# banyancomputer/hot-proofs-blake3-circom

Hardware: AMD Instinct MI355X
Metric: BLAKE3-compression witnesses/sec (higher is better)
Workload: dtype u32

## Files before the change

hot-proofs-blake3-circom_amd/__init__.py:

```python
import ctypes
import os
import re

import numpy as np

from . import workloads


def __getattr__(name):
    if name in ("sharding", "chain", "bao"):
        import importlib
        return importlib.import_module(__name__ + "." + name)
    raise AttributeError(name)

PKG_DIR = os.path.dirname(os.path.abspath(__file__))
LIB_PATH = os.environ.get("B3WIT_LIB") or os.path.join(PKG_DIR, "libb3wit.so")

CIRCUITS = ("compression", "nova_bn254", "nova_vesta", "nova_bn254_o1")
CIRCUIT_ID = {c: i for i, c in enumerate(CIRCUITS)}

B3W_OK = 0
PLACEMENT_NAMES = {0: "plain", 1: "mixed", 2: "interleaved"}
B3W_E_ASSERT_FAILED = 4
B3W_E_BAD_ARGUMENT = 100
B3W_E_NO_DEVICE = 101
B3W_E_DOMAIN = 103

_CIRCOM_ERR = {1: "Signal not found.\n", 2: "Too many signals set.\n", 3: "Signal already set.\n",
               4: "Assert Failed.\n", 5: "Not enough memory.\n", 6: "Input signal array access exceeds the size.\n"}


class B3WError(RuntimeError):
    def __init__(self, status, message):
        super().__init__(message)
        self.status = status


_lib = None


def lib():
    global _lib
    if _lib is not None:
        return _lib
    if not os.path.exists(LIB_PATH):
        raise B3WError(B3W_E_NO_DEVICE, f"{LIB_PATH} not built: run `python -c 'import __graft_entry__ as g; g.build()'`")
    try:
        import torch
    except ImportError:
        pass
    L = ctypes.CDLL(LIB_PATH)
    vp, u32, i32, u64, sz = ctypes.c_void_p, ctypes.c_uint32, ctypes.c_int32, ctypes.c_uint64, ctypes.c_size_t
    sig = {
        "b3w_abi_version": (u32, []),
        "b3w_identify_wasm": (i32, [vp, sz]),
        "b3w_create": (i32, [i32, i32, ctypes.POINTER(vp)]),
        "b3w_destroy": (None, [vp]),
        "b3w_info": (i32, [vp, vp, vp, vp, vp, vp]),
        "b3w_input_signal_size": (i32, [vp, u64]),
        "b3w_calc_witness": (i32, [vp, vp, vp, vp, u32, vp]),
        "b3w_write_wtns_header": (i32, [vp, vp]),
        "b3w_last_error": (i32, [vp, ctypes.c_char_p, sz]),
        "b3w_batch_run_device": (i32, [vp, vp, u32, vp, u64, vp, vp, vp]),
        "b3w_public_words": (u32, [vp]),
        "b3w_batch_alloc": (i32, [vp, u32, u64, ctypes.POINTER(vp)]),
        "b3w_batch_free": (None, [vp]),
        "b3w_batch_run": (i32, [vp, vp, u32, vp]),
        "b3w_batch_outputs": (i32, [vp, vp, vp]),
        "b3w_batch_fetch": (i32, [vp, u32, vp]),
        "b3w_batch_device_ptr": (vp, [vp, ctypes.POINTER(u64)]),
        "b3w_batch_time_device": (i32, [vp, vp, u32, vp, u64, vp, vp, vp, u32, ctypes.POINTER(ctypes.c_float)]),
        "b3w_batch_verify_device": (i32, [vp, vp, u32, u64, vp, vp]),
        "b3w_batch_verify": (i32, [vp, vp]),
        "b3w_r1cs_create": (i32, [vp, vp, sz, ctypes.POINTER(vp)]),
        "b3w_r1cs_info": (i32, [vp, ctypes.POINTER(u32), ctypes.POINTER(u32), ctypes.POINTER(u64), ctypes.POINTER(u32),
                                ctypes.POINTER(u32), ctypes.POINTER(u32)]),
        "b3w_r1cs_is_tiled": (i32, [vp]),
        "b3w_r1cs_destroy": (None, [vp]),
        "b3w_r1cs_check_device": (i32, [vp, vp, vp, u32, u64, vp, vp, vp]),
        "b3w_batch_r1cs_check": (i32, [vp, vp, vp, vp]),
        "b3w_r1cs_consumer": (None, [vp, vp, u64, u64, u32, vp]),
        "b3w_batch_write_wtns": (i32, [vp, u32, u32, ctypes.c_char_p, ctypes.c_char_p, ctypes.POINTER(u32)]),
        "b3w_batch_write_wtns_ex": (i32, [vp, u32, u32, ctypes.c_char_p, ctypes.c_char_p, u32, ctypes.POINTER(u32)]),
        "b3w_batch_autotune_device": (i32, [vp, vp, u32, vp, u64, vp, vp, vp, ctypes.POINTER(i32), ctypes.POINTER(ctypes.c_float)]),
        "b3w_bodies_alloc": (i32, [vp, u64, ctypes.POINTER(vp), ctypes.POINTER(i32)]),
        "b3w_bodies_free": (i32, [vp, vp]),
        "b3w_bodies_trim": (None, []),
        "b3w_ctx_trim": (i32, [vp]),
        "b3w_bodies_configure": (None, [ctypes.c_int64, ctypes.c_int64]),
        "b3w_bodies_stats": (i32, [vp, vp]),
        "b3w_bodies_search_stats": (i32, [vp, ctypes.POINTER(ctypes.c_double)]),
        "b3w_bodies_search_limit": (None, [ctypes.c_double]),
        "b3w_bodies_search_breakdown": (i32, [vp, ctypes.POINTER(ctypes.c_double)]),
        "b3w_bodies_store_rate": (i32, [vp, vp, u32, u64, i32, u32, vp, ctypes.POINTER(ctypes.c_double)]),
        "b3w_batch_placement": (i32, [vp]),
        "b3w_chain_num_chunks": (u64, [u64]),
        "b3w_chain_num_leaf_steps": (u64, [u64]),
        "b3w_chain_path_len": (u32, [u64, u64]),
        "b3w_chain_num_parent_steps": (u64, [u64, u64, u64]),
        "b3w_chain_parent_row": (u64, [u64, u64]),
        "b3w_chain_path_provable": (i32, [u64, u64]),
        "b3w_chain_plan_leaves_device": (i32, [vp, vp, u64, u64, u32, vp, vp, vp]),
        "b3w_chain_tree_device": (i32, [vp, vp, u64, vp, vp]),
        "b3w_chain_plan_parents_device": (i32, [vp, vp, u64, u64, u64, u32, vp, vp]),
        "b3w_commit_key_create": (i32, [vp, i32, u32, vp, ctypes.POINTER(vp)]),
        "b3w_commit_key_create_ex": (i32, [vp, i32, u32, vp, u32, ctypes.POINTER(vp)]),
        "b3w_commit_key_create_folded": (i32, [vp, i32, u32, vp, vp, u32, ctypes.POINTER(vp)]),
        "b3w_slot_widths": (i32, [vp, vp]),
        "b3w_commit_key_window": (u32, [vp]),
        "b3w_commit_key_destroy": (None, [vp]),
        "b3w_commit_key_count": (i32, [vp, i32]),
        "b3w_commit_key_counts": (i32, [vp, ctypes.POINTER(u64)]),
        "b3w_commit_records_device": (i32, [vp, vp, vp, u32, vp, vp, vp, vp]),
        "b3w_commit_records": (i32, [vp, vp, vp, u32, vp, vp, vp]),
        "b3w_chain_commit_only": (i32, [vp, vp, vp]),
        "b3w_chain_commit_from_records": (i32, [vp, vp, vp]),
        "b3w_chain_commit_overlap": (i32, [vp, i32]),
        "b3w_chain_violations_device": (vp, [vp]),
        "b3w_chain_commitments": (i32, [vp, vp, vp]),
        "b3w_chain_check_constraints": (i32, [vp, vp]),
        "b3w_chain_violations": (i32, [vp, vp, vp]),
        "b3w_batch_commit_device": (i32, [vp, vp, vp, u32, u64, vp, vp, vp]),
        "b3w_batch_commit": (i32, [vp, vp, vp, vp]),
        "b3w_commit_consumer": (None, [vp, vp, u64, u64, u32, vp]),
        "b3w_comm_unique_id": (i32, [vp]),
        "b3w_comm_create": (i32, [vp, vp, i32, i32, ctypes.POINTER(vp)]),
        "b3w_comm_create_host": (i32, [vp, ctypes.c_char_p, i32, i32, ctypes.POINTER(vp)]),
        "b3w_comm_create_external": (i32, [vp, i32, i32, vp, vp, ctypes.POINTER(vp)]),
        "b3w_comm_rank": (i32, [vp]),
        "b3w_comm_size": (i32, [vp]),
        "b3w_comm_destroy": (None, [vp]),
        "b3w_comm_allgather": (i32, [vp, vp, vp, u64, vp]),
        "b3w_batch_allgather_public": (i32, [vp, vp, vp]),
        "b3w_chain_create": (i32, [vp, u64, u64, u32, u32, u32, i32, ctypes.POINTER(vp)]),
        "b3w_chain_destroy": (None, [vp]),
        "b3w_chain_run_leaves": (i32, [vp, vp, vp, vp, vp]),
        "b3w_chain_run_parents": (i32, [vp, vp, vp, vp, vp]),
        "b3w_chain_shard": (None, [u64, i32, i32, ctypes.POINTER(u64), ctypes.POINTER(u32)]),
        "b3w_chain_run_parents_sharded": (i32, [vp, vp, vp, vp, vp]),
        "b3w_chain_allgather_hout": (i32, [vp, vp, vp, vp, vp]),
        "b3w_chain_allgather_hout_host": (i32, [vp, vp, vp, vp, vp]),
        "b3w_chain_exchange_ms": (i32, [vp, ctypes.POINTER(ctypes.c_float)]),
        "b3w_chain_info": (i32, [vp, ctypes.POINTER(u64), ctypes.POINTER(u64), ctypes.POINTER(u64), ctypes.POINTER(u32), ctypes.POINTER(i32)]),
        "b3w_chain_outputs": (i32, [vp, vp, vp, vp, vp]),
        "b3w_chain_records": (vp, [vp]),
        "b3w_chain_public": (vp, [vp]),
        "b3w_chain_status": (vp, [vp]),
        "b3w_chain_local_cvs": (vp, [vp]),
        "b3w_chain_root": (vp, [vp]),
        "b3w_bao_outboard_size": (u64, [u64]),
        "b3w_bao_outboard_device": (i32, [vp, vp, u64, vp, vp, vp, vp]),
        "b3w_bao_path_nodes": (i32, [u64, u64, ctypes.POINTER(u64), ctypes.POINTER(u32)]),
        "b3w_bao_slice": (i32, [vp, u64, u64, vp, vp, ctypes.POINTER(u64)]),
        "b3w_sample_rows": (ctypes.c_int64, [u64, vp, u32, vp]),
        "b3w_sample_plan_device": (i32, [vp, u64, vp, vp, vp, u32, vp, vp, vp, vp]),
        "b3w_bao_batch_layout": (u64, [vp, u32, vp]),
        "b3w_bao_batch_scratch_bytes": (u64, [vp, u32]),
        "b3w_bao_outboard_batch_device": (i32, [vp, vp, vp, vp, u32, vp, vp, vp, u64, vp]),
        "b3w_sample_rows_batch": (ctypes.c_int64, [vp, u32, vp, vp, u32, vp]),
        "b3w_sample_plan_batch_device": (i32, [vp, vp, u32, vp, vp, vp, vp, u32, vp, vp, vp, vp]),
        "b3w_bao_group_outboard_size": (u64, [u64, u32]),
        "b3w_bao_group_batch_layout": (u64, [vp, u32, u32, vp]),
        "b3w_bao_group_path_nodes": (i32, [u64, u64, u32, ctypes.POINTER(u64), ctypes.POINTER(u32)]),
        "b3w_bao_group_outboard_batch_device": (i32, [vp, vp, vp, vp, u32, u32, vp, vp, vp, u64, vp]),
        "b3w_sample_plan_group_batch_device": (i32, [vp, vp, u32, u32, vp, vp, vp, vp, u32, vp, vp, vp, vp]),
        "b3w_bao_slice_size": (u64, [u64, u64]),
        "b3w_bao_slice_batch_layout": (ctypes.c_int64, [vp, u32, vp, vp, u32, vp]),
        "b3w_bao_slice_decode": (i32, [vp, u64, u64, u64, vp, vp, ctypes.POINTER(u32), ctypes.POINTER(i32)]),
        "b3w_bao_slice_batch_device": (i32, [vp, vp, u32, u32, vp, vp, vp, u32, vp, vp, vp]),
        "b3w_sample_plan_slices_device": (i32, [vp, vp, u32, vp, vp, vp, u32, vp, vp, vp, vp]),
        "b3w_bao_verify_layout": (u64, [vp, u32, u32, vp]),
        "b3w_bao_verify_scratch_bytes": (u64, [vp, u32]),
        "b3w_bao_verify_batch_device": (i32, [vp, vp, vp, vp, u32, u32, vp, vp, vp, vp, vp, vp, u64, vp]),
        "b3w_bao_verify": (i32, [vp, u64, vp, u32, vp, vp, ctypes.POINTER(i32), ctypes.POINTER(u64)]),
        "b3w_bao_stream_scratch_bytes": (u64, [u64, u32]),
        "b3w_bao_stream_outboard_begin": (i32, [vp, u64, u32, vp, vp, vp, u64, ctypes.POINTER(vp)]),
        "b3w_bao_stream_verify_begin": (i32, [vp, u64, u32, vp, vp, vp, vp, vp, vp, u64, vp, ctypes.POINTER(vp)]),
        "b3w_bao_stream_push": (i32, [vp, u64, vp, u64, vp]),
        "b3w_bao_stream_finish": (i32, [vp, vp]),
        "b3w_bao_stream_free": (None, [vp]),
        "b3w_bao_stream_push_many": (i32, [vp, vp, vp, vp, vp, u32, vp]),
        "b3w_bao_stream_finish_many": (i32, [vp, vp, u32, vp]),
        "b3w_bao_stream_open_staging_bytes": (u64, [u64, u32]),
        "b3w_bao_stream_open_scratch_bytes": (u64, [u64]),
        "b3w_bao_stream_open_block_pos": (u64, [u64, u32, u64]),
        "b3w_bao_stream_open_begin": (i32, [vp, u64, u32, vp, u64, vp, u64, ctypes.POINTER(vp)]),
        "b3w_bao_stream_open_finish": (i32, [vp, vp, u64, vp, u64, vp, vp, ctypes.POINTER(u64)]),
        "b3w_bao_stream_open_finish_many": (i32, [vp, vp, vp, vp, vp, vp, vp, u32, vp, vp]),
        "b3w_sample_plan_arena_device": (i32, [vp, vp, u64, vp, vp, u32, u32, vp, vp, vp, vp, u32, vp, vp, vp]),
        "b3w_bao_slice_arena_device": (i32, [vp, vp, u64, vp, vp, u32, u32, vp, vp, vp, u32, vp, vp]),
        "b3w_bao_update_scratch_bytes": (u64, [vp, vp, vp, vp, u32]),
        "b3w_bao_outboard_update_batch_device": (i32, [vp, vp, u64, vp, vp, u32, u32, vp, vp, vp, vp, vp, vp, u32, vp, u64, vp]),
        "b3w_bao_outboard_update": (i32, [vp, u64, vp, u32, vp, vp, u32, vp]),
        "b3w_bao_resize_kept_tiles": (u64, [u64, u64]),
        "b3w_bao_resize_scratch_bytes": (u64, [vp, vp, u32]),
        "b3w_bao_outboard_resize_batch_device": (i32, [vp, vp, u64, vp, vp, vp, u32, u32, vp, vp, vp, vp, vp, vp, u32, vp, u64, vp]),
        "b3w_bao_outboard_resize": (i32, [vp, u64, vp, u64, u32, vp, vp]),
        "b3w_bao_verify_ranges_scratch_bytes": (u64, [vp, vp, vp, vp, u32]),
        "b3w_bao_verify_ranges_batch_device": (i32, [vp, vp, u64, vp, vp, u32, u32, vp, vp, vp, vp, vp, vp, u32, vp, vp, vp, vp, vp, u64, vp]),
        "b3w_bao_verify_ranges": (i32, [vp, u64, vp, u32, vp, vp, vp, u32, vp, vp, vp]),
    }
    for name, (res, args) in sig.items():
        fn = getattr(L, name)
        fn.restype, fn.argtypes = res, args
    _lib = L
    return L


EXPORTED_SYMBOLS = ("b3w_abi_version", "b3w_identify_wasm", "b3w_create", "b3w_destroy", "b3w_info",
                    "b3w_input_signal_size", "b3w_calc_witness", "b3w_write_wtns_header", "b3w_last_error",
                    "b3w_batch_run_device", "b3w_public_words", "b3w_batch_alloc", "b3w_batch_free",
                    "b3w_batch_run", "b3w_batch_outputs", "b3w_batch_fetch", "b3w_batch_device_ptr",
                    "b3w_batch_time_device", "b3w_batch_verify_device", "b3w_batch_verify",
                    "b3w_r1cs_create", "b3w_r1cs_info", "b3w_r1cs_is_tiled", "b3w_r1cs_destroy", "b3w_r1cs_check_device", "b3w_batch_r1cs_check", "b3w_r1cs_consumer", "b3w_batch_write_wtns", "b3w_batch_write_wtns_ex", "b3w_batch_autotune_device", "b3w_bodies_alloc", "b3w_bodies_free", "b3w_bodies_trim", "b3w_ctx_trim", "b3w_bodies_configure", "b3w_bodies_stats", "b3w_bodies_search_stats", "b3w_bodies_search_limit", "b3w_bodies_search_breakdown", "b3w_bodies_store_rate", "b3w_batch_placement", "b3w_chain_num_chunks", "b3w_chain_num_leaf_steps", "b3w_chain_path_len",
                    "b3w_chain_num_parent_steps", "b3w_chain_parent_row", "b3w_chain_path_provable",
                    "b3w_chain_plan_leaves_device", "b3w_chain_tree_device", "b3w_chain_plan_parents_device",
                    "b3w_commit_key_create", "b3w_commit_key_create_ex", "b3w_commit_key_create_folded", "b3w_slot_widths", "b3w_commit_key_window", "b3w_commit_key_destroy", "b3w_commit_key_count", "b3w_commit_key_counts", "b3w_commit_records_device", "b3w_commit_records", "b3w_chain_commit_only", "b3w_chain_commit_from_records", "b3w_chain_commit_overlap", "b3w_chain_violations_device", "b3w_chain_commitments", "b3w_chain_check_constraints", "b3w_chain_violations", "b3w_batch_commit_device", "b3w_batch_commit", "b3w_commit_consumer",
                    "b3w_comm_unique_id", "b3w_comm_create", "b3w_comm_create_host", "b3w_comm_create_external", "b3w_comm_rank", "b3w_comm_size", "b3w_comm_destroy", "b3w_comm_allgather", "b3w_batch_allgather_public",
                    "b3w_chain_create", "b3w_chain_destroy", "b3w_chain_run_leaves", "b3w_chain_run_parents", "b3w_chain_shard", "b3w_chain_run_parents_sharded", "b3w_chain_allgather_hout", "b3w_chain_allgather_hout_host", "b3w_chain_exchange_ms", "b3w_chain_info",
                    "b3w_chain_outputs", "b3w_chain_records", "b3w_chain_public", "b3w_chain_status", "b3w_chain_local_cvs", "b3w_chain_root",
                    "b3w_bao_outboard_size", "b3w_bao_outboard_device", "b3w_bao_path_nodes", "b3w_bao_slice", "b3w_sample_rows",
                    "b3w_sample_plan_device", "b3w_bao_batch_layout", "b3w_bao_batch_scratch_bytes", "b3w_bao_outboard_batch_device",
                    "b3w_sample_rows_batch", "b3w_sample_plan_batch_device", "b3w_bao_group_outboard_size", "b3w_bao_group_batch_layout",
                    "b3w_bao_group_path_nodes", "b3w_bao_group_outboard_batch_device", "b3w_sample_plan_group_batch_device",
                    "b3w_bao_slice_size", "b3w_bao_slice_batch_layout", "b3w_bao_slice_decode", "b3w_bao_slice_batch_device",
                    "b3w_sample_plan_slices_device",
                    "b3w_bao_verify_layout", "b3w_bao_verify_scratch_bytes", "b3w_bao_verify_batch_device", "b3w_bao_verify",
                    "b3w_bao_stream_scratch_bytes", "b3w_bao_stream_outboard_begin", "b3w_bao_stream_verify_begin", "b3w_bao_stream_push",
                    "b3w_bao_stream_finish", "b3w_bao_stream_free", "b3w_bao_stream_push_many", "b3w_bao_stream_finish_many",
                    "b3w_bao_stream_open_staging_bytes", "b3w_bao_stream_open_scratch_bytes", "b3w_bao_stream_open_block_pos",
                    "b3w_bao_stream_open_begin", "b3w_bao_stream_open_finish", "b3w_bao_stream_open_finish_many",
                    "b3w_sample_plan_arena_device", "b3w_bao_slice_arena_device",
                    "b3w_bao_update_scratch_bytes", "b3w_bao_outboard_update_batch_device", "b3w_bao_outboard_update",
                    "b3w_bao_resize_kept_tiles", "b3w_bao_resize_scratch_bytes", "b3w_bao_outboard_resize_batch_device", "b3w_bao_outboard_resize",
                    "b3w_bao_verify_ranges_scratch_bytes", "b3w_bao_verify_ranges_batch_device", "b3w_bao_verify_ranges")


class graph_capture:

    def __init__(self, graph, stream=None, **kw):
        import torch
        self._inner = torch.cuda.graph(graph, stream=stream, **kw)
        self._gc_was_on = False

    def __enter__(self):
        import gc
        gc.collect()
        self._gc_was_on = gc.isenabled()
        gc.disable()
        try:
            return self._inner.__enter__()
        except BaseException:
            if self._gc_was_on:
                gc.enable()
            raise

    def __exit__(self, *exc):
        import gc
        try:
            return self._inner.__exit__(*exc)
        finally:
            if self._gc_was_on:
                gc.enable()


def fnv_hash(name):
    h = 0xCBF29CE484222325
    for ch in name:
        h ^= ord(ch)
        h = (h * 0x100000001B3) % (1 << 64)
    return h


def flat_array(a):
    out = []

    def fill(x):
        if isinstance(x, (list, tuple)):
            for y in x:
                fill(y)
        else:
            out.append(x)
    fill(a)
    return out


def _to_int(v):
    if isinstance(v, str):
        return int(v, 0)
    return int(v)


class Context:

    def __init__(self, circuit, device=0):
        self.circuit = circuit if isinstance(circuit, str) else CIRCUITS[circuit]
        self._lib = lib()
        h = ctypes.c_void_p()
        rc = self._lib.b3w_create(CIRCUIT_ID[self.circuit], int(device), ctypes.byref(h))
        if rc != B3W_OK:
# ... 183 lines not shown
        c._cb = _ALLGATHER_FN(_cb)
        h = ctypes.c_void_p()
        rc = lib().b3w_comm_create_external(ctx.handle, int(rank), int(nranks), ctypes.cast(c._cb, ctypes.c_void_p), None, ctypes.byref(h))
        if rc != B3W_OK:
            raise B3WError(rc, f"b3w_comm_create_external: status {rc}: {ctx.last_error()}")
        c.handle = h
        return c

    def allgather(self, d_send, d_recv, bytes_per_rank, stream=0):
        rc = lib().b3w_comm_allgather(self.handle, d_send, d_recv, bytes_per_rank, stream or None)
        if rc != B3W_OK:
            err, self._cb_error = self._cb_error, None
            raise B3WError(rc, f"b3w_comm_allgather: status {rc}: {self.ctx.last_error()}" + (f" ({err!r})" if err else ""))

    def close(self):
        if getattr(self, "handle", None):
            lib().b3w_comm_destroy(self.handle)
            self.handle = None


R1CS_DIR = os.path.join(PKG_DIR, "constraints")
BUILTIN_R1CS = {"compression": "blake3_compression.r1cs.gz", "nova_bn254_o1": "blake3_nova_bn254_o1.r1cs.gz",
                "nova_bn254": "blake3_nova_bn254.r1cs.gz", "nova_vesta": "blake3_nova_vesta.r1cs.gz"}


def read_r1cs_image(image):
    if isinstance(image, (str, os.PathLike)):
        path = image if os.path.exists(image) else os.path.join(R1CS_DIR, image)
        raw = open(path, "rb").read()
        if raw[:2] == b"\x1f\x8b":
            import gzip
            raw = gzip.decompress(raw)
        return raw
    return bytes(image)


class R1cs:

    def __init__(self, ctx, image=None):
        self.ctx = ctx
        if image is None:
            if ctx.circuit not in BUILTIN_R1CS:
                raise B3WError(100, f"no derived constraint system for {ctx.circuit}: pass the circuit's .r1cs")
            image = os.path.join(R1CS_DIR, BUILTIN_R1CS[ctx.circuit])
        if isinstance(image, (str, os.PathLike)):
            raw = open(image, "rb").read()
            if raw[:2] == b"\x1f\x8b":
                import gzip
                raw = gzip.decompress(raw)
            image = raw
        buf = bytes(image)
        h = ctypes.c_void_p()
        rc = lib().b3w_r1cs_create(ctx.handle, buf, len(buf), ctypes.byref(h))
        if rc != B3W_OK:
            raise B3WError(rc, f"b3w_r1cs_create: status {rc}: {ctx.last_error()}")
        self.handle = h
        m, nw, nt, po, pi, pr = (ctypes.c_uint32(), ctypes.c_uint32(), ctypes.c_uint64(), ctypes.c_uint32(), ctypes.c_uint32(),
                                 ctypes.c_uint32())
        lib().b3w_r1cs_info(h, ctypes.byref(m), ctypes.byref(nw), ctypes.byref(nt), ctypes.byref(po), ctypes.byref(pi), ctypes.byref(pr))
        self.n_constraints, self.n_wires, self.n_terms = m.value, nw.value, nt.value
        self.n_pub_out, self.n_pub_in, self.n_prv_in = po.value, pi.value, pr.value
        self.tiled = bool(lib().b3w_r1cs_is_tiled(h))

    def check_device(self, d_bodies, n, pitch, d_violations, d_first=0, stream=0):
        rc = lib().b3w_r1cs_check_device(self.ctx.handle, self.handle, d_bodies, n, pitch, d_violations, d_first or None, stream or None)
        if rc != B3W_OK:
            raise B3WError(rc, f"b3w_r1cs_check_device: status {rc}: {self.ctx.last_error()}")

    def close(self):
        if getattr(self, "handle", None):
            lib().b3w_r1cs_destroy(self.handle)
            self.handle = None

    def __del__(self):
        try:
            self.close()
        except Exception:
            pass


class CommitKey:
    CURVES = {"bn254_g1": 0, "pallas": 1, "vesta": 1}

    def __init__(self, ctx, curve, generators, first_slot=0, window=0, fold=None):
        self.ctx = ctx
        buf = bytes(generators)
        nslots = ctx.witness_size - first_slot
        if len(buf) != 64 * nslots:
            raise B3WError(100, "generators: 64 bytes per committed slot")
        self.folded_slots, mask = 0, None
        if fold is not None and fold is not False:
            from . import fold as _fold
            image = read_r1cs_image(BUILTIN_R1CS[ctx.circuit]) if fold is True else read_r1cs_image(fold)
            buf, mask, self.fold_stats = _fold.fold_generators(image, ctx.slot_widths(), first_slot, buf, curve)
            self.folded_slots = sum(1 for v in mask if v)
        h = ctypes.c_void_p()
        rc = lib().b3w_commit_key_create_folded(ctx.handle, self.CURVES[curve], first_slot, buf, bytes(mask) if mask is not None else None, window,
                                                ctypes.byref(h))
        if rc != B3W_OK:
            raise B3WError(rc, f"b3w_commit_key_create_folded: status {rc}: {ctx.last_error()}")
        self.handle = h
        self.window = lib().b3w_commit_key_window(h)

    def commit_device(self, d_bodies, n, pitch, d_points, d_status=0, stream=0):
        rc = lib().b3w_batch_commit_device(self.ctx.handle, self.handle, d_bodies, n, pitch, d_points, d_status or None, stream or None)
        if rc != B3W_OK:
            raise B3WError(rc, f"b3w_batch_commit_device: status {rc}: {self.ctx.last_error()}")

    def commit_records_device(self, d_records, n, d_points, d_status, d_public=0, stream=0):
        rc = lib().b3w_commit_records_device(self.ctx.handle, self.handle, d_records, n, d_points, d_public or None, d_status, stream or None)
        if rc != B3W_OK:
            raise B3WError(rc, f"b3w_commit_records_device: status {rc}: {self.ctx.last_error()}")

    def commit_records(self, records):
        recs = np.ascontiguousarray(records, dtype=np.uint32)
        n = recs.shape[0]
        pts = np.zeros((n, 64), dtype=np.uint8)
        pub = np.zeros((n, self.ctx.public_words), dtype=np.uint32)
        st = np.zeros(n, dtype=np.int32)
        rc = lib().b3w_commit_records(self.ctx.handle, self.handle, recs.ctypes.data, n, pts.ctypes.data, pub.ctypes.data, st.ctypes.data)
        if rc != B3W_OK:
            raise B3WError(rc, f"b3w_commit_records: status {rc}: {self.ctx.last_error()}")
        return pts, pub, st

    def count(self, on=True):
        lib().b3w_commit_key_count(self.handle, 1 if on else 0)

    def counts(self):
        out = (ctypes.c_uint64 * 2)()
        lib().b3w_commit_key_counts(self.handle, out)
        return int(out[0]), int(out[1])

    def close(self):
        if getattr(self, "handle", None):
            lib().b3w_commit_key_destroy(self.handle)
            self.handle = None

    def __del__(self):
        try:
            self.close()
        except Exception:
            pass


class ChainPlanner:

    def __init__(self, ctx):
        self.ctx = ctx

    def _chk(self, rc, what):
        if rc != B3W_OK:
            raise B3WError(rc, f"{what}: status {rc}: {self.ctx.last_error()}")

    def parent_rows(self, n_chunks, first_chunk=0, n_chunks_local=None):
        L = lib()
        nl = n_chunks - first_chunk if n_chunks_local is None else n_chunks_local
        r0 = L.b3w_chain_parent_row(first_chunk, n_chunks)
        return [(L.b3w_chain_parent_row(c, n_chunks) - r0, L.b3w_chain_path_len(c, n_chunks), bool(L.b3w_chain_path_provable(c, n_chunks)))
                for c in range(first_chunk, first_chunk + nl)]

    def plan(self, d_preimage, with_parents=True, first_chunk=0, n_chunks_local=None, stream=0):
        import torch
        L = lib()
        ln = d_preimage.numel()
        dev = d_preimage.device
        n = L.b3w_chain_num_chunks(ln)
        nl = n - first_chunk if n_chunks_local is None else n_chunks_local
        last_local = first_chunk + nl == n
        last_blocks = (max(ln - (n - 1) * 1024, 1) + 63) // 64
        n_leaf = nl * 16 - ((16 - last_blocks) if last_local else 0)
        P = L.b3w_chain_path_len(0, n)
        complete = (n & (n - 1)) == 0
        n_par = L.b3w_chain_num_parent_steps(ln, first_chunk, nl) if with_parents else 0
        recs = torch.zeros((nl * 16 + n_par, 32), dtype=torch.int32, device=dev)
        levels = torch.zeros(((2 * n + 64) * 8,), dtype=torch.int32, device=dev)
        root = torch.zeros(8, dtype=torch.int32, device=dev)
        s = stream or None
        allrecs = recs if (first_chunk == 0 and nl == n) else None
        if allrecs is None:
            tmp = torch.zeros((n * 16, 32), dtype=torch.int32, device=dev)
            self._chk(L.b3w_chain_plan_leaves_device(self.ctx.handle, d_preimage.data_ptr(), ln, 0, n, tmp.data_ptr(),
                                                     levels.data_ptr(), s), "plan_leaves")
            recs[:nl * 16] = tmp[first_chunk * 16:(first_chunk + nl) * 16]
        else:
            self._chk(L.b3w_chain_plan_leaves_device(self.ctx.handle, d_preimage.data_ptr(), ln, 0, n, recs.data_ptr(),
                                                     levels.data_ptr(), s), "plan_leaves")
        self._chk(L.b3w_chain_tree_device(self.ctx.handle, levels.data_ptr(), n, root.data_ptr(), s), "tree")
        if n_par:
            self._chk(L.b3w_chain_plan_parents_device(self.ctx.handle, levels.data_ptr(), n, ln, first_chunk, nl,
                                                      recs[nl * 16:].data_ptr(), s), "plan_parents")
        if last_local and last_blocks < 16:
            keep = torch.ones(recs.shape[0], dtype=torch.bool, device=dev)
            keep[(nl - 1) * 16 + last_blocks: nl * 16] = False
            recs = recs[keep].contiguous()
        return dict(records=recs, n_leaf_steps=n_leaf, n_parent_steps=n_par, chunk_cvs=levels[:n * 8].view(n, 8),
                    root=root, n_chunks=n, path_len=P, complete=complete, last_blocks=last_blocks)


class Batch:

    def __init__(self, ctx, capacity, pitch=0):
        self.ctx = ctx
        h = ctypes.c_void_p()
        rc = lib().b3w_batch_alloc(ctx.handle, capacity, pitch, ctypes.byref(h))
        if rc != B3W_OK:
            raise B3WError(rc, f"b3w_batch_alloc: status {rc}: {ctx.last_error()}")
        self.handle, self.capacity, self.n = h, capacity, 0

    def run(self, records):
        records = np.ascontiguousarray(records, dtype=np.uint32)
        assert records.ndim == 2 and records.shape[1] == self.ctx.input_size
        rc = lib().b3w_batch_run(self.handle, records.ctypes.data, records.shape[0], None)
        if rc != B3W_OK:
            raise B3WError(rc, f"b3w_batch_run: status {rc}: {self.ctx.last_error()}")
        self.n = records.shape[0]

    def outputs(self):
        pub = np.zeros((self.n, self.ctx.public_words), dtype=np.uint32)
        st = np.zeros(self.n, dtype=np.int32)
# ... 153 lines not shown
```

hot-proofs-blake3-circom_amd/build.py:

```python
import os, shutil, subprocess, sys

PKG = os.path.dirname(os.path.abspath(__file__))
ROOT = os.path.dirname(PKG)
CSRC = os.path.join(PKG, "csrc")
LIB = os.path.join(PKG, "libb3wit.so")
NAPI = os.path.join(PKG, "js", "b3wit_napi.node")
ARCH = "gfx950"


def _newer(target, sources):
    if not os.path.exists(target):
        return True
    t = os.path.getmtime(target)
    return any(os.path.getmtime(s) > t for s in sources)


def _run(cmd, **kw):
    print("+", " ".join(cmd), flush=True)
    subprocess.check_call(cmd, **kw)


def hipcc():
    for c in (os.environ.get("HIPCC"), shutil.which("hipcc"), "/opt/rocm/bin/hipcc"):
        if c and os.path.exists(c):
            return c
    raise RuntimeError("hipcc not found")


def build_lib(force=False, extra_flags=()):
    from concurrent.futures import ThreadPoolExecutor
    names = ("b3w_kernels.hip", "b3w_exact.hip", "b3w_plan.hip", "b3w_bao.hip", "b3w_placement.hip", "b3w_commit.hip", "b3w_r1cs.hip", "b3w_r1cs_walk.hip", "b3w_r1cs_host.cpp", "b3w_hostcomm.cpp",
             "b3w_ctx.cpp", "b3w_bodies.cpp", "b3w_wtns.cpp", "b3w_r1cs_api.cpp", "b3w_commit_api.cpp", "b3w_comm.cpp", "b3w_chain.cpp")
    srcs = [os.path.join(CSRC, f) for f in names]
    hdrs = [os.path.join(CSRC, f) for f in sorted(os.listdir(CSRC)) if f.endswith((".h", ".inc"))] + \
        [os.path.join(ROOT, "include", "b3wit.h")]
    objdir = os.path.join(PKG, "build")
    os.makedirs(objdir, exist_ok=True)
    if os.environ.get("B3W_BUILD_DIAG") == "1":
        extra_flags = (*extra_flags, "-DB3W_R1CS_DIAG")
    flags = [f"--offload-arch={ARCH}", "-O3", "-std=c++17", "-fPIC", "-x", "hip", "-Wall", "-Wno-unused-function", *extra_flags]
    jobs = []
    for src in srcs:
        obj = os.path.join(objdir, os.path.basename(src) + ".o")
        if force or extra_flags or _newer(obj, [src] + hdrs):
            jobs.append([hipcc(), *flags, "-c", src, "-o", obj])
    if jobs:
        with ThreadPoolExecutor(max_workers=min(len(jobs), os.cpu_count() or 1)) as ex:
            list(ex.map(_run, jobs))
    objs = [os.path.join(objdir, os.path.basename(src) + ".o") for src in srcs]
    if jobs or _newer(LIB, objs):
        _run([hipcc(), f"--offload-arch={ARCH}", "-fPIC", "-shared", "-o", LIB, *objs, "-ldl", "-lrt", "-lpthread"])
    return LIB


def build_oracle(force=False):
    so = os.path.join(ROOT, "oracle", "libb3w_oracle.so")
    if force or _newer(so, [os.path.join(ROOT, "oracle", "b3w_oracle.c")]):
        _run(["make", "-C", os.path.join(ROOT, "oracle")])
    return so


def build_napi(force=False):
    src = os.path.join(PKG, "js", "b3wit_napi.cc")
    if not os.path.exists(src):
        return None
    inc = "/usr/include/node"
    if not os.path.exists(os.path.join(inc, "node_api.h")):
        print("node_api.h not found; skipping N-API addon", file=sys.stderr)
        return None
    if force or _newer(NAPI, [src, os.path.join(ROOT, "include", "b3wit.h")]):
        _run(["g++", "-O2", "-std=c++17", "-fPIC", "-shared", "-DNODE_GYP_MODULE_NAME=b3wit_napi", "-I", inc,
              "-I", os.path.join(ROOT, "include"), "-o", NAPI, src, "-ldl"])
    return NAPI


def build_all(force=False):
    build_lib(force)
    build_oracle(force)
    build_napi(force)


if __name__ == "__main__":
    build_all(force="--force" in sys.argv)
```

hot-proofs-blake3-circom_amd/chain.py:

```python
import ctypes

import numpy as np
import torch
import torch.distributed as dist

from . import B3W_OK, PLACEMENT_NAMES, B3WError, lib
from .sharding import gather_rows, shard_range


def _chk(ctx, rc, what):
    if rc != B3W_OK:
        raise B3WError(rc, f"{what}: status {rc}: {ctx.last_error()}")


class _DevArray:

    def __init__(self, ptr, shape, typestr):
        self.__cuda_array_interface__ = {"shape": tuple(shape), "typestr": typestr, "data": (ptr, False), "version": 2,
                                         "strides": None}


def _view(ptr, shape, typestr, dev):
    return torch.as_tensor(_DevArray(ptr, shape, typestr), device=dev)


_CONSUMER = ctypes.CFUNCTYPE(None, ctypes.c_void_p, ctypes.c_void_p, ctypes.c_uint64, ctypes.c_uint64, ctypes.c_uint32,
                             ctypes.c_void_p)


def step_shards(preimage_len, world, with_parents=True):
    L = lib()
    n = L.b3w_chain_num_chunks(preimage_len)
    last_bytes = preimage_len - (n - 1) * 1024 if preimage_len > (n - 1) * 1024 else 0
    last_blocks = -(-last_bytes // 64) if last_bytes else 1
    out = []
    for r in range(world):
        f, e = shard_range(n, r, world)
        k = e - f
        leaf = k * 16 - ((16 - last_blocks) if (k and e == n) else 0)
        p0 = L.b3w_chain_parent_row(f, n) if with_parents else 0
        p1 = L.b3w_chain_parent_row(e, n) if with_parents else 0
        out.append((f, k, leaf, p0, p1 - p0))
    return out


def gather_h_out(public_local, n_leaf_local, preimage_len, with_parents=True, group=None):
    world = dist.get_world_size(group) if dist.is_initialized() else 1
    h = public_local[:, 2:10]
    if world == 1:
        return h[:n_leaf_local], h[n_leaf_local:]
    sh = step_shards(preimage_len, world, with_parents)
    leaf = gather_rows(h[:n_leaf_local].contiguous(), [x[2] for x in sh], group)
    par = gather_rows(h[n_leaf_local:].contiguous(), [x[4] for x in sh], group)
    return leaf, par


COMMIT_OVERLAP = {"auto": -1, "serial": 0, "free": 1, "gated": 2}


def fold_witnesses(ctx, preimage, batch_steps=16384, ring=2, slice_chunks=1024, with_parents=True, consumer=None,
                   device=None, commit_only=None, gather_hout=True, comm=None, commit_records=None, check=None, commit_overlap="auto"):
    L = lib()
    world = dist.get_world_size() if dist.is_initialized() else 1
    rank = dist.get_rank() if dist.is_initialized() else 0
    if comm is not None:
        world, rank = comm.nranks, comm.rank
    dev = device or torch.device("cuda", torch.cuda.current_device())
    host = torch.from_numpy(preimage) if isinstance(preimage, np.ndarray) else preimage
    assert host.dtype == torch.uint8 and host.dim() == 1 and host.numel() > 0 and host.is_contiguous()
    ln = host.numel()
    n = L.b3w_chain_num_chunks(ln)
    c0, c1 = shard_range(n, rank, world)
    nl = c1 - c0
    body = ctx.body_bytes

    cache = ctx.__dict__.setdefault("_chain_cache", {})
    key = (ln, c0, nl, batch_steps, ring, bool(with_parents))
    if key not in cache:
        for h in cache.values():
            L.b3w_chain_destroy(h)
        cache.clear()
        h = ctypes.c_void_p()
        _chk(ctx, L.b3w_chain_create(ctx.handle, ln, c0, nl, batch_steps, ring, 1 if with_parents else 0, ctypes.byref(h)),
             "b3w_chain_create")
        cache[key] = h
    h = cache[key]
    nleaf, npar, nch, P, pl = ctypes.c_uint64(), ctypes.c_uint64(), ctypes.c_uint64(), ctypes.c_uint32(), ctypes.c_int32()
    L.b3w_chain_info(h, ctypes.byref(nleaf), ctypes.byref(npar), ctypes.byref(nch), ctypes.byref(P), ctypes.byref(pl))
    n_leaf, n_par = nleaf.value, npar.value
    if commit_only is not None:
        _chk(ctx, L.b3w_chain_commit_only(h, commit_only[0].handle, commit_only[1].data_ptr()), "b3w_chain_commit_only")
    elif commit_records is not None:
        _chk(ctx, L.b3w_chain_commit_from_records(h, commit_records[0].handle, commit_records[1].data_ptr()), "b3w_chain_commit_from_records")
    else:
        _chk(ctx, L.b3w_chain_commit_only(h, None, None), "b3w_chain_commit_only")
    if commit_records is not None:
        _chk(ctx, L.b3w_chain_commit_overlap(h, COMMIT_OVERLAP[commit_overlap]), "b3w_chain_commit_overlap")
    _chk(ctx, L.b3w_chain_check_constraints(h, check.handle if check is not None else None), "b3w_chain_check_constraints")
    compute = torch.cuda.current_stream(dev)
    nbatch = [0]
    cb = _CONSUMER()
    if consumer is not None:
        def _cb(user, d_bodies, pitch, first_step, count, stream):
            nbatch[0] += 1
            consumer(_view(d_bodies, (count, body), "|u1", dev), first_step, count)
        cb = _CONSUMER(_cb)
    _chk(ctx, L.b3w_chain_run_leaves(h, host.data_ptr(), cb, None, compute.cuda_stream), "b3w_chain_run_leaves")

    rows = n_leaf + n_par
    public = _view(L.b3w_chain_public(h), (rows, 15), "<i4", dev)
    h_leaf, h_par = None, None
    timer = None
    if comm is not None:
        _chk(ctx, L.b3w_chain_run_parents_sharded(h, comm.handle, cb, None, compute.cuda_stream), "b3w_chain_run_parents_sharded")
        if gather_hout:
            sh = step_shards(ln, world, with_parents)
            h_leaf = torch.empty((sum(x[2] for x in sh), 8), dtype=torch.int32, device=dev)
            h_par = torch.empty((sum(x[4] for x in sh), 8), dtype=torch.int32, device=dev)
            with torch.cuda.stream(compute):
                _chk(ctx, L.b3w_chain_allgather_hout(h, comm.handle, h_leaf.data_ptr(), h_par.data_ptr() if h_par.numel() else None,
                                                     compute.cuda_stream), "b3w_chain_allgather_hout")
        timer = ("native", h, bool(gather_hout))
    else:
        all_cvs = None
        ev = [torch.cuda.Event(enable_timing=True) for _ in range(4)] if world > 1 else None
        if world > 1:
            ev[0].record(compute)
            cvs_local = _view(L.b3w_chain_local_cvs(h), (max(nl, 1), 8), "<i4", dev)
            all_cvs = gather_rows(cvs_local[:nl], [e - s for s, e in (shard_range(n, r, world) for r in range(world))]).contiguous()
            ev[1].record(compute)
        _chk(ctx, L.b3w_chain_run_parents(h, all_cvs.data_ptr() if all_cvs is not None else None, cb, None, compute.cuda_stream),
             "b3w_chain_run_parents")
        if gather_hout or world == 1:
            if world > 1:
                ev[2].record(compute)
            h_leaf, h_par = gather_h_out(public, n_leaf, ln, with_parents)
            if world > 1:
                ev[3].record(compute)
        if world > 1:
            timer = ("torch", ev, bool(gather_hout))

    return dict(public=public, h_out_all=h_leaf, h_out_parents_all=h_par, chunk_cvs_local=_view(L.b3w_chain_local_cvs(h), (max(nl, 1), 8), "<i4", dev)[:nl],
                status=_view(L.b3w_chain_status(h), (rows,), "<i4", dev),
                violations=_view(L.b3w_chain_violations_device(h), (rows,), "<i4", dev) if check is not None else None,
                records=_view(L.b3w_chain_records(h), (rows, 32), "<i4", dev), root=_view(L.b3w_chain_root(h), (8,), "<i4", dev),
                n_leaf_steps=n_leaf, n_parent_steps=n_par, first_chunk=c0, n_chunks_local=nl, n_chunks=n, path_len=P.value,
                batches=-(-n_leaf // batch_steps) + -(-n_par // batch_steps) if consumer is None else nbatch[0],
                placement=PLACEMENT_NAMES.get(pl.value, "plain"), exchange_timer=timer)


def exchange_ms(out):
    t = out.get("exchange_timer")
    if t is None:
        return 0.0, 0.0
    if t[0] == "native":
        ms = (ctypes.c_float * 2)()
        lib().b3w_chain_exchange_ms(t[1], ms)
        return float(ms[0]), float(ms[1]) if t[2] else 0.0
    ev = t[1]
    ev[1].synchronize()
    a = ev[0].elapsed_time(ev[1])
    b = 0.0
    if t[2]:
        ev[3].synchronize()
        b = ev[2].elapsed_time(ev[3])
    return a, b
```

hot-proofs-blake3-circom_amd/csrc/b3w_commit.hip:

```cpp
#include <hip/hip_runtime.h>
#include <stdint.h>
#include <stdlib.h>
#include "b3w_kernels.h"
#include "b3w_atoms.h"

namespace {

struct Fp { uint32_t l[8]; };
struct Jac { Fp X, Y, Z; };

__device__ __forceinline__ bool fp_is_zero(const Fp &a) {
  uint32_t o = 0;
#pragma unroll
  for (int i = 0; i < 8; ++i) o |= a.l[i];
  return o == 0;
}
__device__ __forceinline__ bool fp_eq(const Fp &a, const Fp &b) {
  uint32_t o = 0;
#pragma unroll
  for (int i = 0; i < 8; ++i) o |= a.l[i] ^ b.l[i];
  return o == 0;
}
__device__ __forceinline__ Fp fp_zero() { Fp r; for (int i = 0; i < 8; ++i) r.l[i] = 0; return r; }

// ... 443 lines not shown
  const F9 XX = sqr29(P.X, C), M = s_add(s_dbl(XX, C), XX, C);
  const F9 X3 = s_sub(sqr29(M, C), s_dbl(S, C), C);
  const F9 Y3 = s_sub(mul29(M, s_sub(S, X3, C), C), mul29(W, P.Y, C), C);
  P.ZZ = mul29(V, P.ZZ, C);
  P.ZZZ = mul29(W, P.ZZZ, C);
  P.X = X3; P.Y = Y3;
}
template <class CV>
__device__ __forceinline__ void j9_madd(J9 &P, const F9 &x2, const F9 &y2, const CV &C) {
  if (P.inf) {
    P.X = x2; P.Y = y2; P.ZZ = one29(C); P.ZZZ = one29(C); P.inf = false;
    return;
  }
  const F9 U2 = mul29(x2, P.ZZ, C), S2 = mul29(y2, P.ZZZ, C);
  const F9 Pd = cn29(sub29(U2, P.X, C));
  const F9 R = cn29(sub29(S2, P.Y, C));
  if (Pd.l[0] == C.kp0[0] || Pd.l[0] == C.kp0[1] || Pd.l[0] == C.kp0[2]) {
    if (is_kp29(Pd, 3, C) || is_kp29(Pd, 4, C) || is_kp29(Pd, 5, C)) {
      if (!(is_kp29(R, 3, C) || is_kp29(R, 4, C) || is_kp29(R, 5, C))) { P.inf = true; return; }
      P.X = x2; P.Y = y2; P.ZZ = one29(C); P.ZZZ = one29(C);
      j9_dbl(P, C);
      return;
    }
  }
  const F9 PP = sqr29(Pd, C);
  const F9 PPP = mul29(Pd, PP, C), Q = mul29(P.X, PP, C);
  const F9 X3 = red29(add29(add29(sqr29(R, C), neg29(PPP, C)), shl29(neg29(Q, C), 1)), C);
  P.Y = muladd29(R, sub29(Q, X3, C), neg29(P.Y, C), PPP, C);
  P.X = X3;
  P.ZZ = mul29(P.ZZ, PP, C);
  P.ZZZ = mul29(P.ZZZ, PPP, C);
}
template <class CV>
__device__ __forceinline__ void j9_add(J9 &P, const J9 &Q, const CV &C) {
  if (Q.inf) return;
  if (P.inf) { P.X = Q.X; P.Y = Q.Y; P.ZZ = Q.ZZ; P.ZZZ = Q.ZZZ; P.inf = false; return; }
  const F9 U1 = mul29(P.X, Q.ZZ, C), U2 = mul29(Q.X, P.ZZ, C);
  const F9 S1 = mul29(P.Y, Q.ZZZ, C), S2 = mul29(Q.Y, P.ZZZ, C);
  const F9 Pd = s_sub(U2, U1, C), R = s_sub(S2, S1, C);
  if (s_is_zero(Pd, C)) {
    if (s_is_zero(R, C)) j9_dbl(P, C); else P.inf = true;
    return;
  }
  const F9 PP = sqr29(Pd, C), PPP = mul29(Pd, PP, C), Qq = mul29(U1, PP, C);
  const F9 X3 = s_sub(s_sub(sqr29(R, C), PPP, C), s_dbl(Qq, C), C);
  P.Y = s_sub(mul29(R, s_sub(Qq, X3, C), C), mul29(S1, PPP, C), C);
  P.ZZ = mul29(mul29(P.ZZ, Q.ZZ, C), PP, C);
  P.ZZZ = mul29(mul29(P.ZZZ, Q.ZZZ, C), PPP, C);
  P.X = X3;
}

__global__ __launch_bounds__(64) void b3w_commit_setup_kernel(const uint32_t *__restrict__ gens ,
                                                              const uint32_t *__restrict__ first_v, const uint32_t *__restrict__ nbits,
                                                              uint32_t nslots, uint32_t *__restrict__ points, B3wCurve C) {
  const uint32_t s = blockIdx.x, t = threadIdx.x;
  if (s >= nslots) return;
  const uint32_t nb = nbits[s], v0 = first_v[s];
  if (t >= nb) return;
  Fp r2;
#pragma unroll
  for (int i = 0; i < 8; ++i) r2.l[i] = C.r2[i];
  Jac P;
  P.X = fp_mul(load_fp(gens + (uint64_t)s * 16), r2, C);
  P.Y = fp_mul(load_fp(gens + (uint64_t)s * 16 + 8), r2, C);
#pragma unroll
  for (int i = 0; i < 8; ++i) P.Z.l[i] = C.one[i];
  Fp c32;
#pragma unroll
  for (int k = 0; k < 8; ++k) c32.l[k] = C.one[k];
#pragma unroll 1
  for (int k = 0; k < 5; ++k) c32 = fp_dbl(c32, C);
#pragma unroll 1
  for (uint32_t i = 0; i < t; ++i) P = jac_dbl(P, C);
#pragma unroll 1
  for (uint32_t k = t; k < nb; k += 64) {
    Fp x, y;
    if (k == 0) { x = P.X; y = P.Y; } else jac_to_affine(P, x, y, C);
    store_fp(points + (uint64_t)(v0 + k) * 16, fp_mul(x, c32, C));
    store_fp(points + (uint64_t)(v0 + k) * 16 + 8, fp_mul(y, c32, C));
    if (k + 64 < nb)
#pragma unroll 1
      for (int i = 0; i < 64; ++i) P = jac_dbl(P, C);
  }
}

__global__ __launch_bounds__(64) void b3w_commit_invtab_kernel(const uint32_t *__restrict__ gens ,
                                                               const uint32_t *__restrict__ inv_slot ,
                                                               const uint32_t *__restrict__ inverses ,
                                                               uint32_t njobs, uint32_t nk, uint32_t *__restrict__ invtab, B3wCurve C) {
  const uint64_t gid = (uint64_t)blockIdx.x * 64 + threadIdx.x;
  if (gid >= (uint64_t)njobs * nk) return;
  const uint32_t j = (uint32_t)(gid / nk), mag = (uint32_t)(gid % nk) + 1u;
  uint32_t *o = invtab + ((uint64_t)j * 2 * nk + mag - 1u) * 16, *on = o + (uint64_t)nk * 16;
  const uint32_t s = inv_slot[j];
  if (s == 0xFFFFFFFFu) { store_fp(o, fp_zero()); store_fp(o + 8, fp_zero()); store_fp(on, fp_zero()); store_fp(on + 8, fp_zero()); return; }
  Fp r2;
#pragma unroll
  for (int i = 0; i < 8; ++i) r2.l[i] = C.r2[i];
  const Fp gx = fp_mul(load_fp(gens + (uint64_t)s * 16), r2, C), gy = fp_mul(load_fp(gens + (uint64_t)s * 16 + 8), r2, C);
  const uint32_t *sc = inverses + 8ull * mag;
  Jac R = jac_infinity();
#pragma unroll 1
  for (int b = 255; b >= 0; --b) {
    R = jac_dbl(R, C);
    if ((sc[b >> 5] >> (b & 31)) & 1u) R = jac_madd(R, gx, gy, C);
  }
  Fp x, y, c32;
  jac_to_affine(R, x, y, C);
#pragma unroll
  for (int k = 0; k < 8; ++k) c32.l[k] = C.one[k];
#pragma unroll 1
  for (int k = 0; k < 5; ++k) c32 = fp_dbl(c32, C);
  const Fp xo = fp_mul(x, c32, C);
  store_fp(o, xo);
  store_fp(o + 8, fp_mul(y, c32, C));
  store_fp(on, xo);
  store_fp(on + 8, fp_mul(fp_sub(fp_zero(), y, C), c32, C));
}

#define B3W_WINDOW_K 4
template <int W>
__global__ __launch_bounds__(64) void b3w_commit_window_kernel(const uint32_t *__restrict__ points, uint32_t nwin,
                                                               uint32_t *__restrict__ table, B3wCurve C, B3wCurve9 C9) {
  constexpr int K = B3W_WINDOW_K;
  constexpr uint32_t CHUNKS = (1u << W) / K;
  __shared__ uint32_t lds[5 * K * 9 * 64];
  const uint32_t tid = threadIdx.x;
  const uint64_t gid = (uint64_t)blockIdx.x * 64 + tid;
  if (gid >= (uint64_t)nwin * CHUNKS) return;
  const uint32_t win = (uint32_t)(gid / CHUNKS), g0 = (uint32_t)(gid % CHUNKS) * K;
  auto at = [&](int what, int e, int l) -> uint32_t & { return lds[((what * K + e) * 9 + l) * 64 + tid]; };
  auto point = [&](uint32_t b, bool negate, F9 &x, F9 &y) {
    const uint32_t *pt = points + (uint64_t)(win * W + b) * 16;
    Fp py = load_fp(pt + 8);
    if (negate) py = fp_sub(fp_zero(), py, C);
    x = to29(load_fp(pt)); y = to29(py);
  };
  J9 acc = j9_infinity();
  const uint32_t m0 = g0 ^ (g0 >> 1);
#pragma unroll 1
  for (uint32_t b = 0; b < (uint32_t)W; ++b) {
    if (!((m0 >> b) & 1)) continue;
    F9 x, y;
    point(b, false, x, y);
    j9_madd(acc, x, y, C9);
  }
#pragma unroll 1
  for (int e = 0; e < K; ++e) {
    if (e > 0) {
      const uint32_t g = g0 + e, m = g ^ (g >> 1), b = (uint32_t)__builtin_ctz(g);
      F9 x, y;
      point(b, !((m >> b) & 1), x, y);
      j9_madd(acc, x, y, C9);
    }
    const F9 A = acc.inf ? one29(C9) : mul29(acc.ZZ, acc.ZZZ, C9);
#pragma unroll
    for (int l = 0; l < 9; ++l) {
      at(0, e, l) = acc.X.l[l]; at(1, e, l) = acc.Y.l[l];
      at(2, e, l) = acc.inf ? 0u : acc.ZZ.l[l]; at(3, e, l) = acc.inf ? 0u : acc.ZZZ.l[l];
    }
    F9 c;
    if (e == 0) c = A;
    else {
#pragma unroll
      for (int l = 0; l < 9; ++l) c.l[l] = at(4, e - 1, l);
      c = mul29(c, A, C9);
// ... 301 lines not shown
    F9 a = one29(C9);
    if (w < n) {
      const F9 zz = coord(w, 2);
      if (!is_zero(zz)) a = mul29(zz, coord(w, 3), C9);
    }
    pre[e] = e == 0 ? a : mul29(pre[e - 1], a, C9);
  }
  F9 inv = inv29(pre[K - 1], C.pm2, C9);
  F9 unit;
#pragma unroll
  for (int i = 0; i < 9; ++i) unit.l[i] = i == 0 ? 1u : 0u;
#pragma unroll
  for (int e = K - 1; e >= 0; --e) {
    const uint64_t w = w0 + e;
    if (w >= n) continue;
    const F9 zz = coord(w, 2);
    Fp x = fp_zero(), y = fp_zero();
    if (!is_zero(zz)) {
      const F9 zzz = coord(w, 3);
      const F9 ia = e > 0 ? mul29(inv, pre[e - 1], C9) : inv;
      inv = mul29(inv, mul29(zz, zzz, C9), C9);
      const F9 xs = mul29(mul29(coord(w, 0), mul29(ia, zzz, C9), C9), unit, C9);
      const F9 ys = mul29(mul29(coord(w, 1), mul29(ia, zz, C9), C9), unit, C9);
      uint32_t hi;
      x = from29(xs, hi); x = fp_reduce_once(x, hi, C);
      y = from29(ys, hi); y = fp_reduce_once(y, hi, C);
    }
    uint32_t *o = reinterpret_cast<uint32_t *>(out + w * 64);
    store_fp(o, x);
    store_fp(o + 8, y);
  }
}

void u288_split29(const uint32_t w[9], uint32_t out[9]) {
  for (int k = 0; k < 9; ++k) {
    const int bit = 29 * k, i = bit >> 5, sh = bit & 31;
    uint64_t v = w[i];
    if (i + 1 < 9) v |= (uint64_t)w[i + 1] << 32;
    out[k] = (uint32_t)(v >> sh) & (k < 8 ? M29 : 0xFFFFFFFFu);
  }
}
bool u256_geq_h(const uint32_t a[8], const uint32_t b[8]) {
  for (int i = 7; i >= 0; --i) if (a[i] != b[i]) return a[i] > b[i];
  return true;
}
void u256_dbl_mod_h(uint32_t a[8], const uint32_t p[8]) {
  uint32_t c = 0;
  for (int i = 0; i < 8; ++i) { const uint32_t n = (a[i] << 1) | c; c = a[i] >> 31; a[i] = n; }
  if (c || u256_geq_h(a, p)) { uint64_t br = 0; for (int i = 0; i < 8; ++i) { const uint64_t t = (uint64_t)a[i] - p[i] - br; a[i] = (uint32_t)t; br = (t >> 63) & 1; } }
}
B3wCurve9 make_curve9(const B3wCurve &C) {
  B3wCurve9 D{};
  uint32_t w[9];
  for (int i = 0; i < 8; ++i) w[i] = C.p[i];
  w[8] = 0;
  u288_split29(w, D.p);
  uint32_t p4[9];
  for (int i = 0; i < 9; ++i) p4[i] = (i < 8 ? C.p[i] << 2 : 0u) | (i > 0 ? C.p[i - 1] >> 30 : 0u);
  u288_split29(p4, D.sp4);
  for (int i = 0; i < 8; ++i) D.sp4[i] += (1u << 29) - (i > 0 ? 1u : 0u);
  D.sp4[8] -= 1u;
  uint32_t x[8];
  for (int i = 0; i < 8; ++i) x[i] = C.one[i];
  for (int k = 0; k < 5; ++k) u256_dbl_mod_h(x, C.p);
  for (int i = 0; i < 8; ++i) w[i] = x[i];
  w[8] = 0;
  u288_split29(w, D.one);
  D.inv = C.inv & M29;
  const uint64_t phi = ((uint64_t)C.p[7] << 32) | C.p[6];
  D.mu = (uint32_t)((((unsigned __int128)1) << 77) / ((unsigned __int128)phi + 1));
  for (uint32_t k = 3; k <= 5; ++k) D.kp0[k - 3] = (k * D.p[0]) & M29;
  return D;
}

}

extern "C" int b3w_launch_commit_setup(const uint32_t *d_gens, const uint32_t *d_first_v, const uint32_t *d_nbits, uint32_t nslots,
                                       uint32_t *d_points, const B3wCurve *curve, hipStream_t stream) {
  if (!nslots) return 0;
  hipLaunchKernelGGL(b3w_commit_setup_kernel, dim3(nslots), dim3(64), 0, stream, d_gens, d_first_v, d_nbits, nslots, d_points, *curve);
  return (int)hipGetLastError();
}

extern "C" int b3w_launch_commit_windows(const uint32_t *d_points, uint32_t nwin, uint32_t window, uint32_t *d_table, const B3wCurve *curve, hipStream_t stream) {
  if (!nwin) return 0;
  if (!B3W_COMMIT_WINDOW_OK(window)) return (int)hipErrorInvalidValue;
  const uint64_t total = (uint64_t)nwin * ((1u << window) / B3W_WINDOW_K);
  const dim3 grid((uint32_t)((total + 63) / 64));
  const B3wCurve9 c9 = make_curve9(*curve);
  if (window == B3W_COMMIT_WINDOW_XL)
    hipLaunchKernelGGL(b3w_commit_window_kernel<B3W_COMMIT_WINDOW_XL>, grid, dim3(64), 0, stream, d_points, nwin, d_table, *curve, c9);
  else if (window == B3W_COMMIT_WINDOW_LARGE)
    hipLaunchKernelGGL(b3w_commit_window_kernel<B3W_COMMIT_WINDOW_LARGE>, grid, dim3(64), 0, stream, d_points, nwin, d_table, *curve, c9);
  else
    hipLaunchKernelGGL(b3w_commit_window_kernel<B3W_COMMIT_WINDOW_SMALL>, grid, dim3(64), 0, stream, d_points, nwin, d_table, *curve, c9);
  return (int)hipGetLastError();
}

extern "C" int b3w_launch_commit(const uint8_t *d_bodies, uint32_t n, uint64_t pitch, uint32_t first_slot, uint32_t nslots,
                                 const uint32_t *d_slotdesc, const uint32_t *d_images , uint32_t img_row, const uint32_t *d_runs,
                                 uint32_t nruns, const uint32_t *d_table, uint32_t nwin, uint32_t window,
                                 uint32_t *d_sums , uint8_t *d_out, int32_t *d_status,
                                 const uint32_t *d_invtab, uint32_t inv_nk, const uint32_t *d_invmeta, const uint32_t *d_aux,
                                 unsigned long long *d_adds, const B3wCurve *curve, hipStream_t stream) {
  if (!n) return 0;
  if (!d_images && !(d_invtab && d_invmeta && d_aux)) { d_invtab = nullptr; d_invmeta = nullptr; }
  if (!B3W_COMMIT_WINDOW_OK(window)) return (int)hipErrorInvalidValue;
  const uint32_t bits_words = (nwin * window + 31) / 32 + 2;
  if (bits_words * 4 > 32 * 1024) return (int)hipErrorInvalidValue;
  const B3wCurve9 c9 = make_curve9(*curve);
  static const int env_tpw = getenv("B3W_COMMIT_THREADS") ? atoi(getenv("B3W_COMMIT_THREADS")) : 0;
  const int tpw = window > B3W_COMMIT_WINDOW_LARGE ? 64 : env_tpw ? env_tpw : ((uint64_t)nwin * window > 55200 || n >= 8192) ? 64 : 32;
  bool vesta = true;
  for (int i = 0; i < 9; ++i) vesta = vesta && c9.p[i] == B3wCurve9Vesta::P(i);
  vesta = vesta && c9.inv == B3wCurve9Vesta::INV() && tpw == 64;
  B3wCurve9Vesta c9v;
  static_cast<B3wCurve9 &>(c9v) = c9;
#define B3W_COMMIT_LAUNCH(T, WPB, W, CV, cv)                                                                              \
  {                                                                                                                       \
    const uint32_t region = bits_words > 36u * T ? bits_words : 36u * T;                                                  \
    if ((size_t)region * WPB * 4 > 64 * 1024) return (int)hipErrorInvalidValue;    \
    hipLaunchKernelGGL((b3w_commit_kernel<T, WPB, W, CV>), dim3((n + WPB - 1) / WPB), dim3(T * WPB), region * WPB * 4, stream, d_bodies, n, \
                       pitch, first_slot, nslots, d_slotdesc, d_images, img_row, reinterpret_cast<const uint2 *>(d_runs), nruns, region, d_table, nwin, \
                       d_sums, d_status, d_invtab, inv_nk, d_invmeta, d_aux, d_adds, cv);                                         \
  }
  if (window == B3W_COMMIT_WINDOW_XL) {
    if (vesta) B3W_COMMIT_LAUNCH(64, 4, B3W_COMMIT_WINDOW_XL, B3wCurve9Vesta, c9v)
    else B3W_COMMIT_LAUNCH(64, 4, B3W_COMMIT_WINDOW_XL, B3wCurve9, c9)
  } else if (window == B3W_COMMIT_WINDOW_LARGE) {
    if (vesta) B3W_COMMIT_LAUNCH(64, 4, B3W_COMMIT_WINDOW_LARGE, B3wCurve9Vesta, c9v)
    else if (tpw == 64) B3W_COMMIT_LAUNCH(64, 4, B3W_COMMIT_WINDOW_LARGE, B3wCurve9, c9)
    else B3W_COMMIT_LAUNCH(32, 2, B3W_COMMIT_WINDOW_LARGE, B3wCurve9, c9)
  } else {
    if (vesta) B3W_COMMIT_LAUNCH(64, 4, B3W_COMMIT_WINDOW_SMALL, B3wCurve9Vesta, c9v)
    else if (tpw == 64) B3W_COMMIT_LAUNCH(64, 4, B3W_COMMIT_WINDOW_SMALL, B3wCurve9, c9)
    else B3W_COMMIT_LAUNCH(32, 2, B3W_COMMIT_WINDOW_SMALL, B3wCurve9, c9)
  }
#undef B3W_COMMIT_LAUNCH
  if (!d_out) return (int)hipGetLastError();
  if (vesta) hipLaunchKernelGGL(b3w_commit_normalize_kernel<B3wCurve9Vesta>, dim3((n + 63) / 64), dim3(64), 0, stream, d_sums, n, d_out, *curve, c9v);
  else hipLaunchKernelGGL(b3w_commit_normalize_kernel<B3wCurve9>, dim3((n + 63) / 64), dim3(64), 0, stream, d_sums, n, d_out, *curve, c9);
  return (int)hipGetLastError();
}

extern "C" int b3w_launch_commit_normalize(const uint32_t *d_sums, uint64_t n, uint8_t *d_out, const B3wCurve *curve, hipStream_t stream) {
  if (!n) return 0;
  const B3wCurve9 c9 = make_curve9(*curve);
  const uint64_t threads = (n + B3W_NORMALIZE_K - 1) / B3W_NORMALIZE_K;
  hipLaunchKernelGGL(b3w_commit_normalize_many_kernel<B3wCurve9>, dim3((uint32_t)((threads + 63) / 64)), dim3(64), 0, stream, d_sums, n, d_out, *curve, c9);
  return (int)hipGetLastError();
}

extern "C" int b3w_launch_commit_invtab(const uint32_t *d_gens, const uint32_t *d_inv_slot, const uint32_t *d_inverses, uint32_t njobs, uint32_t nk,
                                        uint32_t *d_invtab, const B3wCurve *curve, hipStream_t stream) {
  if (!njobs || !nk) return 0;
  const uint64_t total = (uint64_t)njobs * nk;
  hipLaunchKernelGGL(b3w_commit_invtab_kernel, dim3((uint32_t)((total + 63) / 64)), dim3(64), 0, stream, d_gens, d_inv_slot, d_inverses, njobs, nk, d_invtab,
                     *curve);
  return (int)hipGetLastError();
}
```

hot-proofs-blake3-circom_amd/csrc/b3w_commit_api.cpp:

```cpp
#include "b3w_internal.h"


struct b3w_commit_key {
  b3w_ctx *ctx = nullptr;
  B3wCurve curve{};
  uint32_t first_slot = 0, nwin = 0, window = 0;
  uint32_t nslots = 0;
  uint32_t *d_slotdesc = nullptr;
  uint32_t *d_runs = nullptr; uint32_t nruns = 0;
  uint32_t *d_images = nullptr; uint32_t images_cap = 0;
  uint32_t *d_table = nullptr;
  uint32_t *d_invtab = nullptr; uint32_t inv_nk = 0;
  uint32_t *d_invmeta = nullptr;
  uint32_t *d_sums = nullptr;
  uint32_t sums_cap = 0;
  unsigned long long *d_counts = nullptr;
  uint64_t host_witnesses = 0;
  bool counting = false;
};

namespace {
bool u256_geq(const uint32_t a[8], const uint32_t b[8]) { for (int i = 7; i >= 0; --i) if (a[i] != b[i]) return a[i] > b[i]; return true; }
void u256_sub_host(uint32_t a[8], const uint32_t b[8]) {
  uint64_t br = 0;
  for (int i = 0; i < 8; i++) { const uint64_t t = (uint64_t)a[i] - b[i] - br; a[i] = (uint32_t)t; br = (t >> 63) & 1; }
}
void u256_double_mod(uint32_t a[8], const uint32_t p[8]) {
  uint32_t c = 0;
  for (int i = 0; i < 8; i++) { const uint32_t n = (a[i] << 1) | c; c = a[i] >> 31; a[i] = n; }
  if (c || u256_geq(a, p)) u256_sub_host(a, p);
}
B3wCurve make_curve(const uint64_t p64[4]) {
  B3wCurve C{};
  memcpy(C.p, p64, 32);
  uint32_t x[8] = {1, 0, 0, 0, 0, 0, 0, 0};
  for (int i = 0; i < 256; i++) u256_double_mod(x, C.p);
  memcpy(C.one, x, 32);
  for (int i = 0; i < 256; i++) u256_double_mod(x, C.p);
  memcpy(C.r2, x, 32);
  memcpy(C.pm2, C.p, 32);
  const uint32_t two[8] = {2, 0, 0, 0, 0, 0, 0, 0};
  u256_sub_host(C.pm2, two);
  uint32_t inv = C.p[0];
  for (int i = 0; i < 5; i++) inv *= 2u - C.p[0] * inv;
  C.inv = 0u - inv;
  return C;
}
const uint64_t Q_BN254[4] = {0x3c208c16d87cfd47ull, 0x97816a916871ca8dull, 0xb85045b68181585dull, 0x30644e72e131a029ull};
const uint64_t P_VESTA_BASE[4] = {0x992d30ed00000001ull, 0x224698fc094cf91bull, 0x0ull, 0x4000000000000000ull};
}

extern "C" {

int32_t b3w_commit_key_create(b3w_ctx *ctx, int32_t curve, uint32_t first_slot, const uint8_t *host_generators, b3w_commit_key **out) {
  return b3w_commit_key_create_ex(ctx, curve, first_slot, host_generators, 0, out);
}

uint32_t b3w_commit_key_window(const b3w_commit_key *key) { return key ? key->window : 0; }

int32_t b3w_commit_key_create_ex(b3w_ctx *ctx, int32_t curve, uint32_t first_slot, const uint8_t *host_generators, uint32_t window_bits,
                                 b3w_commit_key **out) {
  return b3w_commit_key_create_folded(ctx, curve, first_slot, host_generators, nullptr, window_bits, out);
}

int32_t b3w_slot_widths(b3w_ctx *ctx, uint16_t *out_bits) {
  if (!ctx || !out_bits) return B3W_E_BAD_ARGUMENT;
  std::vector<uint32_t> table;
  if (!b3w_int_build_slot_table(ctx->desc, table, ctx->last_error)) return B3W_E_BAD_ARGUMENT;
  for (uint32_t i = 0; i < ctx->desc.nwit; i++) {
    const uint32_t mode = (table[i] >> 17) & 3u;
    out_bits[i] = mode == B3W_MODE_BIT ? 1 : mode == B3W_MODE_W32 ? 32 : mode == B3W_MODE_W64 ? 64 : 256;
  }
  return B3W_OK;
}

static int32_t commit_key_create_once(b3w_ctx *ctx, int32_t curve, uint32_t first_slot, const uint8_t *host_generators,
                                      const uint8_t *folded, uint32_t window_bits, b3w_commit_key **out, uint32_t *auto_window, hipError_t *herr);

int32_t b3w_commit_key_create_folded(b3w_ctx *ctx, int32_t curve, uint32_t first_slot, const uint8_t *host_generators,
                                     const uint8_t *folded , uint32_t window_bits, b3w_commit_key **out) {
  uint32_t chosen = 0;
  hipError_t herr = hipSuccess;
  int32_t rc = commit_key_create_once(ctx, curve, first_slot, host_generators, folded, window_bits, out, &chosen, &herr);
  while (rc == B3W_E_HIP && herr == hipErrorOutOfMemory && chosen > B3W_COMMIT_WINDOW_SMALL) {
    (void)hipGetLastError();
    const uint32_t narrower = chosen == B3W_COMMIT_WINDOW_XL ? B3W_COMMIT_WINDOW_LARGE : B3W_COMMIT_WINDOW_SMALL;
    uint32_t ignored = 0;
    herr = hipSuccess;
    rc = commit_key_create_once(ctx, curve, first_slot, host_generators, folded, narrower, out, &ignored, &herr);
    chosen = narrower;
  }
  return rc;
}

static int32_t commit_key_create_once(b3w_ctx *ctx, int32_t curve, uint32_t first_slot, const uint8_t *host_generators,
                                      const uint8_t *folded, uint32_t window_bits, b3w_commit_key **out, uint32_t *auto_window, hipError_t *herr) {
  if (!ctx || !out || !host_generators || (curve != B3W_CURVE_BN254_G1 && curve != B3W_CURVE_VESTA) || first_slot >= ctx->desc.nwit ||
      (window_bits != 0 && !B3W_COMMIT_WINDOW_OK(window_bits))) {
    if (ctx) ctx->last_error = "commit key: curve 0/1, first_slot < witness_size, window_bits 0 (auto), 12, 16 or 18";
    return B3W_E_BAD_ARGUMENT;
  }
  *out = nullptr;
  std::vector<uint32_t> table;
  if (!b3w_int_build_slot_table(ctx->desc, table, ctx->last_error)) return B3W_E_BAD_ARGUMENT;
  const uint32_t nslots = ctx->desc.nwit - first_slot;
  std::vector<uint32_t> nbits(nslots), first_v(nslots);
  uint64_t nv = 0;
  for (uint32_t i = 0; i < nslots; i++) {
    const uint32_t mode = (table[first_slot + i] >> 17) & 3u;
    nbits[i] = mode == B3W_MODE_BIT ? 1u : mode == B3W_MODE_W32 ? 32u : mode == B3W_MODE_W64 ? 64u : 256u;
    if (folded && folded[i] == 1) nbits[i] = 0;
    else if (folded && (folded[i] & 0x80)) {
      if (mode != B3W_MODE_W32 || (folded[i] & 0x60)) { ctx->last_error = "commit key: a single-bit fold needs a 32-bit slot and a bit below 32"; return B3W_E_BAD_ARGUMENT; }
      nbits[i] = 1;
    } else if (folded && folded[i]) { ctx->last_error = "commit key: folded[] holds 0, 1 or 0x80 | bit"; return B3W_E_BAD_ARGUMENT; }
    first_v[i] = (uint32_t)nv;
    nv += nbits[i];
  }
  DeviceGuard guard(ctx->device);
  hipError_t e = guard.err;
  uint32_t window = window_bits;
  if (!window && getenv("B3W_COMMIT_WINDOW")) {
    window = (uint32_t)atoi(getenv("B3W_COMMIT_WINDOW"));
    if (!B3W_COMMIT_WINDOW_OK(window)) window = 0;
  }
  if (!window) {
    size_t free_b = 0, total_b = 0;
    bool known = e == hipSuccess && hipMemGetInfo(&free_b, &total_b) == hipSuccess;
    if (known && getenv("B3W_COMMIT_ASSUME_FREE_GIB")) free_b = (size_t)atoll(getenv("B3W_COMMIT_ASSUME_FREE_GIB")) << 30;
    auto table_bytes = [&](uint32_t w) { return (nv / w + 1) * (uint64_t)B3W_COMMIT_ENTRIES(w) * 64; };
    window = known && table_bytes(B3W_COMMIT_WINDOW_XL) <= free_b / 4      ? B3W_COMMIT_WINDOW_XL
             : known && table_bytes(B3W_COMMIT_WINDOW_LARGE) <= free_b / 4 ? B3W_COMMIT_WINDOW_LARGE
                                                                           : B3W_COMMIT_WINDOW_SMALL;
    *auto_window = window;
  }
  const uint32_t V0 = (uint32_t)nv;
  nv = (nv + window - 1) / window * window;
  b3w_commit_key *key = new b3w_commit_key;
  key->ctx = ctx;
  key->curve = make_curve(curve == B3W_CURVE_BN254_G1 ? Q_BN254 : P_VESTA_BASE);
  key->first_slot = first_slot;
  key->window = window;
  key->nwin = (uint32_t)(nv / window);
  key->nslots = nslots;
  uint32_t *d_gens = nullptr, *d_first = nullptr, *d_nbits = nullptr, *d_points = nullptr;
  std::vector<uint32_t> desc(nslots);
  auto one_bit_of_word = [&](uint32_t i) { return folded && (folded[i] & 0x80) != 0; };
  for (uint32_t i = 0; i < nslots; i++)
    desc[i] = first_v[i] | (one_bit_of_word(i) ? 8u + (folded[i] & 31u) : nbits[i] == 0 ? 4u : nbits[i] == 1 ? 0u : nbits[i] == 32 ? 1u : nbits[i] == 64 ? 2u : 3u) << 24;
  static const bool want_invtab = !(getenv("B3W_COMMIT_INVTAB") && !strcmp(getenv("B3W_COMMIT_INVTAB"), "0"));
  const bool order_is_prime = (ctx->desc.prime == P_BN254 && curve == B3W_CURVE_BN254_G1) || (ctx->desc.prime == P_VESTA && curve == B3W_CURVE_PALLAS);
  const bool with_invtab = want_invtab && order_is_prime && ctx->desc.kind == B3W_KIND_NOVA_O2 && ctx->d_aux;
  std::vector<uint32_t> invmeta(2 * B3W_NOVA_ISZERO + 4, 0xFFFFFFFFu);
  if (with_invtab) {
    for (uint32_t i = 0; i < nslots; i++) {
      const uint32_t src = table[first_slot + i] & 0xFFFu;
      if (nbits[i] == 256 && src >= B3W_LDS_WIDE && (src - B3W_LDS_WIDE) % 8 == 0 && (src - B3W_LDS_WIDE) / 8 < B3W_NOVA_ISZERO)
        invmeta[(src - B3W_LDS_WIDE) / 8] = i;
    }
    const uint32_t want_src[4] = {B3W_LDS_NV + NV_N_BLOCKS, B3W_LDS_NV + NV_BLOCK_COUNT, B3W_LDS_NV + NV_TOTAL_DEPTH, B3W_LDS_NV + NV_DEPTH};
    bool inputs_found = true;
    for (int q = 0; q < 4; q++) {
      for (uint32_t sidx = 0; sidx < ctx->desc.nwit && invmeta[B3W_NOVA_ISZERO + q] == 0xFFFFFFFFu; sidx++)
        if ((table[sidx] & 0xFFFu) == want_src[q] && ((table[sidx] >> 17) & 3u) == B3W_MODE_W32 && ((table[sidx] >> 12) & 31u) == 0) invmeta[B3W_NOVA_ISZERO + q] = sidx;
      inputs_found = inputs_found && invmeta[B3W_NOVA_ISZERO + q] != 0xFFFFFFFFu;
    }
    for (uint32_t j = 0; j < B3W_NOVA_ISZERO; j++)
      if (invmeta[j] != 0xFFFFFFFFu) {
        invmeta[B3W_NOVA_ISZERO + 4 + j] = first_v[invmeta[j]];
        if (inputs_found) desc[invmeta[j]] = j | 5u << 24;
      }
  }
  std::vector<uint32_t> runs;
  for (uint32_t i = 0; i < nslots; i++) {
    const uint32_t ent = table[first_slot + i], src = ent & 0xFFFu, sh = (ent >> 12) & 31u, v0 = first_v[i];
    if (nbits[i] == 0) continue;
    if (one_bit_of_word(i)) {
      runs.push_back(v0 | 0u << 24); runs.push_back(src | (sh + (folded[i] & 31u)) << 16);
      continue;
    }
    if (nbits[i] == 1) {
      if (!runs.empty()) {
        const uint32_t a = runs[runs.size() - 2], b = runs[runs.size() - 1];
        const uint32_t plen = (a >> 24) + 1, pv = a & 0xFFFFFFu, psrc = b & 0xFFFFu, psh = b >> 16;
        if ((a >> 31) == 0 && psrc == src && psh + plen == sh && pv + plen == v0 && plen < 32 && i > 0 && nbits[i - 1] == 1) {
          runs[runs.size() - 2] = pv | plen << 24;
          continue;
        }
      }
      runs.push_back(v0 | 0u << 24); runs.push_back(src | sh << 16);
    } else {
      const uint32_t words = nbits[i] / 32;
      for (uint32_t k = 0; k < words; k++) {
        runs.push_back((v0 + 32 * k) | 31u << 24); runs.push_back((src + k) | ((k == 0 || k == 4) ? sh : 0u) << 16);
      }
    }
  }
  key->nruns = (uint32_t)(runs.size() / 2);
  if (e == hipSuccess) e = hipMalloc((void **)&key->d_runs, runs.size() * 4);
  if (e == hipSuccess) e = hipMemcpy(key->d_runs, runs.data(), runs.size() * 4, hipMemcpyHostToDevice);
  if (e == hipSuccess) e = hipMalloc((void **)&key->d_slotdesc, (size_t)nslots * 4);
  if (e == hipSuccess) e = hipMemcpy(key->d_slotdesc, desc.data(), (size_t)nslots * 4, hipMemcpyHostToDevice);
  if (e == hipSuccess) e = hipMalloc((void **)&key->d_table, (size_t)key->nwin * B3W_COMMIT_ENTRIES(window) * 64);
  if (e == hipSuccess) e = hipMalloc((void **)&d_points, (size_t)nv * 64);
  if (e == hipSuccess) e = hipMalloc((void **)&d_gens, (size_t)nslots * 64);
  if (e == hipSuccess) e = hipMalloc((void **)&d_first, (size_t)nslots * 4);
  if (e == hipSuccess) e = hipMalloc((void **)&d_nbits, (size_t)nslots * 4);
  if (e == hipSuccess) e = hipMemcpy(d_gens, host_generators, (size_t)nslots * 64, hipMemcpyHostToDevice);
  if (e == hipSuccess) e = hipMemcpy(d_first, first_v.data(), (size_t)nslots * 4, hipMemcpyHostToDevice);
  if (e == hipSuccess) e = hipMemcpy(d_nbits, nbits.data(), (size_t)nslots * 4, hipMemcpyHostToDevice);
  int rc = e == hipSuccess ? b3w_launch_commit_setup(d_gens, d_first, d_nbits, nslots, d_points, &key->curve, nullptr) : 0;
  for (uint32_t v = V0; v < nv && e == hipSuccess && rc == 0; v++)
    e = hipMemcpyAsync(d_points + (size_t)v * 16, d_points, 64, hipMemcpyDeviceToDevice, nullptr);
  if (e == hipSuccess && rc == 0) rc = b3w_launch_commit_windows(d_points, key->nwin, key->window, key->d_table, &key->curve, nullptr);
  if (e == hipSuccess && rc == 0 && with_invtab) {
    key->inv_nk = B3W_INV_TABLE_N - 1;
    e = hipMalloc((void **)&key->d_invmeta, invmeta.size() * 4);
    if (e == hipSuccess) e = hipMemcpy(key->d_invmeta, invmeta.data(), invmeta.size() * 4, hipMemcpyHostToDevice);
    if (e == hipSuccess) e = hipMalloc((void **)&key->d_invtab, (size_t)B3W_NOVA_ISZERO * 2 * key->inv_nk * 64);
    if (e == hipSuccess)
      rc = b3w_launch_commit_invtab(d_gens, key->d_invmeta, static_cast<const uint32_t *>(ctx->d_aux) + 16, B3W_NOVA_ISZERO, key->inv_nk, key->d_invtab, &key->curve,
                                    nullptr);
  }
  if (e == hipSuccess && rc == 0) e = hipDeviceSynchronize();
  if (d_gens) (void)hipFree(d_gens);
  if (d_first) (void)hipFree(d_first);
  if (d_nbits) (void)hipFree(d_nbits);
  if (d_points) (void)hipFree(d_points);
  if (e != hipSuccess || rc != 0) {
    b3w_commit_key_destroy(key);
    *herr = e != hipSuccess ? e : (hipError_t)rc;
    (void)hipGetLastError();
    return hip_fail(ctx, e != hipSuccess ? e : (hipError_t)rc, "commitment key set-up");
  }
  *out = key;
  return B3W_OK;
}

void b3w_commit_key_destroy(b3w_commit_key *key) {
  if (!key) return;
  B3wCaptureRelaxed relaxed;
  DeviceGuard guard(key->ctx->device);
  if (key->d_slotdesc) (void)hipFree(key->d_slotdesc);
  if (key->d_invmeta) (void)hipFree(key->d_invmeta);
  if (key->d_runs) (void)hipFree(key->d_runs);
  if (key->d_images) (void)hipFree(key->d_images);
  if (key->d_table) (void)hipFree(key->d_table);
  if (key->d_invtab) (void)hipFree(key->d_invtab);
  if (key->d_sums) (void)hipFree(key->d_sums);
  if (key->d_counts) (void)hipFree(key->d_counts);
  delete key;
}

int32_t b3w_commit_key_count(b3w_commit_key *key, int32_t on) {
  if (!key) return B3W_E_BAD_ARGUMENT;
  b3w_ctx *ctx = key->ctx;
  ON_DEVICE(ctx);
  HIP_TRY(ctx, hipDeviceSynchronize());
  if (on && !key->d_counts) HIP_TRY(ctx, hipMalloc((void **)&key->d_counts, 8));
  if (on) { HIP_TRY(ctx, hipMemset(key->d_counts, 0, 8)); key->host_witnesses = 0; }
  key->counting = on != 0;
  return B3W_OK;
}

int32_t b3w_commit_key_counts(const b3w_commit_key *key, uint64_t out[2]) {
  if (!key || !out) return B3W_E_BAD_ARGUMENT;
  b3w_ctx *ctx = key->ctx;
  out[0] = 0; out[1] = key->host_witnesses;
  if (!key->d_counts) return B3W_OK;
  ON_DEVICE(ctx);
  HIP_TRY(ctx, hipDeviceSynchronize());
  unsigned long long v = 0;
  HIP_TRY(ctx, hipMemcpy(&v, key->d_counts, 8, hipMemcpyDeviceToHost));
  out[0] = v;
  return B3W_OK;
}

int32_t b3w_batch_commit_device(b3w_ctx *ctx, const b3w_commit_key *key, const uint8_t *d_bodies, uint32_t n, uint64_t pitch,
                                uint8_t *d_points, int32_t *d_status, void *stream) {
  if (!ctx || !key || key->ctx != ctx || !d_bodies || !d_points) return B3W_E_BAD_ARGUMENT;
  const uint64_t body = 32ull * ctx->desc.nwit;
  if (pitch == 0) pitch = body;
  if (pitch < body || (pitch & 15) || (reinterpret_cast<uintptr_t>(d_bodies) & 15) || (reinterpret_cast<uintptr_t>(d_points) & 15)) {
    ctx->last_error = "pitch must be >= witness_size*32 and a multiple of 16, bodies and points 16-byte aligned";
    return B3W_E_BAD_ARGUMENT;
  }
  b3w_commit_key *k = const_cast<b3w_commit_key *>(key);
  ON_DEVICE(ctx);
  if (k->sums_cap < n) {
    HIP_TRY(ctx, hipStreamSynchronize((hipStream_t)stream));
    if (k->d_sums) (void)hipFree(k->d_sums);
    k->d_sums = nullptr; k->sums_cap = 0;
    HIP_TRY(ctx, hipMalloc((void **)&k->d_sums, (size_t)n * B3W_COMMIT_SUM_WORDS * 4));
    k->sums_cap = n;
  }
  const int rc = b3w_launch_commit(d_bodies, n, pitch, key->first_slot, key->nslots, key->d_slotdesc, nullptr, 0, nullptr, 0, key->d_table,
                                   key->nwin, key->window, k->d_sums, d_points, d_status, key->d_invtab, key->inv_nk, key->d_invmeta,
                                   static_cast<const uint32_t *>(ctx->d_aux), key->counting ? key->d_counts : nullptr, &key->curve, (hipStream_t)stream);
  if (rc == 0 && key->counting) k->host_witnesses += n;
  return rc ? hip_fail(ctx, (hipError_t)rc, "commit launch") : B3W_OK;
}

int32_t b3w_commit_records_device(b3w_ctx *ctx, const b3w_commit_key *key, const uint32_t *d_records, uint32_t n, uint8_t *d_points,
                                  uint32_t *d_public, int32_t *d_status, void *stream) {
  return b3w_int_commit_records(ctx, key, d_records, n, d_points, d_public, d_status, stream, nullptr, nullptr, nullptr);
}

}

int32_t b3w_int_commit_normalize(b3w_ctx *ctx, const b3w_commit_key *key, const uint32_t *d_sums, uint64_t n, uint8_t *d_points, void *stream) {
  if (!ctx || !key || key->ctx != ctx || !d_sums || !d_points) return B3W_E_BAD_ARGUMENT;
  ON_DEVICE(ctx);
  const int rc = b3w_launch_commit_normalize(d_sums, n, d_points, &key->curve, (hipStream_t)stream);
  return rc ? hip_fail(ctx, (hipError_t)rc, "commit normalise launch") : B3W_OK;
}

int32_t b3w_int_commit_records(b3w_ctx *ctx, const b3w_commit_key *key, const uint32_t *d_records, uint32_t n, uint8_t *d_points, uint32_t *d_public,
                               int32_t *d_status, void *stream, uint32_t *d_sums_out, void *trace_stream, hipEvent_t trace_done) {
  if (!ctx || !key || key->ctx != ctx || !d_records || !d_points || !d_status) return B3W_E_BAD_ARGUMENT;
  const bool split = trace_done != nullptr && trace_stream != stream;
  if (split && n > 32768u) return B3W_E_BAD_ARGUMENT;
  if (n == 0) return B3W_OK;
  if ((reinterpret_cast<uintptr_t>(d_points) & 15) || (reinterpret_cast<uintptr_t>(d_records) & 3)) {
    ctx->last_error = "records 4-byte and points 16-byte aligned";
    return B3W_E_BAD_ARGUMENT;
  }
  ON_DEVICE(ctx);
  b3w_commit_key *k = const_cast<b3w_commit_key *>(key);
  constexpr uint32_t CHUNK = 32768;
  const uint32_t want = std::min(n, CHUNK);
  if (k->images_cap < want || k->sums_cap < want) {
    HIP_TRY(ctx, hipStreamSynchronize((hipStream_t)stream));
    if (split) HIP_TRY(ctx, hipStreamSynchronize((hipStream_t)trace_stream));
    if (k->sums_cap < want) {
      if (k->d_sums) (void)hipFree(k->d_sums);
      k->d_sums = nullptr; k->sums_cap = 0;
      HIP_TRY(ctx, hipMalloc((void **)&k->d_sums, (size_t)want * B3W_COMMIT_SUM_WORDS * 4));
      k->sums_cap = want;
    }
    if (k->images_cap < want) {
      if (k->d_images) (void)hipFree(k->d_images);
      k->d_images = nullptr; k->images_cap = 0;
      HIP_TRY(ctx, hipMalloc((void **)&k->d_images, (size_t)want * ctx->desc.lds_words * 4));
      k->images_cap = want;
    }
  }
  const uint32_t cap = k->images_cap;
  const uint32_t rw = ctx->desc.nin, pw = ctx->desc.npub;
  for (uint32_t c0 = 0; c0 < n; c0 += cap) {
    const uint32_t cn = std::min(cap, n - c0);
    int lrc = b3w_launch_trace(ctx->desc.kind, d_records + (uint64_t)c0 * rw, cn, k->d_images, cap, ctx->d_table, ctx->desc.nwit,
                               d_public ? d_public + (uint64_t)c0 * pw : nullptr, d_status + c0, ctx->d_aux, (hipStream_t)(split ? trace_stream : stream));
    if (lrc == 0 && split) {
      hipError_t e = hipEventRecord(trace_done, (hipStream_t)trace_stream);
      if (e == hipSuccess) e = hipStreamWaitEvent((hipStream_t)stream, trace_done, 0);
      if (e != hipSuccess) return hip_fail(ctx, e, "TRACE event");
    }
    if (lrc == 0)
      lrc = b3w_launch_commit(nullptr, cn, 0, key->first_slot, key->nslots, key->d_slotdesc, k->d_images, cap, key->d_runs, key->nruns,
                              key->d_table, key->nwin, key->window, d_sums_out ? d_sums_out + (uint64_t)c0 * B3W_COMMIT_SUM_WORDS : k->d_sums,
                              d_sums_out ? nullptr : d_points + (uint64_t)c0 * 64, nullptr, key->d_invtab, key->inv_nk,
                              nullptr, nullptr, key->counting ? key->d_counts : nullptr, &key->curve, (hipStream_t)stream);
    if (lrc == 0 && key->counting) k->host_witnesses += cn;
    if (lrc) return hip_fail(ctx, (hipError_t)lrc, "commit-from-records launch");
  }
  return B3W_OK;
}

extern "C" {

int32_t b3w_commit_records(b3w_ctx *ctx, const b3w_commit_key *key, const uint32_t *host_records, uint32_t n, uint8_t *host_points,
                           uint32_t *host_public, int32_t *host_status) {
  if (!ctx || !key || key->ctx != ctx || !host_records || !host_points) return B3W_E_BAD_ARGUMENT;
  if (n == 0) return B3W_OK;
  ON_DEVICE(ctx);
  const size_t rb = (size_t)n * ctx->desc.nin * 4, pb = (size_t)n * ctx->desc.npub * 4;
  uint8_t *d = nullptr;
  const size_t o_pts = (rb + 255) & ~(size_t)255, o_pub = o_pts + (size_t)n * 64, o_st = o_pub + ((pb + 255) & ~(size_t)255);
  HIP_TRY(ctx, hipMalloc((void **)&d, o_st + (size_t)n * 4));
  hipError_t e = hipMemset(d + o_pub, 0, o_st - o_pub);
  if (e == hipSuccess) e = hipMemcpy(d, host_records, rb, hipMemcpyHostToDevice);
  int32_t rc = B3W_OK;
  if (e == hipSuccess) rc = b3w_commit_records_device(ctx, key, reinterpret_cast<uint32_t *>(d), n, d + o_pts, reinterpret_cast<uint32_t *>(d + o_pub),
                                                      reinterpret_cast<int32_t *>(d + o_st), nullptr);
  if (e == hipSuccess && rc == B3W_OK) e = hipMemcpy(host_points, d + o_pts, (size_t)n * 64, hipMemcpyDeviceToHost);
  if (e == hipSuccess && rc == B3W_OK && host_public) e = hipMemcpy(host_public, d + o_pub, pb, hipMemcpyDeviceToHost);
  if (e == hipSuccess && rc == B3W_OK && host_status) e = hipMemcpy(host_status, d + o_st, (size_t)n * 4, hipMemcpyDeviceToHost);
  (void)hipFree(d);
  if (rc) return rc;
  return e == hipSuccess ? B3W_OK : hip_fail(ctx, e, "hipMemcpy(commit from records)");
}

void b3w_commit_consumer(void *user, const uint8_t *d_bodies, uint64_t pitch, uint64_t first_step, uint32_t count, void *stream) {
  b3w_commit_sink *sink = static_cast<b3w_commit_sink *>(user);
  if (!sink || !sink->ctx || !sink->key || !sink->d_points) return;
  const int32_t rc = b3w_batch_commit_device(sink->ctx, sink->key, d_bodies, count, pitch, sink->d_points + first_step * 64,
                                             sink->d_status ? sink->d_status + first_step : nullptr, stream);
  if (rc && !sink->error) sink->error = rc;
}

int32_t b3w_batch_commit(b3w_batch *b, const b3w_commit_key *key, uint8_t *host_points, int32_t *host_status) {
  if (!b || !key || !host_points) return B3W_E_BAD_ARGUMENT;
  b3w_ctx *ctx = b->ctx;
  if (!b->n) return B3W_OK;
  ON_DEVICE(ctx);
  uint8_t *d_pts = nullptr;
  int32_t *d_st = nullptr;
  HIP_TRY(ctx, hipMalloc((void **)&d_pts, (size_t)b->n * 64));
  HIP_TRY(ctx, hipMalloc((void **)&d_st, (size_t)b->n * 4));
  int32_t rc = b3w_batch_commit_device(ctx, key, b->d_bodies, b->n, b->pitch, d_pts, d_st, nullptr);
  hipError_t e = rc == B3W_OK ? hipMemcpy(host_points, d_pts, (size_t)b->n * 64, hipMemcpyDeviceToHost) : hipSuccess;
  if (rc == B3W_OK && e == hipSuccess && host_status) e = hipMemcpy(host_status, d_st, (size_t)b->n * 4, hipMemcpyDeviceToHost);
  (void)hipFree(d_pts); (void)hipFree(d_st);
  if (rc) return rc;
  return e == hipSuccess ? B3W_OK : hip_fail(ctx, e, "hipMemcpy(commitments)");
}

}

b3w_ctx *b3w_int_key_ctx(const b3w_commit_key *key) { return key ? key->ctx : nullptr; }
```

hot-proofs-blake3-circom_amd/csrc/b3w_ctx.cpp:

```cpp
#include "b3w_internal.h"
#include "b3w_layout_tables.inc"
#include "b3w_trace_tables.inc"

namespace {

struct Sha256 {
  uint32_t h[8];
  uint8_t buf[64];
  uint64_t len = 0;
  size_t fill = 0;
  Sha256() {
    static const uint32_t init[8] = {0x6a09e667, 0xbb67ae85, 0x3c6ef372, 0xa54ff53a, 0x510e527f, 0x9b05688c, 0x1f83d9ab, 0x5be0cd19};
    memcpy(h, init, sizeof h);
  }
  static uint32_t ror(uint32_t x, int r) { return (x >> r) | (x << (32 - r)); }
  void block(const uint8_t *p) {
    static const uint32_t K[64] = {
        0x428a2f98, 0x71374491, 0xb5c0fbcf, 0xe9b5dba5, 0x3956c25b, 0x59f111f1, 0x923f82a4, 0xab1c5ed5, 0xd807aa98, 0x12835b01,
        0x243185be, 0x550c7dc3, 0x72be5d74, 0x80deb1fe, 0x9bdc06a7, 0xc19bf174, 0xe49b69c1, 0xefbe4786, 0x0fc19dc6, 0x240ca1cc,
        0x2de92c6f, 0x4a7484aa, 0x5cb0a9dc, 0x76f988da, 0x983e5152, 0xa831c66d, 0xb00327c8, 0xbf597fc7, 0xc6e00bf3, 0xd5a79147,
        0x06ca6351, 0x14292967, 0x27b70a85, 0x2e1b2138, 0x4d2c6dfc, 0x53380d13, 0x650a7354, 0x766a0abb, 0x81c2c92e, 0x92722c85,
        0xa2bfe8a1, 0xa81a664b, 0xc24b8b70, 0xc76c51a3, 0xd192e819, 0xd6990624, 0xf40e3585, 0x106aa070, 0x19a4c116, 0x1e376c08,
        0x2748774c, 0x34b0bcb5, 0x391c0cb3, 0x4ed8aa4a, 0x5b9cca4f, 0x682e6ff3, 0x748f82ee, 0x78a5636f, 0x84c87814, 0x8cc70208,
        0x90befffa, 0xa4506ceb, 0xbef9a3f7, 0xc67178f2};
    uint32_t w[64];
    for (int i = 0; i < 16; i++) w[i] = (uint32_t)p[4 * i] << 24 | (uint32_t)p[4 * i + 1] << 16 | (uint32_t)p[4 * i + 2] << 8 | p[4 * i + 3];
    for (int i = 16; i < 64; i++) {
      uint32_t s0 = ror(w[i - 15], 7) ^ ror(w[i - 15], 18) ^ (w[i - 15] >> 3);
      uint32_t s1 = ror(w[i - 2], 17) ^ ror(w[i - 2], 19) ^ (w[i - 2] >> 10);
      w[i] = w[i - 16] + s0 + w[i - 7] + s1;
    }
    uint32_t a = h[0], b = h[1], c = h[2], d = h[3], e = h[4], f = h[5], g = h[6], hh = h[7];
    for (int i = 0; i < 64; i++) {
      uint32_t t1 = hh + (ror(e, 6) ^ ror(e, 11) ^ ror(e, 25)) + ((e & f) ^ (~e & g)) + K[i] + w[i];
      uint32_t t2 = (ror(a, 2) ^ ror(a, 13) ^ ror(a, 22)) + ((a & b) ^ (a & c) ^ (b & c));
      hh = g; g = f; f = e; e = d + t1; d = c; c = b; b = a; a = t1 + t2;
    }
    h[0] += a; h[1] += b; h[2] += c; h[3] += d; h[4] += e; h[5] += f; h[6] += g; h[7] += hh;
  }
  void update(const uint8_t *p, size_t n) {
    len += n;
    while (n) {
      size_t k = 64 - fill < n ? 64 - fill : n;
      memcpy(buf + fill, p, k);
      fill += k; p += k; n -= k;
      if (fill == 64) { block(buf); fill = 0; }
    }
  }
  void final(uint8_t out[32]) {
    uint64_t bits = len * 8;
    uint8_t pad = 0x80;
    update(&pad, 1);
    uint8_t z = 0;
    while (fill != 56) update(&z, 1);
    uint8_t lb[8];
    for (int i = 0; i < 8; i++) lb[i] = (uint8_t)(bits >> (56 - 8 * i));
    update(lb, 8);
    for (int i = 0; i < 8; i++) { out[4 * i] = h[i] >> 24; out[4 * i + 1] = h[i] >> 16; out[4 * i + 2] = h[i] >> 8; out[4 * i + 3] = h[i]; }
  }
};

const char *const WASM_SHA256[4] = {
    "6faf23ddfd697bbb7e8e922577589c2c06486258968a5a14f96fb5a16091b142",
    "020bd11f289864c54c7d02cd05723dcf8323e31fa5c77d8700c618232685978e",
    "b982f960ebbfcabe957fe13857ea47adfeee30e18fbe05474e9b982eab187f46",
    "8d6317b72eab34d34e12dfd7bd310dce40f4190768669772f992a9510c441fca"};


uint64_t fnv1a64(const char *s) {
  uint64_t h = 0xCBF29CE484222325ull;
  for (; *s; ++s) { h ^= (uint8_t)*s; h *= 0x100000001B3ull; }
  return h;
}
const CircuitDesc CIRCUITS[4] = {
    {B3W_KIND_COMP, 24093, 28, 16, P_BN254, B3W_LAYOUT_0, B3W_LAYOUT_0_NRUNS, B3W_LDS_WORDS_COMP},
    {B3W_KIND_NOVA_O2, 23291, 32, 15, P_BN254, B3W_LAYOUT_1, B3W_LAYOUT_1_NRUNS, B3W_LDS_WORDS_NOVA_O2},
    {B3W_KIND_NOVA_O2, 23291, 32, 15, P_VESTA, B3W_LAYOUT_2, B3W_LAYOUT_2_NRUNS, B3W_LDS_WORDS_NOVA_O2},
    {B3W_KIND_NOVA_O1, 24614, 32, 15, P_BN254, B3W_LAYOUT_3, B3W_LAYOUT_3_NRUNS, B3W_LDS_WORDS_NOVA_O1},
};

bool atom_lds(int kind, uint32_t atom, uint32_t *word, int *width ) {
  if (atom < B3W_A_HG) { *word = atom; *width = 32; return true; }
  if (atom < B3W_A_NV) {
    const uint32_t k = (atom - B3W_A_HG) / 8, j = (atom - B3W_A_HG) % 8;
    static const uint32_t off[8] = {0, 0, 2, 2, 4, 5, 6, 7};
    *word = B3W_LDS_HG + 8 * k + off[j];
    *width = (j == B3W_HG_S1 || j == B3W_HG_S3) ? 64 : 32;
    return true;
  }
  if (kind == B3W_KIND_COMP) return false;
  const uint32_t i = atom - B3W_A_NV;
  if (i == NV_CHUNK_IDX) { *word = B3W_LDS_CHUNK_IDX; *width = 64; return true; }
  if (i < NV_NARROW_COUNT) { *word = B3W_LDS_NV + i; *width = 32; return true; }
  if (i >= NV_COUNT) return false;
  uint32_t j = i - NV_NARROW_COUNT;
  if (kind == B3W_KIND_NOVA_O2) {
    if (j < 3) {  }
    else if (i >= NV_EQ_INV && i < NV_EQ_INV + 64) j = 3 + (i - NV_EQ_INV);
    else return false;
  }
  *word = B3W_LDS_WIDE + 8 * j;
  *width = 256;
  return true;
}

void inv_small_host(uint32_t k, const uint32_t P[8], uint32_t out[8]) {
  uint64_t r = 0;
  for (int i = 7; i >= 0; --i) r = ((r << 32) | P[i]) % k;
  int64_t x0 = 0, x1 = 1;
  uint64_t a = k, b = r;
  while (b > 1) {
    const uint64_t q = a / b, tt = a - q * b;
    a = b; b = tt;
    const int64_t tx = x0 - (int64_t)q * x1;
    x0 = x1; x1 = tx;
  }
  int64_t x = x1 % (int64_t)k;
  if (x < 0) x += k;
  const uint64_t t = ((uint64_t)k - (uint64_t)x) % k;
  uint32_t prod[9];
  uint64_t carry = 1;
  for (int i = 0; i < 8; ++i) {
    const uint64_t cur = (uint64_t)P[i] * t + carry;
    prod[i] = (uint32_t)cur;
    carry = cur >> 32;
  }
  prod[8] = (uint32_t)carry;
  uint64_t rem = 0;
  for (int i = 8; i >= 0; --i) {
    const uint64_t cur = (rem << 32) | prod[i];
    const uint64_t qd = cur / k;
    rem = cur - qd * k;
    if (i < 8) out[i] = (uint32_t)qd;
  }
}
std::vector<uint32_t> build_nova_aux(const uint64_t *prime) {
  std::vector<uint32_t> aux(16 + 8 * B3W_INV_TABLE_N, 0);
  memcpy(aux.data(), prime, 32);
  aux[8] = B3W_INV_TABLE_N;
  for (uint32_t k = 1; k < B3W_INV_TABLE_N; ++k) inv_small_host(k, aux.data(), aux.data() + 16 + 8 * k);
  return aux;
}

bool build_slot_table(const CircuitDesc &c, std::vector<uint32_t> &table, std::string &err) {
  const uint32_t padded = ((c.nwit + 31) / 32 + 8) * 32;
  table.assign(padded, B3W_ENTRY(0, 31, B3W_MODE_BIT));
  std::vector<uint8_t> seen(c.nwit, 0);
  char msg[128];
  for (uint32_t r = 0; r < c.nruns; r++) {
    const b3w_layout_run &run = c.runs[r];
    for (uint32_t j = 0; j < run.len; j++) {
      const uint32_t slot = run.slot + j;
      if (slot >= c.nwit || seen[slot]) { err = "layout: bad or duplicate slot"; return false; }
      seen[slot] = 1;
      uint32_t word; int width;
      if (run.kind == 'W') {
        if (!atom_lds(c.kind, run.atom + j, &word, &width)) {
          snprintf(msg, sizeof msg, "layout: atom %u not staged for this circuit kind", run.atom + j);
          err = msg; return false;
        }
        table[slot] = B3W_ENTRY(word, 0, width == 32 ? B3W_MODE_W32 : width == 64 ? B3W_MODE_W64 : B3W_MODE_W256);
      } else {
        const uint32_t bit = run.bit0 + j;
        if (run.atom == B3W_A_NV + NV_CHUNK_IDX && bit == 64) {
          table[slot] = B3W_ENTRY(B3W_A_ONE, 31, B3W_MODE_BIT);
          continue;
        }
        if (!atom_lds(c.kind, run.atom, &word, &width) || (int)bit >= width || width == 256) {
          snprintf(msg, sizeof msg, "layout: bit %u of atom %u not expressible", bit, run.atom);
          err = msg; return false;
        }
        table[slot] = B3W_ENTRY(word + bit / 32, bit % 32, B3W_MODE_BIT);
      }
    }
  }
  for (uint32_t s = 0; s < c.nwit; s++) if (!seen[s]) { err = "layout: uncovered slot"; return false; }
  return true;
}

bool build_exact_table(const CircuitDesc &c, std::vector<uint32_t> &table) {
  table.assign(c.nwit, 0);
  for (uint32_t r = 0; r < c.nruns; r++) {
    const b3w_layout_run &run = c.runs[r];
    for (uint32_t j = 0; j < run.len; j++) {
      const uint32_t slot = run.slot + j;
      if (slot >= c.nwit) return false;
      if (run.kind == 'W') table[slot] = (run.atom + j) | (0xFFFFu << 16);
      else table[slot] = run.atom | ((run.bit0 + j) << 16);
    }
  }
  return true;
}

const char *reference_trace(int circuit, uint32_t site) {
  static const b3w_trace_entry *const T[4] = {B3W_TRACES_0, B3W_TRACES_1, B3W_TRACES_2, B3W_TRACES_3};
  static const uint32_t N[4] = {B3W_TRACES_0_N, B3W_TRACES_1_N, B3W_TRACES_2_N, B3W_TRACES_3_N};
  for (uint32_t i = 0; i < N[circuit]; i++) if (T[circuit][i].site == site) return T[circuit][i].text;
  return nullptr;
}

bool build_input_slots(const CircuitDesc &c, std::vector<uint32_t> &slots) {
  slots.assign(c.nin, 0xFFFFFFFFu);
  const uint32_t first = c.kind == B3W_KIND_COMP ? B3W_A_H : B3W_A_NV;
  for (uint32_t r = 0; r < c.nruns; r++) {
    const b3w_layout_run &run = c.runs[r];
    if (run.kind != 'W') continue;
    for (uint32_t j = 0; j < run.len; j++) {
      const uint32_t atom = run.atom + j;
      if (atom >= first && atom < first + c.nin && slots[atom - first] == 0xFFFFFFFFu) slots[atom - first] = run.slot + j;
    }
  }
  for (uint32_t v : slots) if (v == 0xFFFFFFFFu) return false;
  return true;
}

const char *assert_site_text(uint32_t site, char *buf, size_t len) {
  const uint32_t code = site & 0xFF, r = (site >> 8) & 0xF, g = (site >> 12) & 0xF, hf = (site >> 16) & 1;
  switch (code) {
    case 1: snprintf(buf, len, "Error in template Bits34 line: 201 (rounds[%u].GS[%u].half%u.add1)\n", r, g, hf + 1); break;
    case 2: snprintf(buf, len, "Error in template ToBits line: 153 (rounds[%u].GS[%u].half%u.rxor2.tb)\n", r, g, hf + 1); break;
    case 3: snprintf(buf, len, "Error in template Bits33 line: 176 (rounds[%u].GS[%u].half%u.add3)\n", r, g, hf + 1); break;
    case 4: snprintf(buf, len, "Error in template ToBits line: 153 (rounds[%u].GS[%u].half%u.rxor4.tb)\n", r, g, hf + 1); break;
    case 5: snprintf(buf, len, "Error in template ToBits line: 153 (outXor[%u].tb_x)\n", g + 8 * hf); break;
    case 6: snprintf(buf, len, "Error in template ToBits line: 153 (outXor[%u].tb_y)\n", g + 8 * hf); break;
    case 10: snprintf(buf, len, "Error in template Num2Bits line: 38 (check_depth.check_parent.n2b)\n"); break;
    case 11: snprintf(buf, len, "Error in template Num2Bits line: 38 (check_depth.exceed_depth.lt.n2b)\n"); break;
    case 12: snprintf(buf, len, "Error in template Blake3NovaTreePath_CheckDepth line: 38\n"); break;
    case 13: snprintf(buf, len, "Error in template Num2Bits line: 38 (final_m.down_left_path.n2b)\n"); break;
    case 14: snprintf(buf, len, "Error in template Blake3GetDownLeftPath line: 77\n"); break;
    default: snprintf(buf, len, "assert site %u\n", site);
  }
  return buf;
}

}

bool b3w_int_build_slot_table(const CircuitDesc &c, std::vector<uint32_t> &table, std::string &err) { return build_slot_table(c, table, err); }

namespace {
int32_t ensure_scratch(b3w_ctx *ctx) {
  if (ctx->d_scratch) return B3W_OK;
  ctx->scratch_cap = B3W_SWEEP_CHUNK;
  hipError_t e = hipMalloc((void **)&ctx->d_scratch, (size_t)ctx->scratch_cap * ctx->desc.lds_words * 4);
  if (e != hipSuccess) { ctx->scratch_cap = 0; return hip_fail(ctx, e, "hipMalloc(sweep scratch)"); }
  return B3W_OK;
}

void set_inputs(b3w_ctx *ctx) {
  struct Def { const char *name; uint32_t count; };
  static const Def comp[] = {{"h", 8}, {"m", 16}, {"t", 2}, {"b", 1}, {"d", 1}};
  static const Def nova[] = {{"n_blocks", 1}, {"block_count", 1}, {"h", 8}, {"chunk_idx_low", 1}, {"chunk_idx_high", 1},
                             {"leaf_depth", 1}, {"total_depth", 1}, {"depth", 1}, {"m", 16}, {"b", 1}};
  const Def *d = ctx->desc.kind == B3W_KIND_COMP ? comp : nova;
  const int nd = ctx->desc.kind == B3W_KIND_COMP ? 5 : 10;
  uint32_t off = 0;
  for (int i = 0; i < nd; i++) {
    ctx->inputs.push_back({d[i].name, d[i].count, off, fnv1a64(d[i].name)});
    off += d[i].count;
  }
}
}

int b3w_int_default_variant(const b3w_ctx *ctx, uint32_t n, const uint8_t *d_bodies, uint64_t pitch) {
  const bool comp = ctx->desc.kind == B3W_KIND_COMP, nova2 = ctx->desc.kind == B3W_KIND_NOVA_O2;
  const bool fillable = ctx->fill_ok && !(reinterpret_cast<uintptr_t>(d_bodies) & 31) && !(pitch & 31) && pitch < (1ull << 30) &&
                        (uint64_t)n * pitch + (1ull << 20) < (1ull << 37);
  if (fillable && comp && n >= 128 && (n <= 3072 || !b3w_place_is_mixed(d_bodies))) return B3W_VARIANT_REGIONFILL;
  if (fillable && nova2 && (b3w_place_is_mixed(d_bodies) ? n >= 768 && n <= 2560 : n >= 512)) return B3W_VARIANT_REGIONFILL;
  if (n <= 2560) return B3W_VARIANT_SLICED + (n <= (comp ? 32u : 8u) ? 64 : n <= 96 ? 32 : n <= 192 ? 16 : n <= 768 ? 8 : 4);
  if (comp) return n <= 6144 ? 0 : 8;
  if (nova2) return n <= 3072 ? 0 : n <= 32768 ? 3 : 4;
  return 0;
}

extern "C" {

uint32_t b3w_abi_version(void) { return (1u << 16) | 4u; }

int32_t b3w_identify_wasm(const uint8_t *code, size_t len) {
  if (!code) return B3W_CIRCUIT_UNKNOWN;
  Sha256 s;
  s.update(code, len);
  uint8_t dg[32];
  s.final(dg);
  char hex[65];
  for (int i = 0; i < 32; i++) snprintf(hex + 2 * i, 3, "%02x", dg[i]);
  for (int c = 0; c < 4; c++) if (!strcmp(hex, WASM_SHA256[c])) return c;
  return B3W_CIRCUIT_UNKNOWN;
}

int32_t b3w_create(int32_t circuit, int32_t device, b3w_ctx **out) {
  if (!out || circuit < 0 || circuit > 3) return B3W_E_BAD_ARGUMENT;
  *out = nullptr;
  int ndev = 0;
  if (hipGetDeviceCount(&ndev) != hipSuccess || ndev <= 0 || device < 0 || device >= ndev) return B3W_E_NO_DEVICE;
  b3w_ctx *ctx = new b3w_ctx;
  ctx->circuit = circuit;
  ctx->desc = CIRCUITS[circuit];
  ctx->device = device;
  set_inputs(ctx);
  std::vector<uint32_t> table;
  if (!build_slot_table(ctx->desc, table, ctx->last_error)) { delete ctx; return B3W_E_BAD_ARGUMENT; }
  std::vector<uint32_t> wide_slots(B3W_NOVA_ISZERO, 0xFFFFFFFFu);
  ctx->fill_ok = ctx->desc.kind == B3W_KIND_COMP || ctx->desc.kind == B3W_KIND_NOVA_O2;
  for (uint32_t i = 0; i < table.size(); i++) {
    const uint32_t e = table[i], src = e & 0xFFFu, sh = (e >> 12) & 31u, mode = (e >> 17) & 3u;
    if (mode != B3W_MODE_BIT && sh != 0) ctx->fill_ok = false;
    if (ctx->desc.kind == B3W_KIND_COMP) {
      if (src >= 1023 || mode == B3W_MODE_W256) ctx->fill_ok = false;
    } else if (mode == B3W_MODE_W256) {
      const uint32_t j = src >= B3W_LDS_WIDE && (src - B3W_LDS_WIDE) % 8 == 0 ? (src - B3W_LDS_WIDE) / 8 : 0xFFFFFFFFu;
      if (j >= B3W_NOVA_ISZERO || wide_slots[j] != 0xFFFFFFFFu) ctx->fill_ok = false; else wide_slots[j] = i;
    } else if (src + (mode == B3W_MODE_W64 ? 1u : 0u) >= B3W_LDS_WIDE) ctx->fill_ok = false;
  }
  if (ctx->desc.kind == B3W_KIND_NOVA_O2) {
    for (uint32_t v : wide_slots) if (v == 0xFFFFFFFFu) ctx->fill_ok = false;
    for (uint32_t j = 0; ctx->fill_ok && j < B3W_NOVA_ISZERO; j++) {
      if (j > 0 && wide_slots[j] <= wide_slots[j - 1]) ctx->fill_ok = false;
      for (int d = -3; ctx->fill_ok && d <= 3; d++) {
        const int64_t k = (int64_t)wide_slots[j] + d;
        if (k < 0 || k >= (int64_t)ctx->desc.nwit) continue;
        const uint32_t e = table[k], src = e & 0xFFFu, mode = (e >> 17) & 3u;
        if (mode != B3W_MODE_W256 && !((src >= B3W_A_H && src < B3W_A_O) || src >= B3W_LDS_NV)) ctx->fill_ok = false;
      }
    }
  }
  std::vector<uint16_t> ftab(table.size(), 0);
  std::vector<uint32_t> alias;
  if (ctx->fill_ok) {
    const bool nova = ctx->desc.kind != B3W_KIND_COMP;
    std::vector<uint8_t> used(4097, 0);
    for (uint32_t i = 0; i < ctx->desc.nwit; i++) {
      const uint32_t e = table[i], src = e & 0xFFFu, mode = (e >> 17) & 3u;
      if (mode == B3W_MODE_W256) continue;
      used[src] = 1;
      if (mode == B3W_MODE_W64) used[src + 1] = 1;
    }
    used[B3W_LDS_OKWORD] = used[B3W_LDS_OKWORD + 1] = 1;
    for (uint32_t k = 0; k < 16; k++) used[B3W_A_O + k] = 1;
    if (nova) for (uint32_t k : {NV_N_BLOCKS, NV_BLOCK_COUNT_OUT, NV_TOTAL_DEPTH, NV_DEPTH_OUT, NV_CIL, NV_CIH, NV_LEAF_DEPTH}) used[B3W_LDS_NV + k] = 1;
    for (uint32_t w = 2048; w < 4097; w++) if (used[w]) ctx->fill_ok = false;
    std::vector<uint16_t> to(2048, 0xFFFFu);
    uint32_t hole = B3W_LDS_HG;
    for (uint32_t w = 1024; w < 2048 && ctx->fill_ok; w++) {
      if (!used[w]) continue;
      while (hole < 1024 && used[hole]) hole++;
      if (hole >= 1024 || alias.size() >= B3W_ALIAS_MAX) { ctx->fill_ok = false; break; }
      used[hole] = 1; to[w] = (uint16_t)hole;
      alias.push_back(w | hole << 16);
    }
    for (uint32_t i = 0; i < table.size() && ctx->fill_ok; i++) {
      const uint32_t e = table[i], sh = (e >> 12) & 31u, mode = (e >> 17) & 3u;
      uint32_t src = e & 0xFFFu;
      if (mode == B3W_MODE_W256) { ftab[i] = (uint16_t)(0x8000u | 2u << 10); continue; }
      if (src >= 1024) {
        if (mode == B3W_MODE_W64 || src >= 2048 || to[src] == 0xFFFFu) { if (i < ctx->desc.nwit) ctx->fill_ok = false; continue; }
        src = to[src];
      }
      if (mode == B3W_MODE_W64 && src + 1 >= 1024) { ctx->fill_ok = false; continue; }
      ftab[i] = (uint16_t)(mode == B3W_MODE_BIT ? (src | sh << 10) : (src | (mode == B3W_MODE_W64 ? 1u : 0u) << 10 | 0x8000u));
    }
  }
  DeviceGuard guard(device);
  if (guard.err != hipSuccess) { delete ctx; return B3W_E_NO_DEVICE; }
  const CircuitDesc &d = ctx->desc;
  hipError_t e = hipMalloc((void **)&ctx->d_table_base, (table.size() + 32) * 4 + ftab.size() * 2);
  if (e == hipSuccess) e = hipMemset(ctx->d_table_base, 0, 32 * 4);
  if (e == hipSuccess) ctx->d_table = ctx->d_table_base + 32;
  if (e == hipSuccess) e = hipMemcpy(ctx->d_table, table.data(), table.size() * 4, hipMemcpyHostToDevice);
  if (e == hipSuccess) e = hipMemcpy(ctx->d_table + table.size(), ftab.data(), ftab.size() * 2, hipMemcpyHostToDevice);
  if (e == hipSuccess && d.kind != B3W_KIND_COMP) {
    std::vector<uint32_t> aux = build_nova_aux(d.prime);
    static_assert(B3W_AUX_WIDE_SLOTS == 16 + 8 * B3W_INV_TABLE_N, "b3w_kernels.h and b3w_internal.h disagree about the inverse table");
    aux.insert(aux.end(), wide_slots.begin(), wide_slots.end());
    if (ctx->fill_ok && d.kind == B3W_KIND_NOVA_O2) {
      aux.resize(B3W_AUX_LINE_LISTS + 2 * 4 * B3W_LINE_LIST_MAX, 0xFFFFFFFFu);
      for (uint32_t ph = 0; ph < 4; ph++) {
        uint32_t cnt = 0, last_line = 0xFFFFFFFFu;
        for (uint32_t j = 0; j < B3W_NOVA_ISZERO; j++) {
          const uint32_t line = (ph + wide_slots[j]) >> 2;
          if (line == last_line) continue;
          last_line = line;
          for (uint32_t i = 0; i < 4; i++) {
            const uint32_t k = line * 4 + i - ph;
            if (k >= d.nwit) continue;
// ... 295 lines not shown
```

hot-proofs-blake3-circom_amd/csrc/b3w_internal.h:

```cpp
#pragma once
#include <hip/hip_runtime_api.h>
#include <hip/hip_ext.h>
#include <errno.h>
#include <fcntl.h>
#include <stdint.h>
#include <stdio.h>
#include <stdlib.h>
#include <string.h>
#include <sys/uio.h>
#include <unistd.h>
#include <algorithm>
#include <array>
#include <chrono>
#include <atomic>
#include <map>
#include <mutex>
#include <thread>
#include <string>
#include <vector>

#include "../../include/b3wit.h"
#include "b3w_atoms.h"
#include "b3w_capture.h"
#include "b3w_kernels.h"
#include "b3w_r1cs_host.h"


struct b3w_layout_run { char kind; uint32_t slot, atom, bit0, len; };

struct InputSignal { const char *name; uint32_t count; uint32_t rec_off; uint64_t hash; };

struct CircuitDesc {
  int kind;
  uint32_t nwit, nin, npub;
  const uint64_t *prime;
  const b3w_layout_run *runs;
  uint32_t nruns;
  uint32_t lds_words;
};
inline constexpr uint64_t P_BN254[4] = {0x43e1f593f0000001ull, 0x2833e84879b97091ull, 0xb85045b68181585dull, 0x30644e72e131a029ull};
inline constexpr uint64_t P_VESTA[4] = {0x8c46eb2100000001ull, 0x224698fc0994a8ddull, 0x0ull, 0x4000000000000000ull};
constexpr uint32_t B3W_INV_TABLE_N = 2048;

struct b3w_ctx {
  int circuit = -1;
  CircuitDesc desc{};
  int device = -1;
  int variant = 0;
  bool variant_auto = true;
  bool fill_ok = false;
  bool variant_tuned = false;
  std::vector<InputSignal> inputs;
  uint32_t *d_table = nullptr;
  uint32_t *d_table_base = nullptr;
  void *d_aux = nullptr;
  uint32_t *d_scratch = nullptr;
  uint32_t *d_exact_table = nullptr;
  uint32_t *d_prime = nullptr;
  uint32_t *d_fe_inputs = nullptr;
  uint32_t *d_status2 = nullptr;
  uint32_t *d_in_slots = nullptr;
  uint32_t scratch_cap = 0;
  uint32_t *d_rec1 = nullptr;
  uint8_t *d_body1 = nullptr;
  int32_t *d_status1 = nullptr;
  float plain_ms_per_gb = 0;
  struct Spare { void *ptr; uint64_t bytes; int32_t placement; };
  std::vector<Spare> ring_spares;
  uint64_t *h_samples = nullptr, *d_samples = nullptr;
  uint32_t samples_cap = 0;
  hipEvent_t samples_done = nullptr;
  uint8_t *h_batch = nullptr, *d_batch = nullptr;
  uint64_t batch_cap = 0;
  hipEvent_t batch_done = nullptr;
  static constexpr uint32_t B3W_MANY_SLOTS = 8;
  struct ManySlot { uint8_t *h = nullptr, *d = nullptr; uint64_t cap = 0; hipEvent_t done = nullptr; bool busy = false; };
  ManySlot many_slots[B3W_MANY_SLOTS];
  uint32_t many_next = 0;
  std::string last_error;
};

struct b3w_batch {
  b3w_ctx *ctx = nullptr;
  uint32_t capacity = 0, n = 0;
  uint64_t pitch = 0;
  int32_t placement = B3W_PLACEMENT_PLAIN;
  uint32_t *d_recs = nullptr;
  uint8_t *d_bodies = nullptr;
  uint32_t *d_pub = nullptr;
  int32_t *d_status = nullptr;
};

inline int32_t hip_fail(b3w_ctx *ctx, hipError_t e, const char *what) {
  if (ctx) ctx->last_error = std::string(what) + ": " + hipGetErrorString(e);
  return B3W_E_HIP;
}
#define HIP_TRY(ctx, call)                                  \
  do {                                                      \
    hipError_t _e = (call);                                 \
    if (_e != hipSuccess) return hip_fail(ctx, _e, #call);  \
  } while (0)

struct DeviceGuard {
  int prev = -1;
  bool switched = false;
  hipError_t err = hipSuccess;
  explicit DeviceGuard(int dev) {
    err = hipGetDevice(&prev);
    if (err == hipSuccess && prev != dev) {
      err = hipSetDevice(dev);
      switched = err == hipSuccess;
    }
  }
  ~DeviceGuard() { if (switched) (void)hipSetDevice(prev); }
  DeviceGuard(const DeviceGuard &) = delete;
  DeviceGuard &operator=(const DeviceGuard &) = delete;
};
#define ON_DEVICE(ctx)                         \
  DeviceGuard _dev_guard((ctx)->device);       \
  if (_dev_guard.err != hipSuccess) return hip_fail(ctx, _dev_guard.err, "hipSetDevice")

bool b3w_int_build_slot_table(const CircuitDesc &c, std::vector<uint32_t> &table, std::string &err);
int b3w_int_default_variant(const b3w_ctx *ctx, uint32_t n, const uint8_t *d_bodies, uint64_t pitch);
b3w_ctx *b3w_int_key_ctx(const b3w_commit_key *key);
int32_t b3w_int_commit_records(b3w_ctx *ctx, const b3w_commit_key *key, const uint32_t *d_records, uint32_t n, uint8_t *d_points, uint32_t *d_public,
                               int32_t *d_status, void *stream, uint32_t *d_sums_out, void *trace_stream = nullptr, hipEvent_t trace_done = nullptr);
int32_t b3w_int_commit_normalize(b3w_ctx *ctx, const b3w_commit_key *key, const uint32_t *d_sums, uint64_t n, uint8_t *d_points, void *stream);
b3w_ctx *b3w_int_r1cs_ctx(const b3w_r1cs *r1cs);
constexpr uint64_t B3W_RING_SPARE_CAP = 26ull << 30;
```

hot-proofs-blake3-circom_amd/csrc/b3w_kernels.h:

```cpp
#pragma once
#include <hip/hip_runtime_api.h>
#include <stdint.h>

#define B3W_VARIANT_SWEEP 100
#define B3W_VARIANT_SLICED 20
#define B3W_VARIANT_REGIONFILL 200
#define B3W_VARIANT_REGIONFILL_LIGHT 201
#define B3W_REGIONFILL_GRID 256
#define B3W_AUX_WIDE_SLOTS (16 + 8 * 2048)
#define B3W_AUX_LINE_COUNTS (B3W_AUX_WIDE_SLOTS + 68)
#define B3W_AUX_LINE_LISTS (B3W_AUX_LINE_COUNTS + 4)
#define B3W_LINE_LIST_MAX 160
#define B3W_AUX_ALIAS_COUNT (B3W_AUX_LINE_LISTS + 2 * 4 * B3W_LINE_LIST_MAX)
#define B3W_AUX_ALIAS_LIST (B3W_AUX_ALIAS_COUNT + 1)
#define B3W_ALIAS_MAX 192
#define B3W_SWEEP_GRID 256
#define B3W_SWEEP_LOGC 13
#define B3W_SWEEP_CHUNK (1u << B3W_SWEEP_LOGC)

extern "C" int b3w_launch_batch(int kind, int variant, const uint32_t *d_recs, uint32_t n, uint8_t *d_out,
                                uint64_t pitch, const uint32_t *d_table, uint32_t nwit, uint32_t *d_pub,
                                int32_t *d_status, const void *d_aux, uint32_t *d_scratch, uint32_t scratch_cap,
                                hipStream_t stream);

extern "C" int b3w_launch_exact(int nova, const uint32_t *d_inputs, const uint32_t *d_prime, const uint32_t *d_table,
                                uint32_t nwit, uint8_t *d_out, uint32_t *d_status, hipStream_t stream);

extern "C" uint32_t b3w_plan_path_len(uint64_t chunk, uint64_t nchunks);
extern "C" int b3w_launch_plan_leaves(const uint8_t *d_pre, uint64_t total_len, uint64_t first_chunk, uint32_t nlocal,
                                      uint64_t nchunks, uint32_t *d_recs, uint32_t *d_chunk_cv, hipStream_t stream);
extern "C" int b3w_launch_plan_merge(const uint32_t *d_left, const uint32_t *d_right, uint32_t stride_words, uint64_t npairs,
                                     uint32_t root, uint32_t *d_parents, hipStream_t stream);
extern "C" int b3w_launch_plan_parents(const uint32_t *d_levels, uint64_t nchunks, uint64_t first_chunk, uint32_t nlocal,
                                       uint32_t last_chunk_blocks, uint32_t *d_recs, hipStream_t stream);
extern "C" uint32_t b3w_plan_tree_first_level(uint64_t nchunks);
extern "C" int b3w_launch_plan_tree(uint32_t *d_levels, uint64_t nchunks, uint32_t l0, uint32_t *d_root, uint64_t first_chunk, uint32_t plan_nlocal,
                                    uint32_t last_chunk_blocks, uint32_t *d_recs, hipStream_t stream);
extern "C" uint64_t b3w_plan_parent_row(uint64_t chunk, uint64_t nchunks);
extern "C" int b3w_plan_path_provable(uint64_t chunk, uint64_t nchunks);
extern "C" int b3w_launch_pack_hout(const uint32_t *d_pub, uint64_t row0, uint64_t count, uint32_t *d_dst, hipStream_t stream);
extern "C" int b3w_launch_unpack_hout(const uint32_t *d_gathered, uint64_t block_words, uint64_t par_off, const uint64_t *d_tab, uint32_t nranks,
                                      uint64_t max_rows, uint32_t *d_leaf_all, uint32_t *d_par_all, hipStream_t stream);

extern "C" int b3w_launch_trace(int kind, const uint32_t *d_recs, uint32_t cn, uint32_t *d_images, uint32_t row, const uint32_t *d_table,
                                uint32_t nwit, uint32_t *d_pub, int32_t *d_status, const void *d_aux, hipStream_t stream);
extern "C" int b3w_launch_verify(int kind, const uint32_t *d_in_slots, uint32_t n, const uint8_t *d_bodies, uint64_t pitch,
                                 const uint32_t *d_table, uint32_t nwit, uint32_t *d_mismatch, const void *d_aux,
                                 hipStream_t stream);

extern "C" int b3w_place_alloc(int device, uint64_t bytes, int want_mixed, void **out, int *mixed, float *rates);
extern "C" int b3w_place_free(void *ptr);
extern "C" int b3w_place_is_mixed(const void *ptr);
extern "C" void b3w_place_trim(void);
extern "C" void b3w_place_configure(int64_t search_gib, int64_t pool_gib);
extern "C" void b3w_place_stats(int device, uint64_t out[6]);
extern "C" void b3w_place_search_limit(double seconds);
extern "C" void b3w_place_search_stats(int device, double out[4]);
extern "C" void b3w_place_cost_breakdown(int device, double out[4]);
extern "C" int b3w_place_store_rate(uint8_t *buf, uint64_t pitch, uint32_t n, uint32_t body_bytes, int shape, uint32_t iters, hipStream_t stream, double *gbs);

#define B3W_COMMIT_WINDOW_SMALL 12
#define B3W_COMMIT_WINDOW_LARGE 16
#define B3W_COMMIT_WINDOW_XL 18
#define B3W_COMMIT_WINDOW_OK(w) ((w) == B3W_COMMIT_WINDOW_SMALL || (w) == B3W_COMMIT_WINDOW_LARGE || (w) == B3W_COMMIT_WINDOW_XL)
#define B3W_COMMIT_ENTRIES(W) ((1u << (W)) - 1u)
#define B3W_COMMIT_SUM_WORDS 36
struct B3wCurve {
  uint32_t p[8];
  uint32_t r2[8];
  uint32_t one[8];
  uint32_t pm2[8];
  uint32_t inv;
};
extern "C" int b3w_launch_commit_setup(const uint32_t *d_gens, const uint32_t *d_first_v, const uint32_t *d_nbits, uint32_t nslots,
                                       uint32_t *d_points, const B3wCurve *curve, hipStream_t stream);
extern "C" int b3w_launch_commit_windows(const uint32_t *d_points, uint32_t nwin, uint32_t window, uint32_t *d_table, const B3wCurve *curve, hipStream_t stream);
extern "C" int b3w_launch_commit(const uint8_t *d_bodies, uint32_t n, uint64_t pitch, uint32_t first_slot, uint32_t nslots,
                                 const uint32_t *d_slotdesc ,
                                 const uint32_t *d_images ,
                                 uint32_t img_row, const uint32_t *d_runs , uint32_t nruns,
                                 const uint32_t *d_table, uint32_t nwin, uint32_t window, uint32_t *d_sums, uint8_t *d_out,
                                 int32_t *d_status, const uint32_t *d_invtab , uint32_t inv_nk,
                                 const uint32_t *d_invmeta ,
                                 const uint32_t *d_aux ,
                                 unsigned long long *d_adds ,
                                 const B3wCurve *curve, hipStream_t stream);
extern "C" int b3w_launch_commit_normalize(const uint32_t *d_sums, uint64_t n, uint8_t *d_out, const B3wCurve *curve, hipStream_t stream);
#define B3W_NOVA_ISZERO 67
extern "C" int b3w_launch_commit_invtab(const uint32_t *d_gens, const uint32_t *d_inv_slot, const uint32_t *d_inverses, uint32_t njobs, uint32_t nk,
                                        uint32_t *d_invtab, const B3wCurve *curve, hipStream_t stream);

#include "b3w_r1cs_defs.h"
extern "C" int b3w_launch_r1cs(const uint8_t *d_bodies, uint32_t n, uint64_t pitch, uint32_t m, const uint32_t *d_rows,
                               const uint32_t *d_row_id, const uint32_t *d_wires, const uint16_t *d_cids, const uint32_t *d_coefR,
                               const B3wField *field, uint32_t *d_violations, uint32_t *d_first, hipStream_t stream);
struct B3wR1csSystem {
  uint32_t nwires, ntiles, max_ext, max_tile_terms, max_tile_rows, ncoef;
  const uint32_t *tiles, *tile_terms, *ext, *rows, *row_id, *row_k, *terms, *coefs;
  const long long *coef_small;
  const uint32_t *g_rows, *g_wires;
  const uint16_t *g_cids;
  uint32_t max_g_words, max_g_rows, smask_groups;
  const uint32_t *srows, *sgdesc, *sgwords, *sgmeta;
  const unsigned long long *smask;
  const unsigned long long *scost;
};
struct B3wWalk {
  uint32_t ntiles, exp_slots, max_gen, max_ent, ncoef, static_words, max_rows, signed_elems;
  const uint32_t *tile;
  const unsigned long long *mask;
  const uint16_t *exp;
  const uint4 *runs;
  const uint32_t *run_row, *ent_w, *ent_m, *row_id;
  const unsigned long long *stat;
  const long long *coef_small;
  const uint32_t *static_k, *static_id;
  uint32_t nstatic, pad2;
  uint32_t static_d0[4];
  uint32_t p[8];
};
extern "C" int b3w_launch_r1cs_walk(const uint8_t *d_bodies, uint32_t n, uint64_t pitch, const B3wWalk *walk, const B3wR1csSystem *sysw, const B3wField *field,
                                    unsigned long long *d_scratch, uint32_t *d_violations, uint32_t *d_first, hipStream_t stream);
extern "C" size_t b3w_r1cs_walk_scratch_bytes(const B3wWalk *walk);
#define B3W_R1CS_SLAB 8192u
extern "C" size_t b3w_r1cs_scratch_bytes(const B3wR1csSystem *sys);
extern "C" int b3w_launch_r1cs_stream(const uint8_t *d_bodies, uint32_t n, uint64_t pitch, const B3wR1csSystem *sys, const B3wField *field,
                                      unsigned long long *d_scratch, uint32_t *d_violations, uint32_t *d_first, hipStream_t stream);
```

include/b3wit.h:

```cpp
#ifndef B3WIT_H
#define B3WIT_H
#include <stddef.h>
#include <stdint.h>

#ifdef __cplusplus
extern "C" {
#endif

#define B3W_CIRCUIT_COMPRESSION_BN254 0
#define B3W_CIRCUIT_NOVA_BN254        1
#define B3W_CIRCUIT_NOVA_VESTA        2
#define B3W_CIRCUIT_NOVA_BN254_O1     3
#define B3W_CIRCUIT_UNKNOWN         (-1)

#define B3W_OK                     0
#define B3W_E_SIGNAL_NOT_FOUND     1
#define B3W_E_TOO_MANY_SIGNALS     2
#define B3W_E_SIGNAL_ALREADY_SET   3
#define B3W_E_ASSERT_FAILED        4
#define B3W_E_NOT_ENOUGH_MEMORY    5
#define B3W_E_ARRAY_ACCESS         6
#define B3W_E_BAD_ARGUMENT       100
#define B3W_E_NO_DEVICE          101
#define B3W_E_HIP                102
// ... 9 lines not shown
int32_t b3w_identify_wasm(const uint8_t *code, size_t len);

int32_t b3w_create(int32_t circuit, int32_t device, b3w_ctx **out);
void b3w_destroy(b3w_ctx *ctx);

int32_t b3w_info(const b3w_ctx *ctx, uint32_t *n32, uint8_t prime_le[32], uint32_t *witness_size,
                 uint32_t *input_size, uint32_t version[3]);

int32_t b3w_input_signal_size(const b3w_ctx *ctx, uint64_t fnv1a64_of_name);

int32_t b3w_calc_witness(b3w_ctx *ctx, const uint64_t *name_hashes, const uint32_t *counts,
                         const uint8_t *values_le32, uint32_t nkeys, uint8_t *out_body);

int32_t b3w_write_wtns_header(const b3w_ctx *ctx, uint8_t out[76]);

int32_t b3w_last_error(const b3w_ctx *ctx, char *buf, size_t len);


int32_t b3w_batch_run_device(b3w_ctx *ctx, const uint32_t *d_records, uint32_t n, uint8_t *d_bodies,
                             uint64_t pitch, uint32_t *d_public, int32_t *d_status, void *stream);

uint32_t b3w_public_words(const b3w_ctx *ctx);

int32_t b3w_batch_alloc(b3w_ctx *ctx, uint32_t capacity, uint64_t pitch , b3w_batch **out);
void b3w_batch_free(b3w_batch *batch);
int32_t b3w_batch_run(b3w_batch *batch, const uint32_t *host_records, uint32_t n, void *stream);
int32_t b3w_batch_outputs(b3w_batch *batch, uint32_t *host_public, int32_t *host_status);
int32_t b3w_batch_fetch(b3w_batch *batch, uint32_t index, uint8_t *out_body);
void *b3w_batch_device_ptr(b3w_batch *batch, uint64_t *pitch);

#define B3W_PLACEMENT_PLAIN 0
#define B3W_PLACEMENT_MIXED 1
#define B3W_PLACEMENT_INTERLEAVED 2
int32_t b3w_bodies_alloc(b3w_ctx *ctx, uint64_t bytes, void **d_ptr, int32_t *placement);
int32_t b3w_bodies_free(b3w_ctx *ctx, void *d_ptr);
void b3w_bodies_trim(void);
int32_t b3w_ctx_trim(b3w_ctx *ctx);
void b3w_bodies_configure(int64_t search_gib, int64_t pool_gib);
void b3w_bodies_search_limit(double seconds);
int32_t b3w_bodies_search_stats(const b3w_ctx *ctx, double out[5]);
int32_t b3w_bodies_search_breakdown(const b3w_ctx *ctx, double out[4]);
int32_t b3w_bodies_store_rate(b3w_ctx *ctx, void *d_bodies, uint32_t n, uint64_t pitch, int32_t shape, uint32_t iters, void *stream,
                              double *gb_per_s);
int32_t b3w_bodies_stats(const b3w_ctx *ctx, uint64_t out[6]);
int32_t b3w_batch_placement(const b3w_batch *batch);

int32_t b3w_batch_time_device(b3w_ctx *ctx, const uint32_t *d_records, uint32_t n, uint8_t *d_bodies,
                              uint64_t pitch, uint32_t *d_public, int32_t *d_status, void *stream,
                              uint32_t iters, float *avg_ms);

typedef struct b3w_r1cs b3w_r1cs;
int32_t b3w_r1cs_create(b3w_ctx *ctx, const uint8_t *r1cs_image, size_t len, b3w_r1cs **out);
int32_t b3w_r1cs_info(const b3w_r1cs *r1cs, uint32_t *n_constraints, uint32_t *n_wires, uint64_t *n_terms,
                      uint32_t *n_pub_out, uint32_t *n_pub_in, uint32_t *n_prv_in);
int32_t b3w_r1cs_is_tiled(const b3w_r1cs *r1cs);
void b3w_r1cs_destroy(b3w_r1cs *r1cs);
int32_t b3w_r1cs_check_device(b3w_ctx *ctx, const b3w_r1cs *r1cs, const uint8_t *d_bodies, uint32_t n, uint64_t pitch,
                              uint32_t *d_violations, uint32_t *d_first, void *stream);
int32_t b3w_batch_r1cs_check(b3w_batch *batch, const b3w_r1cs *r1cs, uint32_t *host_violations, uint32_t *host_first);
typedef struct {
  b3w_ctx *ctx;
  const b3w_r1cs *r1cs;
  uint32_t *d_violations;
  void (*next)(void *user, const uint8_t *d_bodies, uint64_t pitch, uint64_t first_step, uint32_t count, void *stream);
  void *next_user;
  int32_t error;
} b3w_r1cs_sink;
void b3w_r1cs_consumer(void *user, const uint8_t *d_bodies, uint64_t pitch, uint64_t first_step, uint32_t count, void *stream);

int32_t b3w_batch_verify_device(b3w_ctx *ctx, const uint8_t *d_bodies, uint32_t n, uint64_t pitch, uint32_t *d_mismatch,
                                void *stream);

#define B3W_CURVE_BN254_G1 0
#define B3W_CURVE_PALLAS   1
#define B3W_CURVE_VESTA    B3W_CURVE_PALLAS
typedef struct b3w_commit_key b3w_commit_key;
int32_t b3w_commit_key_create(b3w_ctx *ctx, int32_t curve, uint32_t first_slot, const uint8_t *host_generators, b3w_commit_key **out);
int32_t b3w_commit_key_create_ex(b3w_ctx *ctx, int32_t curve, uint32_t first_slot, const uint8_t *host_generators, uint32_t window_bits,
                                 b3w_commit_key **out);
int32_t b3w_commit_key_create_folded(b3w_ctx *ctx, int32_t curve, uint32_t first_slot, const uint8_t *host_generators,
                                     const uint8_t *folded , uint32_t window_bits,
                                     b3w_commit_key **out);
int32_t b3w_slot_widths(b3w_ctx *ctx, uint16_t *out_bits );
uint32_t b3w_commit_key_window(const b3w_commit_key *key);
int32_t b3w_commit_key_count(b3w_commit_key *key, int32_t on);
int32_t b3w_commit_key_counts(const b3w_commit_key *key, uint64_t out[2]);
void b3w_commit_key_destroy(b3w_commit_key *key);
int32_t b3w_batch_commit_device(b3w_ctx *ctx, const b3w_commit_key *key, const uint8_t *d_bodies, uint32_t n, uint64_t pitch,
                                uint8_t *d_points , int32_t *d_status, void *stream);
int32_t b3w_batch_commit(b3w_batch *batch, const b3w_commit_key *key, uint8_t *host_points, int32_t *host_status);

int32_t b3w_commit_records_device(b3w_ctx *ctx, const b3w_commit_key *key, const uint32_t *d_records, uint32_t n, uint8_t *d_points,
                                  uint32_t *d_public, int32_t *d_status, void *stream);

int32_t b3w_commit_records(b3w_ctx *ctx, const b3w_commit_key *key, const uint32_t *host_records, uint32_t n, uint8_t *host_points,
                           uint32_t *host_public, int32_t *host_status);

typedef struct {
  b3w_ctx *ctx;
  const b3w_commit_key *key;
  uint8_t *d_points;
  int32_t *d_status;
  int32_t error;
} b3w_commit_sink;
void b3w_commit_consumer(void *user, const uint8_t *d_bodies, uint64_t pitch, uint64_t first_step, uint32_t count, void *stream);

int32_t b3w_batch_verify(b3w_batch *batch, uint32_t *host_mismatch);

int32_t b3w_batch_write_wtns(b3w_batch *batch, uint32_t first, uint32_t count, const char *dir, const char *prefix,
                             uint32_t *written);
int32_t b3w_batch_write_wtns_ex(b3w_batch *batch, uint32_t first, uint32_t count, const char *dir, const char *prefix,
                                uint32_t threads, uint32_t *written);

int32_t b3w_batch_autotune_device(b3w_ctx *ctx, const uint32_t *d_records, uint32_t n, uint8_t *d_bodies,
                                  uint64_t pitch, uint32_t *d_public, int32_t *d_status, void *stream,
                                  int32_t *chosen_variant, float *chosen_ms);

uint64_t b3w_chain_num_chunks(uint64_t preimage_len);
uint64_t b3w_chain_num_leaf_steps(uint64_t preimage_len);
uint32_t b3w_chain_path_len(uint64_t chunk, uint64_t n_chunks);

int32_t b3w_chain_plan_leaves_device(b3w_ctx *ctx, const uint8_t *d_preimage, uint64_t preimage_len, uint64_t first_chunk,
                                     uint32_t n_chunks_local, uint32_t *d_records, uint32_t *d_chunk_cvs, void *stream);

int32_t b3w_chain_tree_device(b3w_ctx *ctx, uint32_t *d_levels, uint64_t n_chunks, uint32_t *d_root, void *stream);

uint64_t b3w_chain_num_parent_steps(uint64_t preimage_len, uint64_t first_chunk, uint64_t n_chunks_local);
uint64_t b3w_chain_parent_row(uint64_t chunk, uint64_t n_chunks);
int32_t b3w_chain_path_provable(uint64_t chunk, uint64_t n_chunks);
int32_t b3w_chain_plan_parents_device(b3w_ctx *ctx, const uint32_t *d_levels, uint64_t n_chunks, uint64_t preimage_len,
                                      uint64_t first_chunk, uint32_t n_chunks_local, uint32_t *d_records, void *stream);

typedef struct b3w_comm b3w_comm;
#define B3W_COMM_ID_BYTES 128
int32_t b3w_comm_unique_id(uint8_t id[B3W_COMM_ID_BYTES]);
int32_t b3w_comm_create(b3w_ctx *ctx, const uint8_t id[B3W_COMM_ID_BYTES], int32_t rank, int32_t nranks, b3w_comm **out);
typedef int32_t (*b3w_allgather_fn)(void *user, const void *d_send, void *d_recv, uint64_t bytes_per_rank, void *stream);
int32_t b3w_comm_create_host(b3w_ctx *ctx, const char *name, int32_t rank, int32_t nranks, b3w_comm **out);
int32_t b3w_comm_create_external(b3w_ctx *ctx, int32_t rank, int32_t nranks, b3w_allgather_fn allgather, void *user, b3w_comm **out);
int32_t b3w_comm_rank(const b3w_comm *comm);
int32_t b3w_comm_size(const b3w_comm *comm);
void b3w_comm_destroy(b3w_comm *comm);
int32_t b3w_comm_allgather(b3w_comm *comm, const void *d_send, void *d_recv, uint64_t bytes_per_rank, void *stream);
int32_t b3w_batch_allgather_public(b3w_batch *batch, b3w_comm *comm, uint32_t *host_all);

typedef struct b3w_chain b3w_chain;
typedef void (*b3w_batch_consumer)(void *user, const uint8_t *d_bodies, uint64_t pitch, uint64_t first_step, uint32_t count,
                                   void *stream);
int32_t b3w_chain_create(b3w_ctx *ctx, uint64_t preimage_len, uint64_t first_chunk, uint32_t n_chunks_local,
                         uint32_t batch_steps, uint32_t ring, int32_t with_parents, b3w_chain **out);
void b3w_chain_destroy(b3w_chain *chain);
int32_t b3w_chain_commit_only(b3w_chain *chain, const b3w_commit_key *key, uint8_t *d_points);
int32_t b3w_chain_commit_from_records(b3w_chain *chain, const b3w_commit_key *key, uint8_t *d_points);
#define B3W_COMMIT_OVERLAP_AUTO   (-1)
#define B3W_COMMIT_OVERLAP_SERIAL 0
#define B3W_COMMIT_OVERLAP_FREE   1
#define B3W_COMMIT_OVERLAP_GATED  2
int32_t b3w_chain_commit_overlap(b3w_chain *chain, int32_t mode);
int32_t b3w_chain_commitments(b3w_chain *chain, uint8_t *host_points, void *stream);
int32_t b3w_chain_check_constraints(b3w_chain *chain, const b3w_r1cs *r1cs);
int32_t b3w_chain_violations(b3w_chain *chain, uint32_t *host_violations, void *stream);
uint32_t *b3w_chain_violations_device(b3w_chain *chain);
int32_t b3w_chain_run_leaves(b3w_chain *chain, const uint8_t *host_preimage ,
                             b3w_batch_consumer consumer, void *user, void *stream);
int32_t b3w_chain_run_parents(b3w_chain *chain, const uint32_t *d_all_chunk_cvs , b3w_batch_consumer consumer, void *user, void *stream);
void b3w_chain_shard(uint64_t n_chunks, int32_t rank, int32_t nranks, uint64_t *first_chunk, uint32_t *n_chunks_local);
// ... 149 lines not shown
```

integrations/rust/b3wit_ffi.rs:

```rust
use std::ffi::c_void;
use std::os::raw::c_char;

#[link(name = "b3wit")]
extern "C" {
    fn b3w_create(circuit: i32, device: i32, out: *mut *mut c_void) -> i32;
    fn b3w_destroy(ctx: *mut c_void);
    fn b3w_info(ctx: *const c_void, n32: *mut u32, prime_le: *mut u8, witness_size: *mut u32,
                input_size: *mut u32, version: *mut u32) -> i32;
    fn b3w_calc_witness(ctx: *mut c_void, name_hashes: *const u64, counts: *const u32,
                        values_le32: *const u8, nkeys: u32, out_body: *mut u8) -> i32;
    fn b3w_last_error(ctx: *const c_void, buf: *mut c_char, len: usize) -> i32;
}

pub const CIRCUIT_NOVA_BN254: i32 = 1;
pub const CIRCUIT_NOVA_VESTA: i32 = 2;
pub const CURVE_BN254_G1: i32 = 0;
pub const CURVE_PALLAS: i32 = 1;

pub fn fnv1a64(name: &str) -> u64 {
    let mut h: u64 = 0xCBF29CE484222325;
    for b in name.bytes() {
        h ^= b as u64;
        h = h.wrapping_mul(0x100000001B3);
    }
    h
}

pub struct Calculator { ctx: *mut c_void, witness_size: usize }

impl Calculator {
    pub fn new(circuit: i32, device: i32) -> Result<Self, i32> {
        let mut ctx = std::ptr::null_mut();
        let rc = unsafe { b3w_create(circuit, device, &mut ctx) };
        if rc != 0 { return Err(rc); }
        let mut nwit = 0u32;
        unsafe { b3w_info(ctx, std::ptr::null_mut(), std::ptr::null_mut(), &mut nwit, std::ptr::null_mut(), std::ptr::null_mut()) };
        Ok(Calculator { ctx, witness_size: nwit as usize })
    }

    pub fn calculate_witness(&mut self, input: &[(String, Vec<[u8; 32]>)]) -> Result<Vec<[u8; 32]>, String> {
        let hashes: Vec<u64> = input.iter().map(|(k, _)| fnv1a64(k)).collect();
        let counts: Vec<u32> = input.iter().map(|(_, v)| v.len() as u32).collect();
        let values: Vec<u8> = input.iter().flat_map(|(_, v)| v.iter().flat_map(|x| x.iter().copied())).collect();
        let mut body = vec![0u8; self.witness_size * 32];
        let rc = unsafe {
            b3w_calc_witness(self.ctx, hashes.as_ptr(), counts.as_ptr(), values.as_ptr(), input.len() as u32, body.as_mut_ptr())
        };
        if rc != 0 {
            let mut buf = vec![0 as c_char; 1024];
            unsafe { b3w_last_error(self.ctx, buf.as_mut_ptr(), buf.len()) };
            let msg = unsafe { std::ffi::CStr::from_ptr(buf.as_ptr()) }.to_string_lossy().into_owned();
            return Err(format!("status {}: {}", rc, msg));
        }
        Ok(body.chunks_exact(32).map(|c| { let mut a = [0u8; 32]; a.copy_from_slice(c); a }).collect())
    }
}

impl Drop for Calculator {
    fn drop(&mut self) { unsafe { b3w_destroy(self.ctx) } }
}


pub type BatchConsumer = extern "C" fn(user: *mut c_void, d_bodies: *const u8, pitch: u64, first_step: u64, count: u32, stream: *mut c_void);
pub type AllgatherFn = extern "C" fn(user: *mut c_void, d_send: *const c_void, d_recv: *mut c_void, bytes_per_rank: u64, stream: *mut c_void) -> i32;

#[link(name = "b3wit")]
extern "C" {
    pub fn b3w_chain_create(ctx: *mut c_void, preimage_len: u64, first_chunk: u64, n_chunks_local: u32, batch_steps: u32,
                            ring: u32, with_parents: i32, out: *mut *mut c_void) -> i32;
    pub fn b3w_chain_destroy(chain: *mut c_void);
    pub fn b3w_chain_run_leaves(chain: *mut c_void, host_preimage: *const u8,
                                consumer: Option<extern "C" fn(*mut c_void, *const u8, u64, u64, u32, *mut c_void)>,
                                user: *mut c_void, stream: *mut c_void) -> i32;
    pub fn b3w_chain_run_parents(chain: *mut c_void, d_all_chunk_cvs: *const u32,
                                 consumer: Option<extern "C" fn(*mut c_void, *const u8, u64, u64, u32, *mut c_void)>,
                                 user: *mut c_void, stream: *mut c_void) -> i32;
    pub fn b3w_chain_info(chain: *const c_void, n_leaf_steps: *mut u64, n_parent_steps: *mut u64, n_chunks: *mut u64, path_len: *mut u32,
                          placement: *mut i32) -> i32;
    pub fn b3w_chain_outputs(chain: *mut c_void, host_public: *mut u32, host_status: *mut i32, host_root: *mut u32,
                             stream: *mut c_void) -> i32;
    pub fn b3w_chain_shard(n_chunks: u64, rank: i32, nranks: i32, first_chunk: *mut u64, n_chunks_local: *mut u32);
    pub fn b3w_chain_num_chunks(preimage_len: u64) -> u64;
    pub fn b3w_chain_num_leaf_steps(preimage_len: u64) -> u64;
    pub fn b3w_chain_parent_row(chunk: u64, n_chunks: u64) -> u64;
    pub fn b3w_chain_run_parents_sharded(chain: *mut c_void, comm: *mut c_void,
                                         consumer: Option<extern "C" fn(*mut c_void, *const u8, u64, u64, u32, *mut c_void)>,
                                         user: *mut c_void, stream: *mut c_void) -> i32;
    pub fn b3w_chain_allgather_hout(chain: *mut c_void, comm: *mut c_void, d_leaf_hout: *mut u32, d_parent_hout: *mut u32,
                                    stream: *mut c_void) -> i32;
    pub fn b3w_chain_allgather_hout_host(chain: *mut c_void, comm: *mut c_void, host_leaf_hout: *mut u32, host_parent_hout: *mut u32,
                                         stream: *mut c_void) -> i32;
    pub fn b3w_comm_unique_id(id: *mut u8) -> i32;
    pub fn b3w_comm_create(ctx: *mut c_void, id: *const u8, rank: i32, nranks: i32, out: *mut *mut c_void) -> i32;
    pub fn b3w_comm_create_host(ctx: *mut c_void, name: *const c_char, rank: i32, nranks: i32, out: *mut *mut c_void) -> i32;
    pub fn b3w_comm_create_external(ctx: *mut c_void, rank: i32, nranks: i32,
                                    allgather: Option<extern "C" fn(*mut c_void, *const c_void, *mut c_void, u64, *mut c_void) -> i32>,
                                    user: *mut c_void, out: *mut *mut c_void) -> i32;
    pub fn b3w_comm_destroy(comm: *mut c_void);
    pub fn b3w_commit_key_create_ex(ctx: *mut c_void, curve: i32, first_slot: u32, host_generators: *const u8, window_bits: u32,
                                    out: *mut *mut c_void) -> i32;
    pub fn b3w_commit_key_destroy(key: *mut c_void);
    pub fn b3w_commit_records(ctx: *mut c_void, key: *const c_void, host_records: *const u32, n: u32, host_points: *mut u8,
                              host_public: *mut u32, host_status: *mut i32) -> i32;
    pub fn b3w_chain_commit_only(chain: *mut c_void, key: *const c_void, d_points: *mut u8) -> i32;
    pub fn b3w_chain_commitments(chain: *mut c_void, host_points: *mut u8, stream: *mut c_void) -> i32;
    pub fn b3w_chain_commit_from_records(chain: *mut c_void, key: *const c_void, d_points: *mut u8) -> i32;
    pub fn b3w_chain_commit_overlap(chain: *mut c_void, mode: i32) -> i32;
    pub fn b3w_chain_check_constraints(chain: *mut c_void, r1cs: *const c_void) -> i32;
    pub fn b3w_chain_violations(chain: *mut c_void, host_violations: *mut u32, stream: *mut c_void) -> i32;
}

pub struct FoldOutputs { pub public: Vec<u32>, pub status: Vec<i32>, pub root: [u32; 8], pub n_leaf_steps: u64, pub n_parent_steps: u64 }

pub struct Fold { chain: *mut c_void }

impl Fold {
    pub fn new(calc: &Calculator, preimage_len: u64, batch_steps: u32, ring: u32) -> Result<Self, i32> {
        let mut chain = std::ptr::null_mut();
        let n = unsafe { b3w_chain_num_chunks(preimage_len) };
        let rc = unsafe { b3w_chain_create(calc.ctx, preimage_len, 0, n as u32, batch_steps, ring, 1, &mut chain) };
        if rc != 0 { Err(rc) } else { Ok(Fold { chain }) }
    }

    pub fn commit_only(&mut self, key: *const c_void) -> Result<(), i32> {
        let rc = unsafe { b3w_chain_commit_only(self.chain, key, std::ptr::null_mut()) };
        if rc != 0 { Err(rc) } else { Ok(()) }
    }

    pub fn fold_shaped(&mut self, key: *const c_void, r1cs: *const c_void, overlap: i32) -> Result<(), i32> {
        let mut rc = unsafe { b3w_chain_check_constraints(self.chain, r1cs) };
        if rc == 0 { rc = unsafe { b3w_chain_commit_overlap(self.chain, overlap) }; }
        if rc == 0 { rc = unsafe { b3w_chain_commit_from_records(self.chain, key, std::ptr::null_mut()) }; }
        if rc != 0 { Err(rc) } else { Ok(()) }
    }

    pub fn violations(&mut self) -> Result<Vec<u32>, i32> {
        let mut v = vec![0u32; self.steps()?];
        let rc = unsafe { b3w_chain_violations(self.chain, v.as_mut_ptr(), std::ptr::null_mut()) };
        if rc != 0 { Err(rc) } else { Ok(v) }
    }

    fn steps(&self) -> Result<usize, i32> {
        let (mut nl, mut np, mut nc, mut pl, mut place) = (0u64, 0u64, 0u64, 0u32, 0i32);
        let rc = unsafe { b3w_chain_info(self.chain, &mut nl, &mut np, &mut nc, &mut pl, &mut place) };
        if rc != 0 { Err(rc) } else { Ok((nl + np) as usize) }
    }

    pub fn run(&mut self, preimage: &[u8], consumer: Option<BatchConsumer>, user: *mut c_void) -> Result<FoldOutputs, i32> {
        let stream = std::ptr::null_mut();
        let mut rc = unsafe { b3w_chain_run_leaves(self.chain, preimage.as_ptr(), consumer, user, stream) };
        if rc == 0 { rc = unsafe { b3w_chain_run_parents(self.chain, std::ptr::null(), consumer, user, stream) }; }
        if rc != 0 { return Err(rc); }
        let (mut nl, mut np, mut nc, mut pl, mut place) = (0u64, 0u64, 0u64, 0u32, 0i32);
        unsafe { b3w_chain_info(self.chain, &mut nl, &mut np, &mut nc, &mut pl, &mut place) };
        let rows = (nl + np) as usize;
        let mut out = FoldOutputs { public: vec![0u32; rows * 15], status: vec![0i32; rows], root: [0u32; 8], n_leaf_steps: nl, n_parent_steps: np };
        rc = unsafe { b3w_chain_outputs(self.chain, out.public.as_mut_ptr(), out.status.as_mut_ptr(), out.root.as_mut_ptr(), stream) };
        if rc != 0 { Err(rc) } else { Ok(out) }
    }

    pub fn commitments(&mut self) -> Result<Vec<u8>, i32> {
        let mut pts = vec![0u8; self.steps()? * 64];
        let rc = unsafe { b3w_chain_commitments(self.chain, pts.as_mut_ptr(), std::ptr::null_mut()) };
        if rc != 0 { Err(rc) } else { Ok(pts) }
    }
}

impl Drop for Fold {
    fn drop(&mut self) { unsafe { b3w_chain_destroy(self.chain) } }
}
```

Before: 9.346 million.

## Add merged commit key that pre-sums generators of equivalent witness slots

Adds a merged commitment key type. It groups witness slots into classes, and a new GPU kernel pre-adds their generator points into one virtual generator per class, so record-based commitments do fewer scalar multiplications. The Python CommitKey now builds the merged key lazily and uses it for record and chain commitments, while keeping a plain key for body commits. It also moves the slot-table code into its own file. This touches commitment paths only, not the witness-compression path being measured, and adds a second key allocation plus extra setup cost.

```diff
diff --git a/hot-proofs-blake3-circom_amd/__init__.py b/hot-proofs-blake3-circom_amd/__init__.py
--- a/hot-proofs-blake3-circom_amd/__init__.py
+++ b/hot-proofs-blake3-circom_amd/__init__.py
@@ -106,6 +106,8 @@
         "b3w_commit_key_create": (i32, [vp, i32, u32, vp, ctypes.POINTER(vp)]),
         "b3w_commit_key_create_ex": (i32, [vp, i32, u32, vp, u32, ctypes.POINTER(vp)]),
         "b3w_commit_key_create_folded": (i32, [vp, i32, u32, vp, vp, u32, ctypes.POINTER(vp)]),
+        "b3w_commit_key_create_merged": (i32, [vp, i32, u32, vp, vp, u32, ctypes.POINTER(vp)]),
+        "b3w_commit_key_virtual_slots": (u32, [vp]),
         "b3w_slot_widths": (i32, [vp, vp]),
         "b3w_commit_key_window": (u32, [vp]),
         "b3w_commit_key_destroy": (None, [vp]),
@@ -215,7 +217,7 @@
                     "b3w_r1cs_create", "b3w_r1cs_info", "b3w_r1cs_is_tiled", "b3w_r1cs_destroy", "b3w_r1cs_check_device", "b3w_batch_r1cs_check", "b3w_r1cs_consumer", "b3w_batch_write_wtns", "b3w_batch_write_wtns_ex", "b3w_batch_autotune_device", "b3w_bodies_alloc", "b3w_bodies_free", "b3w_bodies_trim", "b3w_ctx_trim", "b3w_bodies_configure", "b3w_bodies_stats", "b3w_bodies_search_stats", "b3w_bodies_search_limit", "b3w_bodies_search_breakdown", "b3w_bodies_store_rate", "b3w_batch_placement", "b3w_chain_num_chunks", "b3w_chain_num_leaf_steps", "b3w_chain_path_len",
                     "b3w_chain_num_parent_steps", "b3w_chain_parent_row", "b3w_chain_path_provable",
                     "b3w_chain_plan_leaves_device", "b3w_chain_tree_device", "b3w_chain_plan_parents_device",
-                    "b3w_commit_key_create", "b3w_commit_key_create_ex", "b3w_commit_key_create_folded", "b3w_slot_widths", "b3w_commit_key_window", "b3w_commit_key_destroy", "b3w_commit_key_count", "b3w_commit_key_counts", "b3w_commit_records_device", "b3w_commit_records", "b3w_chain_commit_only", "b3w_chain_commit_from_records", "b3w_chain_commit_overlap", "b3w_chain_violations_device", "b3w_chain_commitments", "b3w_chain_check_constraints", "b3w_chain_violations", "b3w_batch_commit_device", "b3w_batch_commit", "b3w_commit_consumer",
+                    "b3w_commit_key_create", "b3w_commit_key_create_ex", "b3w_commit_key_create_folded", "b3w_commit_key_create_merged", "b3w_commit_key_virtual_slots", "b3w_slot_widths", "b3w_commit_key_window", "b3w_commit_key_destroy", "b3w_commit_key_count", "b3w_commit_key_counts", "b3w_commit_records_device", "b3w_commit_records", "b3w_chain_commit_only", "b3w_chain_commit_from_records", "b3w_chain_commit_overlap", "b3w_chain_violations_device", "b3w_chain_commitments", "b3w_chain_check_constraints", "b3w_chain_violations", "b3w_batch_commit_device", "b3w_batch_commit", "b3w_commit_consumer",
                     "b3w_comm_unique_id", "b3w_comm_create", "b3w_comm_create_host", "b3w_comm_create_external", "b3w_comm_rank", "b3w_comm_size", "b3w_comm_destroy", "b3w_comm_allgather", "b3w_batch_allgather_public",
                     "b3w_chain_create", "b3w_chain_destroy", "b3w_chain_run_leaves", "b3w_chain_run_parents", "b3w_chain_shard", "b3w_chain_run_parents_sharded", "b3w_chain_allgather_hout", "b3w_chain_allgather_hout_host", "b3w_chain_exchange_ms", "b3w_chain_info",
                     "b3w_chain_outputs", "b3w_chain_records", "b3w_chain_public", "b3w_chain_status", "b3w_chain_local_cvs", "b3w_chain_root",
@@ -565,7 +567,7 @@
 class CommitKey:
     CURVES = {"bn254_g1": 0, "pallas": 1, "vesta": 1}
 
-    def __init__(self, ctx, curve, generators, first_slot=0, window=0, fold=None):
+    def __init__(self, ctx, curve, generators, first_slot=0, window=0, fold=None, merge=True):
         self.ctx = ctx
         buf = bytes(generators)
         nslots = ctx.witness_size - first_slot
@@ -577,13 +579,47 @@
             image = read_r1cs_image(BUILTIN_R1CS[ctx.circuit]) if fold is True else read_r1cs_image(fold)
             buf, mask, self.fold_stats = _fold.fold_generators(image, ctx.slot_widths(), first_slot, buf, curve)
             self.folded_slots = sum(1 for v in mask if v)
+        self._args = (self.CURVES[curve], first_slot, buf, bytes(mask) if mask is not None else None, window)
+        self.merge = bool(merge)
+        self._plain = self._merged = None
+        self._counting = False
+        if not self.merge:
+            self._plain = self._create(False)
+        elif window:
+            self._merged = self._create(True)
+
+    def _create(self, merged):
+        curve, first_slot, buf, mask, window = self._args
+        name = "b3w_commit_key_create_merged" if merged else "b3w_commit_key_create_folded"
         h = ctypes.c_void_p()
-        rc = lib().b3w_commit_key_create_folded(ctx.handle, self.CURVES[curve], first_slot, buf, bytes(mask) if mask is not None else None, window,
-                                                ctypes.byref(h))
-        if rc != B3W_OK:
-            raise B3WError(rc, f"b3w_commit_key_create_folded: status {rc}: {ctx.last_error()}")
-        self.handle = h
-        self.window = lib().b3w_commit_key_window(h)
+        rc = getattr(lib(), name)(self.ctx.handle, curve, first_slot, buf, mask, window, ctypes.byref(h))
+        if rc != B3W_OK:
+            raise B3WError(rc, f"{name}: status {rc}: {self.ctx.last_error()}")
+        if self._counting:
+            lib().b3w_commit_key_count(h, 1)
+        return h
+
+    @property
+    def handle(self):
+        if self._plain is None:
+            if self._args is None:
+                return None
+            self._plain = self._create(False)
+        return self._plain
+
+    @property
+    def records_handle(self):
+        if not self.merge:
+            return self.handle
+        if self._merged is None:
+            if self._args is None:
+                return None
+            self._merged = self._create(True)
+        return self._merged
+
+    @property
+    def window(self):
+        return lib().b3w_commit_key_window(self._merged if self._merged is not None else self.handle)
 
     def commit_device(self, d_bodies, n, pitch, d_points, d_status=0, stream=0):
         rc = lib().b3w_batch_commit_device(self.ctx.handle, self.handle, d_bodies, n, pitch, d_points, d_status or None, stream or None)
@@ -591,7 +627,7 @@
             raise B3WError(rc, f"b3w_batch_commit_device: status {rc}: {self.ctx.last_error()}")
 
     def commit_records_device(self, d_records, n, d_points, d_status, d_public=0, stream=0):
-        rc = lib().b3w_commit_records_device(self.ctx.handle, self.handle, d_records, n, d_points, d_public or None, d_status, stream or None)
+        rc = lib().b3w_commit_records_device(self.ctx.handle, self.records_handle, d_records, n, d_points, d_public or None, d_status, stream or None)
         if rc != B3W_OK:
             raise B3WError(rc, f"b3w_commit_records_device: status {rc}: {self.ctx.last_error()}")
 
@@ -601,23 +637,33 @@
         pts = np.zeros((n, 64), dtype=np.uint8)
         pub = np.zeros((n, self.ctx.public_words), dtype=np.uint32)
         st = np.zeros(n, dtype=np.int32)
-        rc = lib().b3w_commit_records(self.ctx.handle, self.handle, recs.ctypes.data, n, pts.ctypes.data, pub.ctypes.data, st.ctypes.data)
+        rc = lib().b3w_commit_records(self.ctx.handle, self.records_handle, recs.ctypes.data, n, pts.ctypes.data, pub.ctypes.data, st.ctypes.data)
         if rc != B3W_OK:
             raise B3WError(rc, f"b3w_commit_records: status {rc}: {self.ctx.last_error()}")
         return pts, pub, st
 
     def count(self, on=True):
-        lib().b3w_commit_key_count(self.handle, 1 if on else 0)
+        self._counting = bool(on)
+        for h in (self._plain, self._merged):
+            if h is not None:
+                lib().b3w_commit_key_count(h, 1 if on else 0)
 
     def counts(self):
-        out = (ctypes.c_uint64 * 2)()
-        lib().b3w_commit_key_counts(self.handle, out)
-        return int(out[0]), int(out[1])
+        adds = wits = 0
+        for h in (self._plain, self._merged):
+            if h is not None:
+                out = (ctypes.c_uint64 * 2)()
+                lib().b3w_commit_key_counts(h, out)
+                adds, wits = adds + int(out[0]), wits + int(out[1])
+        return adds, wits
 
     def close(self):
-        if getattr(self, "handle", None):
-            lib().b3w_commit_key_destroy(self.handle)
-            self.handle = None
+        for name in ("_plain", "_merged"):
+            h = getattr(self, name, None)
+            if h is not None:
+                setattr(self, name, None)
+                lib().b3w_commit_key_destroy(h)
+        self._args = None
 
     def __del__(self):
         try:
diff --git a/hot-proofs-blake3-circom_amd/build.py b/hot-proofs-blake3-circom_amd/build.py
--- a/hot-proofs-blake3-circom_amd/build.py
+++ b/hot-proofs-blake3-circom_amd/build.py
@@ -30,7 +30,7 @@
 def build_lib(force=False, extra_flags=()):
     from concurrent.futures import ThreadPoolExecutor
     names = ("b3w_kernels.hip", "b3w_exact.hip", "b3w_plan.hip", "b3w_bao.hip", "b3w_placement.hip", "b3w_commit.hip", "b3w_r1cs.hip", "b3w_r1cs_walk.hip", "b3w_r1cs_host.cpp", "b3w_hostcomm.cpp",
-             "b3w_ctx.cpp", "b3w_bodies.cpp", "b3w_wtns.cpp", "b3w_r1cs_api.cpp", "b3w_commit_api.cpp", "b3w_comm.cpp", "b3w_chain.cpp")
+             "b3w_ctx.cpp", "b3w_slot_table.cpp", "b3w_bodies.cpp", "b3w_wtns.cpp", "b3w_r1cs_api.cpp", "b3w_commit_api.cpp", "b3w_commit_merge.cpp", "b3w_comm.cpp", "b3w_chain.cpp")
     srcs = [os.path.join(CSRC, f) for f in names]
     hdrs = [os.path.join(CSRC, f) for f in sorted(os.listdir(CSRC)) if f.endswith((".h", ".inc"))] + \
         [os.path.join(ROOT, "include", "b3wit.h")]
diff --git a/hot-proofs-blake3-circom_amd/chain.py b/hot-proofs-blake3-circom_amd/chain.py
--- a/hot-proofs-blake3-circom_amd/chain.py
+++ b/hot-proofs-blake3-circom_amd/chain.py
@@ -89,9 +89,9 @@
     L.b3w_chain_info(h, ctypes.byref(nleaf), ctypes.byref(npar), ctypes.byref(nch), ctypes.byref(P), ctypes.byref(pl))
     n_leaf, n_par = nleaf.value, npar.value
     if commit_only is not None:
-        _chk(ctx, L.b3w_chain_commit_only(h, commit_only[0].handle, commit_only[1].data_ptr()), "b3w_chain_commit_only")
+        _chk(ctx, L.b3w_chain_commit_only(h, commit_only[0].records_handle, commit_only[1].data_ptr()), "b3w_chain_commit_only")
     elif commit_records is not None:
-        _chk(ctx, L.b3w_chain_commit_from_records(h, commit_records[0].handle, commit_records[1].data_ptr()), "b3w_chain_commit_from_records")
+        _chk(ctx, L.b3w_chain_commit_from_records(h, commit_records[0].records_handle, commit_records[1].data_ptr()), "b3w_chain_commit_from_records")
     else:
         _chk(ctx, L.b3w_chain_commit_only(h, None, None), "b3w_chain_commit_only")
     if commit_records is not None:
diff --git a/hot-proofs-blake3-circom_amd/csrc/b3w_commit.hip b/hot-proofs-blake3-circom_amd/csrc/b3w_commit.hip
--- a/hot-proofs-blake3-circom_amd/csrc/b3w_commit.hip
+++ b/hot-proofs-blake3-circom_amd/csrc/b3w_commit.hip
@@ -549,6 +549,37 @@
 #pragma unroll 1
       for (int i = 0; i < 64; ++i) P = jac_dbl(P, C);
   }
+}
+
+__global__ __launch_bounds__(64) void b3w_commit_merge_kernel(const uint32_t *__restrict__ points, const uint32_t *__restrict__ class_start,
+                                                              const uint32_t *__restrict__ members, const uint32_t *__restrict__ class_v,
+                                                              uint32_t nclass, uint32_t *__restrict__ merged, uint32_t *__restrict__ inf, B3wCurve C,
+                                                              B3wCurve9 C9) {
+  const uint32_t c = blockIdx.x * 64 + threadIdx.x;
+  if (c >= nclass) return;
+  const uint32_t b = class_start[c], e = class_start[c + 1], o = class_v ? class_v[c] : c;
+  if (e - b == 1) {
+    inf[c] = 0;
+    if (o == 0xFFFFFFFFu) return;
+    const uint32_t *pt = points + (uint64_t)members[b] * 16;
+    store_fp(merged + (uint64_t)o * 16, load_fp(pt));
+    store_fp(merged + (uint64_t)o * 16 + 8, load_fp(pt + 8));
+    return;
+  }
+  J9 acc = j9_infinity();
+#pragma unroll 1
+  for (uint32_t i = b; i < e; ++i) {
+    const uint32_t *pt = points + (uint64_t)members[i] * 16;
+    j9_madd(acc, to29(load_fp(pt)), to29(load_fp(pt + 8)), C9);
+  }
+  inf[c] = acc.inf ? 1u : 0u;
+  if (acc.inf || o == 0xFFFFFFFFu) return;
+  const F9 ia = inv29(mul29(acc.ZZ, acc.ZZZ, C9), C.pm2, C9);
+  uint32_t hi;
+  Fp x = from29(mul29(acc.X, mul29(ia, acc.ZZZ, C9), C9), hi); x = fp_reduce_once(x, hi, C);
+  Fp y = from29(mul29(acc.Y, mul29(ia, acc.ZZ, C9), C9), hi); y = fp_reduce_once(y, hi, C);
+  store_fp(merged + (uint64_t)o * 16, x);
+  store_fp(merged + (uint64_t)o * 16 + 8, y);
 }
 
 __global__ __launch_bounds__(64) void b3w_commit_invtab_kernel(const uint32_t *__restrict__ gens ,
@@ -1016,6 +1047,15 @@
   return (int)hipGetLastError();
 }
 
+extern "C" int b3w_launch_commit_merge(const uint32_t *d_points, const uint32_t *d_class_start, const uint32_t *d_members, const uint32_t *d_class_v,
+                                       uint32_t nclass, uint32_t *d_merged, uint32_t *d_inf, const B3wCurve *curve, hipStream_t stream) {
+  if (!nclass) return 0;
+  const B3wCurve9 c9 = make_curve9(*curve);
+  hipLaunchKernelGGL(b3w_commit_merge_kernel, dim3((nclass + 63) / 64), dim3(64), 0, stream, d_points, d_class_start, d_members, d_class_v, nclass, d_merged,
+                     d_inf, *curve, c9);
+  return (int)hipGetLastError();
+}
+
 extern "C" int b3w_launch_commit_windows(const uint32_t *d_points, uint32_t nwin, uint32_t window, uint32_t *d_table, const B3wCurve *curve, hipStream_t stream) {
   if (!nwin) return 0;
   if (!B3W_COMMIT_WINDOW_OK(window)) return (int)hipErrorInvalidValue;
diff --git a/hot-proofs-blake3-circom_amd/csrc/b3w_commit_api.cpp b/hot-proofs-blake3-circom_amd/csrc/b3w_commit_api.cpp
--- a/hot-proofs-blake3-circom_amd/csrc/b3w_commit_api.cpp
+++ b/hot-proofs-blake3-circom_amd/csrc/b3w_commit_api.cpp
@@ -1,10 +1,13 @@
 #include "b3w_internal.h"
+#include "b3w_commit_merge.h"
 
 
 struct b3w_commit_key {
   b3w_ctx *ctx = nullptr;
   B3wCurve curve{};
   uint32_t first_slot = 0, nwin = 0, window = 0;
+  uint32_t nvirt = 0;
+  bool merged = false;
   uint32_t nslots = 0;
   uint32_t *d_slotdesc = nullptr;
   uint32_t *d_runs = nullptr; uint32_t nruns = 0;
@@ -48,6 +51,10 @@
 }
 const uint64_t Q_BN254[4] = {0x3c208c16d87cfd47ull, 0x97816a916871ca8dull, 0xb85045b68181585dull, 0x30644e72e131a029ull};
 const uint64_t P_VESTA_BASE[4] = {0x992d30ed00000001ull, 0x224698fc094cf91bull, 0x0ull, 0x4000000000000000ull};
+int32_t merged_key_refused(b3w_ctx *ctx) {
+  ctx->last_error = "commit: a merged key (b3w_commit_key_create_merged) commits from records only";
+  return B3W_E_BAD_ARGUMENT;
+}
 }
 
 extern "C" {
@@ -74,27 +81,39 @@
   return B3W_OK;
 }
 
-static int32_t commit_key_create_once(b3w_ctx *ctx, int32_t curve, uint32_t first_slot, const uint8_t *host_generators,
-                                      const uint8_t *folded, uint32_t window_bits, b3w_commit_key **out, uint32_t *auto_window, hipError_t *herr);
-
-int32_t b3w_commit_key_create_folded(b3w_ctx *ctx, int32_t curve, uint32_t first_slot, const uint8_t *host_generators,
-                                     const uint8_t *folded , uint32_t window_bits, b3w_commit_key **out) {
+static int32_t commit_key_create_once(b3w_ctx *ctx, int32_t curve, uint32_t first_slot, const uint8_t *host_generators, const uint8_t *folded,
+                                      bool merge, uint32_t window_bits, b3w_commit_key **out, uint32_t *auto_window, hipError_t *herr);
+
+static int32_t commit_key_create_any(b3w_ctx *ctx, int32_t curve, uint32_t first_slot, const uint8_t *host_generators, const uint8_t *folded,
+                                     bool merge, uint32_t window_bits, b3w_commit_key **out) {
   uint32_t chosen = 0;
   hipError_t herr = hipSuccess;
-  int32_t rc = commit_key_create_once(ctx, curve, first_slot, host_generators, folded, window_bits, out, &chosen, &herr);
+  int32_t rc = commit_key_create_once(ctx, curve, first_slot, host_generators, folded, merge, window_bits, out, &chosen, &herr);
   while (rc == B3W_E_HIP && herr == hipErrorOutOfMemory && chosen > B3W_COMMIT_WINDOW_SMALL) {
     (void)hipGetLastError();
     const uint32_t narrower = chosen == B3W_COMMIT_WINDOW_XL ? B3W_COMMIT_WINDOW_LARGE : B3W_COMMIT_WINDOW_SMALL;
     uint32_t ignored = 0;
     herr = hipSuccess;
-    rc = commit_key_create_once(ctx, curve, first_slot, host_generators, folded, narrower, out, &ignored, &herr);
+    rc = commit_key_create_once(ctx, curve, first_slot, host_generators, folded, merge, narrower, out, &ignored, &herr);
     chosen = narrower;
   }
   return rc;
 }
 
-static int32_t commit_key_create_once(b3w_ctx *ctx, int32_t curve, uint32_t first_slot, const uint8_t *host_generators,
-                                      const uint8_t *folded, uint32_t window_bits, b3w_commit_key **out, uint32_t *auto_window, hipError_t *herr) {
+int32_t b3w_commit_key_create_folded(b3w_ctx *ctx, int32_t curve, uint32_t first_slot, const uint8_t *host_generators,
+                                     const uint8_t *folded , uint32_t window_bits, b3w_commit_key **out) {
+  return commit_key_create_any(ctx, curve, first_slot, host_generators, folded, false, window_bits, out);
+}
+
+int32_t b3w_commit_key_create_merged(b3w_ctx *ctx, int32_t curve, uint32_t first_slot, const uint8_t *host_generators,
+                                     const uint8_t *folded , uint32_t window_bits, b3w_commit_key **out) {
+  return commit_key_create_any(ctx, curve, first_slot, host_generators, folded, true, window_bits, out);
+}
+
+uint32_t b3w_commit_key_virtual_slots(const b3w_commit_key *key) { return key ? key->nvirt : 0; }
+
+static int32_t commit_key_create_once(b3w_ctx *ctx, int32_t curve, uint32_t first_slot, const uint8_t *host_generators, const uint8_t *folded,
+                                      bool merge, uint32_t window_bits, b3w_commit_key **out, uint32_t *auto_window, hipError_t *herr) {
   if (!ctx || !out || !host_generators || (curve != B3W_CURVE_BN254_G1 && curve != B3W_CURVE_VESTA) || first_slot >= ctx->desc.nwit ||
       (window_bits != 0 && !B3W_COMMIT_WINDOW_OK(window_bits))) {
     if (ctx) ctx->last_error = "commit key: curve 0/1, first_slot < witness_size, window_bits 0 (auto), 12, 16 or 18";
@@ -104,18 +123,15 @@
   std::vector<uint32_t> table;
   if (!b3w_int_build_slot_table(ctx->desc, table, ctx->last_error)) return B3W_E_BAD_ARGUMENT;
   const uint32_t nslots = ctx->desc.nwit - first_slot;
-  std::vector<uint32_t> nbits(nslots), first_v(nslots);
-  uint64_t nv = 0;
-  for (uint32_t i = 0; i < nslots; i++) {
-    const uint32_t mode = (table[first_slot + i] >> 17) & 3u;
-    nbits[i] = mode == B3W_MODE_BIT ? 1u : mode == B3W_MODE_W32 ? 32u : mode == B3W_MODE_W64 ? 64u : 256u;
-    if (folded && folded[i] == 1) nbits[i] = 0;
-    else if (folded && (folded[i] & 0x80)) {
-      if (mode != B3W_MODE_W32 || (folded[i] & 0x60)) { ctx->last_error = "commit key: a single-bit fold needs a 32-bit slot and a bit below 32"; return B3W_E_BAD_ARGUMENT; }
-      nbits[i] = 1;
-    } else if (folded && folded[i]) { ctx->last_error = "commit key: folded[] holds 0, 1 or 0x80 | bit"; return B3W_E_BAD_ARGUMENT; }
-    first_v[i] = (uint32_t)nv;
-    nv += nbits[i];
+  B3wCommitBits bits;
+  if (!b3w_commit_bits(table.data() + first_slot, nslots, folded, bits, ctx->last_error)) return B3W_E_BAD_ARGUMENT;
+  const std::vector<uint32_t> &nbits = bits.nbits, &first_v = bits.first_v;
+  B3wCommitMerge classes;
+  std::vector<uint32_t> merged_runs, class_v;
+  uint64_t nv = bits.nv;
+  if (merge) {
+    b3w_commit_merge_classes(bits.runs, classes);
+    nv = b3w_commit_merge_runs(classes, nullptr, merged_runs, class_v);
   }
   DeviceGuard guard(ctx->device);
   hipError_t e = guard.err;
@@ -134,15 +150,13 @@
                                                                            : B3W_COMMIT_WINDOW_SMALL;
     *auto_window = window;
   }
-  const uint32_t V0 = (uint32_t)nv;
-  nv = (nv + window - 1) / window * window;
   b3w_commit_key *key = new b3w_commit_key;
   key->ctx = ctx;
   key->curve = make_curve(curve == B3W_CURVE_BN254_G1 ? Q_BN254 : P_VESTA_BASE);
   key->first_slot = first_slot;
   key->window = window;
-  key->nwin = (uint32_t)(nv / window);
   key->nslots = nslots;
+  key->merged = merge;
   uint32_t *d_gens = nullptr, *d_first = nullptr, *d_nbits = nullptr, *d_points = nullptr;
   std::vector<uint32_t> desc(nslots);
   auto one_bit_of_word = [&](uint32_t i) { return folded && (folded[i] & 0x80) != 0; };
@@ -171,38 +185,11 @@
         if (inputs_found) desc[invmeta[j]] = j | 5u << 24;
       }
   }
-  std::vector<uint32_t> runs;
-  for (uint32_t i = 0; i < nslots; i++) {
-    const uint32_t ent = table[first_slot + i], src = ent & 0xFFFu, sh = (ent >> 12) & 31u, v0 = first_v[i];
-    if (nbits[i] == 0) continue;
-    if (one_bit_of_word(i)) {
-      runs.push_back(v0 | 0u << 24); runs.push_back(src | (sh + (folded[i] & 31u)) << 16);
-      continue;
-    }
-    if (nbits[i] == 1) {
-      if (!runs.empty()) {
-        const uint32_t a = runs[runs.size() - 2], b = runs[runs.size() - 1];
-        const uint32_t plen = (a >> 24) + 1, pv = a & 0xFFFFFFu, psrc = b & 0xFFFFu, psh = b >> 16;
-        if ((a >> 31) == 0 && psrc == src && psh + plen == sh && pv + plen == v0 && plen < 32 && i > 0 && nbits[i - 1] == 1) {
-          runs[runs.size() - 2] = pv | plen << 24;
-          continue;
-        }
-      }
-      runs.push_back(v0 | 0u << 24); runs.push_back(src | sh << 16);
-    } else {
-      const uint32_t words = nbits[i] / 32;
-      for (uint32_t k = 0; k < words; k++) {
-        runs.push_back((v0 + 32 * k) | 31u << 24); runs.push_back((src + k) | ((k == 0 || k == 4) ? sh : 0u) << 16);
-      }
-    }
-  }
-  key->nruns = (uint32_t)(runs.size() / 2);
-  if (e == hipSuccess) e = hipMalloc((void **)&key->d_runs, runs.size() * 4);
-  if (e == hipSuccess) e = hipMemcpy(key->d_runs, runs.data(), runs.size() * 4, hipMemcpyHostToDevice);
-  if (e == hipSuccess) e = hipMalloc((void **)&key->d_slotdesc, (size_t)nslots * 4);
-  if (e == hipSuccess) e = hipMemcpy(key->d_slotdesc, desc.data(), (size_t)nslots * 4, hipMemcpyHostToDevice);
-  if (e == hipSuccess) e = hipMalloc((void **)&key->d_table, (size_t)key->nwin * B3W_COMMIT_ENTRIES(window) * 64);
-  if (e == hipSuccess) e = hipMalloc((void **)&d_points, (size_t)nv * 64);
+  uint32_t *d_class_start = nullptr, *d_members = nullptr, *d_class_v = nullptr, *d_inf = nullptr, *d_merged = nullptr;
+  if (e == hipSuccess && !merge) e = hipMalloc((void **)&key->d_slotdesc, (size_t)nslots * 4);
+  if (e == hipSuccess && !merge) e = hipMemcpy(key->d_slotdesc, desc.data(), (size_t)nslots * 4, hipMemcpyHostToDevice);
+  const uint64_t plain_padded = ((uint64_t)bits.nv + window - 1) / window * window;
+  if (e == hipSuccess) e = hipMalloc((void **)&d_points, (size_t)std::max<uint64_t>(plain_padded, 1) * 64);
   if (e == hipSuccess) e = hipMalloc((void **)&d_gens, (size_t)nslots * 64);
   if (e == hipSuccess) e = hipMalloc((void **)&d_first, (size_t)nslots * 4);
   if (e == hipSuccess) e = hipMalloc((void **)&d_nbits, (size_t)nslots * 4);
@@ -210,9 +197,40 @@
   if (e == hipSuccess) e = hipMemcpy(d_first, first_v.data(), (size_t)nslots * 4, hipMemcpyHostToDevice);
   if (e == hipSuccess) e = hipMemcpy(d_nbits, nbits.data(), (size_t)nslots * 4, hipMemcpyHostToDevice);
   int rc = e == hipSuccess ? b3w_launch_commit_setup(d_gens, d_first, d_nbits, nslots, d_points, &key->curve, nullptr) : 0;
+  uint32_t *d_string = d_points;
+  if (merge && e == hipSuccess && rc == 0) {
+    const uint32_t nclass = (uint32_t)classes.class_key.size();
+    const uint64_t room = (nv + window - 1) / window * window;
+    e = hipMalloc((void **)&d_merged, (size_t)std::max<uint64_t>(room, 1) * 64);
+    if (e == hipSuccess) e = hipMalloc((void **)&d_class_start, classes.class_start.size() * 4);
+    if (e == hipSuccess) e = hipMalloc((void **)&d_members, std::max<size_t>(classes.members.size(), 1) * 4);
+    if (e == hipSuccess) e = hipMalloc((void **)&d_inf, std::max<size_t>(nclass, 1) * 4);
+    if (e == hipSuccess) e = hipMemcpy(d_class_start, classes.class_start.data(), classes.class_start.size() * 4, hipMemcpyHostToDevice);
+    if (e == hipSuccess) e = hipMemcpy(d_members, classes.members.data(), classes.members.size() * 4, hipMemcpyHostToDevice);
+    if (e == hipSuccess) rc = b3w_launch_commit_merge(d_points, d_class_start, d_members, nullptr, nclass, d_merged, d_inf, &key->curve, nullptr);
+    std::vector<uint32_t> inf(nclass, 0);
+    if (e == hipSuccess && rc == 0) e = hipMemcpy(inf.data(), d_inf, (size_t)nclass * 4, hipMemcpyDeviceToHost);
+    if (e == hipSuccess && rc == 0 && std::find(inf.begin(), inf.end(), 1u) != inf.end()) {
+      std::vector<uint8_t> dropped(inf.begin(), inf.end());
+      nv = b3w_commit_merge_runs(classes, dropped.data(), merged_runs, class_v);
+      e = hipMalloc((void **)&d_class_v, (size_t)nclass * 4);
+      if (e == hipSuccess) e = hipMemcpy(d_class_v, class_v.data(), (size_t)nclass * 4, hipMemcpyHostToDevice);
+      if (e == hipSuccess) rc = b3w_launch_commit_merge(d_points, d_class_start, d_members, d_class_v, nclass, d_merged, d_inf, &key->curve, nullptr);
+    }
+    d_string = d_merged;
+  }
+  const uint32_t V0 = (uint32_t)nv;
+  nv = (nv + window - 1) / window * window;
+  key->nvirt = V0;
+  key->nwin = (uint32_t)(nv / window);
+  const std::vector<uint32_t> &runs = merge ? merged_runs : bits.runs;
+  key->nruns = (uint32_t)(runs.size() / 2);
+  if (e == hipSuccess) e = hipMalloc((void **)&key->d_runs, std::max<size_t>(runs.size(), 2) * 4);
+  if (e == hipSuccess) e = hipMemcpy(key->d_runs, runs.data(), runs.size() * 4, hipMemcpyHostToDevice);
+  if (e == hipSuccess) e = hipMalloc((void **)&key->d_table, std::max<size_t>((size_t)key->nwin * B3W_COMMIT_ENTRIES(window) * 64, 64));
   for (uint32_t v = V0; v < nv && e == hipSuccess && rc == 0; v++)
-    e = hipMemcpyAsync(d_points + (size_t)v * 16, d_points, 64, hipMemcpyDeviceToDevice, nullptr);
-  if (e == hipSuccess && rc == 0) rc = b3w_launch_commit_windows(d_points, key->nwin, key->window, key->d_table, &key->curve, nullptr);
+    e = hipMemcpyAsync(d_string + (size_t)v * 16, d_string, 64, hipMemcpyDeviceToDevice, nullptr);
+  if (e == hipSuccess && rc == 0) rc = b3w_launch_commit_windows(d_string, key->nwin, key->window, key->d_table, &key->curve, nullptr);
   if (e == hipSuccess && rc == 0 && with_invtab) {
     key->inv_nk = B3W_INV_TABLE_N - 1;
     e = hipMalloc((void **)&key->d_invmeta, invmeta.size() * 4);
@@ -227,6 +245,11 @@
   if (d_first) (void)hipFree(d_first);
   if (d_nbits) (void)hipFree(d_nbits);
   if (d_points) (void)hipFree(d_points);
+  if (d_merged) (void)hipFree(d_merged);
+  if (d_class_start) (void)hipFree(d_class_start);
+  if (d_members) (void)hipFree(d_members);
+  if (d_class_v) (void)hipFree(d_class_v);
+  if (d_inf) (void)hipFree(d_inf);
   if (e != hipSuccess || rc != 0) {
     b3w_commit_key_destroy(key);
     *herr = e != hipSuccess ? e : (hipError_t)rc;
@@ -279,6 +302,7 @@
 int32_t b3w_batch_commit_device(b3w_ctx *ctx, const b3w_commit_key *key, const uint8_t *d_bodies, uint32_t n, uint64_t pitch,
                                 uint8_t *d_points, int32_t *d_status, void *stream) {
   if (!ctx || !key || key->ctx != ctx || !d_bodies || !d_points) return B3W_E_BAD_ARGUMENT;
+  if (key->merged) return merged_key_refused(ctx);
   const uint64_t body = 32ull * ctx->desc.nwit;
   if (pitch == 0) pitch = body;
   if (pitch < body || (pitch & 15) || (reinterpret_cast<uintptr_t>(d_bodies) & 15) || (reinterpret_cast<uintptr_t>(d_points) & 15)) {
@@ -402,6 +426,7 @@
 int32_t b3w_batch_commit(b3w_batch *b, const b3w_commit_key *key, uint8_t *host_points, int32_t *host_status) {
   if (!b || !key || !host_points) return B3W_E_BAD_ARGUMENT;
   b3w_ctx *ctx = b->ctx;
+  if (key->merged) return merged_key_refused(ctx);
   if (!b->n) return B3W_OK;
   ON_DEVICE(ctx);
   uint8_t *d_pts = nullptr;
diff --git a/hot-proofs-blake3-circom_amd/csrc/b3w_commit_merge.cpp b/hot-proofs-blake3-circom_amd/csrc/b3w_commit_merge.cpp
--- /dev/null
+++ b/hot-proofs-blake3-circom_amd/csrc/b3w_commit_merge.cpp
@@ -0,0 +1,104 @@
+#include "b3w_commit_merge.h"
+
+#include <algorithm>
+#include <utility>
+
+#include "b3w_atoms.h"
+
+bool b3w_commit_bits(const uint32_t *table, uint32_t nslots, const uint8_t *folded, B3wCommitBits &out, std::string &err) {
+  std::vector<uint32_t> &nbits = out.nbits, &first_v = out.first_v, &runs = out.runs;
+  nbits.assign(nslots, 0); first_v.assign(nslots, 0); runs.clear();
+  uint64_t nv = 0;
+  for (uint32_t i = 0; i < nslots; i++) {
+    const uint32_t mode = (table[i] >> 17) & 3u;
+    nbits[i] = mode == B3W_MODE_BIT ? 1u : mode == B3W_MODE_W32 ? 32u : mode == B3W_MODE_W64 ? 64u : 256u;
+    if (folded && folded[i] == 1) nbits[i] = 0;
+    else if (folded && (folded[i] & 0x80)) {
+      if (mode != B3W_MODE_W32 || (folded[i] & 0x60)) { err = "commit key: a single-bit fold needs a 32-bit slot and a bit below 32"; return false; }
+      nbits[i] = 1;
+    } else if (folded && folded[i]) { err = "commit key: folded[] holds 0, 1 or 0x80 | bit"; return false; }
+    first_v[i] = (uint32_t)nv;
+    nv += nbits[i];
+  }
+  if (nv >= (1u << 24)) { err = "commit key: more than 2^24 virtual slots"; return false; }
+  out.nv = (uint32_t)nv;
+  auto one_bit_of_word = [&](uint32_t i) { return folded && (folded[i] & 0x80) != 0; };
+  for (uint32_t i = 0; i < nslots; i++) {
+    const uint32_t ent = table[i], src = ent & 0xFFFu, sh = (ent >> 12) & 31u, v0 = first_v[i];
+    if (nbits[i] == 0) continue;
+    if (one_bit_of_word(i)) {
+      runs.push_back(v0 | 0u << 24); runs.push_back(src | (sh + (folded[i] & 31u)) << 16);
+      continue;
+    }
+    if (nbits[i] == 1) {
+      if (!runs.empty()) {
+        const uint32_t a = runs[runs.size() - 2], b = runs[runs.size() - 1];
+        const uint32_t plen = (a >> 24) + 1, pv = a & 0xFFFFFFu, psrc = b & 0xFFFFu, psh = b >> 16;
+        if ((a >> 31) == 0 && psrc == src && psh + plen == sh && pv + plen == v0 && plen < 32 && i > 0 && nbits[i - 1] == 1) {
+          runs[runs.size() - 2] = pv | plen << 24;
+          continue;
+        }
+      }
+      runs.push_back(v0 | 0u << 24); runs.push_back(src | sh << 16);
+    } else {
+      const uint32_t words = nbits[i] / 32;
+      for (uint32_t k = 0; k < words; k++) {
+        runs.push_back((v0 + 32 * k) | 31u << 24); runs.push_back((src + k) | ((k == 0 || k == 4) ? sh : 0u) << 16);
+      }
+    }
+  }
+  return true;
+}
+
+void b3w_commit_merge_classes(const std::vector<uint32_t> &runs, B3wCommitMerge &out) {
+  out = B3wCommitMerge();
+  std::vector<std::pair<uint32_t, uint32_t>> bits;
+  std::vector<std::pair<uint32_t, uint32_t>> wide;
+  for (size_t r = 0; r + 1 < runs.size(); r += 2) {
+    const uint32_t v0 = runs[r] & 0xFFFFFFu, len = (runs[r] >> 24) + 1u, src = runs[r + 1] & 0xFFFFu, sh = runs[r + 1] >> 16;
+    if (src >= B3W_LDS_WIDE) { wide.emplace_back(v0, (uint32_t)r); continue; }
+    for (uint32_t j = 0; j < len; j++) {
+      if (sh + j >= 32) { out.dead++; continue; }
+      bits.emplace_back(src << 5 | (sh + j), v0 + j);
+    }
+  }
+  std::sort(bits.begin(), bits.end());
+  for (size_t i = 0; i < bits.size(); i++) {
+    if (i == 0 || bits[i].first != bits[i - 1].first) {
+      out.class_key.push_back(bits[i].first);
+      out.class_start.push_back((uint32_t)out.members.size());
+    }
+    out.members.push_back(bits[i].second);
+  }
+  out.narrow = (uint32_t)out.class_key.size();
+  for (const auto &w : wide) {
+    const uint32_t len = (runs[w.second] >> 24) + 1u;
+    out.wide.push_back({len, runs[w.second + 1], (uint32_t)out.class_key.size()});
+    for (uint32_t j = 0; j < len; j++) {
+      out.class_key.push_back(0xFFFFFFFFu);
+      out.class_start.push_back((uint32_t)out.members.size());
+      out.members.push_back(w.first + j);
+    }
+  }
+  out.class_start.push_back((uint32_t)out.members.size());
+}
+
+uint32_t b3w_commit_merge_runs(const B3wCommitMerge &m, const uint8_t *dropped, std::vector<uint32_t> &runs, std::vector<uint32_t> &class_v) {
+  runs.clear();
+  class_v.assign(m.class_key.size(), 0xFFFFFFFFu);
+  uint32_t v = 0, next_key = 0xFFFFFFFFu;
+  for (uint32_t c = 0; c < m.narrow; c++) {
+    if (dropped && dropped[c]) continue;
+    const uint32_t key = m.class_key[c];
+    if (key == next_key && (key & 31u) != 0) runs[runs.size() - 2] += 1u << 24;
+    else { runs.push_back(v); runs.push_back((key >> 5) | (key & 31u) << 16); }
+    next_key = key + 1;
+    class_v[c] = v++;
+  }
+  for (const auto &w : m.wide) {
+    runs.push_back(v | (w.len - 1u) << 24); runs.push_back(w.src_sh);
+    for (uint32_t j = 0; j < w.len; j++) class_v[w.first_class + j] = v + j;
+    v += w.len;
+  }
+  return v;
+}
diff --git a/hot-proofs-blake3-circom_amd/csrc/b3w_commit_merge.h b/hot-proofs-blake3-circom_amd/csrc/b3w_commit_merge.h
--- /dev/null
+++ b/hot-proofs-blake3-circom_amd/csrc/b3w_commit_merge.h
@@ -0,0 +1,21 @@
+#pragma once
+#include <stdint.h>
+#include <string>
+#include <vector>
+
+struct B3wCommitBits {
+  std::vector<uint32_t> nbits, first_v, runs;
+  uint32_t nv = 0;
+};
+bool b3w_commit_bits(const uint32_t *table, uint32_t nslots, const uint8_t *folded, B3wCommitBits &out, std::string &err);
+
+struct B3wCommitMerge {
+  std::vector<uint32_t> class_key;
+  std::vector<uint32_t> class_start, members;
+  uint32_t narrow = 0, dead = 0;
+  struct WideRun { uint32_t len, src_sh, first_class; };
+  std::vector<WideRun> wide;
+};
+void b3w_commit_merge_classes(const std::vector<uint32_t> &runs, B3wCommitMerge &out);
+uint32_t b3w_commit_merge_runs(const B3wCommitMerge &m, const uint8_t *dropped , std::vector<uint32_t> &runs,
+                               std::vector<uint32_t> &class_v);
diff --git a/hot-proofs-blake3-circom_amd/csrc/b3w_ctx.cpp b/hot-proofs-blake3-circom_amd/csrc/b3w_ctx.cpp
--- a/hot-proofs-blake3-circom_amd/csrc/b3w_ctx.cpp
+++ b/hot-proofs-blake3-circom_amd/csrc/b3w_ctx.cpp
@@ -1,5 +1,4 @@
 #include "b3w_internal.h"
-#include "b3w_layout_tables.inc"
 #include "b3w_trace_tables.inc"
 
 namespace {
@@ -72,38 +71,6 @@
   for (; *s; ++s) { h ^= (uint8_t)*s; h *= 0x100000001B3ull; }
   return h;
 }
-const CircuitDesc CIRCUITS[4] = {
-    {B3W_KIND_COMP, 24093, 28, 16, P_BN254, B3W_LAYOUT_0, B3W_LAYOUT_0_NRUNS, B3W_LDS_WORDS_COMP},
-    {B3W_KIND_NOVA_O2, 23291, 32, 15, P_BN254, B3W_LAYOUT_1, B3W_LAYOUT_1_NRUNS, B3W_LDS_WORDS_NOVA_O2},
-    {B3W_KIND_NOVA_O2, 23291, 32, 15, P_VESTA, B3W_LAYOUT_2, B3W_LAYOUT_2_NRUNS, B3W_LDS_WORDS_NOVA_O2},
-    {B3W_KIND_NOVA_O1, 24614, 32, 15, P_BN254, B3W_LAYOUT_3, B3W_LAYOUT_3_NRUNS, B3W_LDS_WORDS_NOVA_O1},
-};
-
-bool atom_lds(int kind, uint32_t atom, uint32_t *word, int *width ) {
-  if (atom < B3W_A_HG) { *word = atom; *width = 32; return true; }
-  if (atom < B3W_A_NV) {
-    const uint32_t k = (atom - B3W_A_HG) / 8, j = (atom - B3W_A_HG) % 8;
-    static const uint32_t off[8] = {0, 0, 2, 2, 4, 5, 6, 7};
-    *word = B3W_LDS_HG + 8 * k + off[j];
-    *width = (j == B3W_HG_S1 || j == B3W_HG_S3) ? 64 : 32;
-    return true;
-  }
-  if (kind == B3W_KIND_COMP) return false;
-  const uint32_t i = atom - B3W_A_NV;
-  if (i == NV_CHUNK_IDX) { *word = B3W_LDS_CHUNK_IDX; *width = 64; return true; }
-  if (i < NV_NARROW_COUNT) { *word = B3W_LDS_NV + i; *width = 32; return true; }
-  if (i >= NV_COUNT) return false;
-  uint32_t j = i - NV_NARROW_COUNT;
-  if (kind == B3W_KIND_NOVA_O2) {
-    if (j < 3) {  }
-    else if (i >= NV_EQ_INV && i < NV_EQ_INV + 64) j = 3 + (i - NV_EQ_INV);
-    else return false;
-  }
-  *word = B3W_LDS_WIDE + 8 * j;
-  *width = 256;
-  return true;
-}
-
 void inv_small_host(uint32_t k, const uint32_t P[8], uint32_t out[8]) {
   uint64_t r = 0;
   for (int i = 7; i >= 0; --i) r = ((r << 32) | P[i]) % k;
@@ -140,42 +107,6 @@
   aux[8] = B3W_INV_TABLE_N;
   for (uint32_t k = 1; k < B3W_INV_TABLE_N; ++k) inv_small_host(k, aux.data(), aux.data() + 16 + 8 * k);
   return aux;
-}
-
-bool build_slot_table(const CircuitDesc &c, std::vector<uint32_t> &table, std::string &err) {
-  const uint32_t padded = ((c.nwit + 31) / 32 + 8) * 32;
-  table.assign(padded, B3W_ENTRY(0, 31, B3W_MODE_BIT));
-  std::vector<uint8_t> seen(c.nwit, 0);
-  char msg[128];
-  for (uint32_t r = 0; r < c.nruns; r++) {
-    const b3w_layout_run &run = c.runs[r];
-    for (uint32_t j = 0; j < run.len; j++) {
-      const uint32_t slot = run.slot + j;
-      if (slot >= c.nwit || seen[slot]) { err = "layout: bad or duplicate slot"; return false; }
-      seen[slot] = 1;
-      uint32_t word; int width;
-      if (run.kind == 'W') {
-        if (!atom_lds(c.kind, run.atom + j, &word, &width)) {
-          snprintf(msg, sizeof msg, "layout: atom %u not staged for this circuit kind", run.atom + j);
-          err = msg; return false;
-        }
-        table[slot] = B3W_ENTRY(word, 0, width == 32 ? B3W_MODE_W32 : width == 64 ? B3W_MODE_W64 : B3W_MODE_W256);
-      } else {
-        const uint32_t bit = run.bit0 + j;
-        if (run.atom == B3W_A_NV + NV_CHUNK_IDX && bit == 64) {
-          table[slot] = B3W_ENTRY(B3W_A_ONE, 31, B3W_MODE_BIT);
-          continue;
-        }
-        if (!atom_lds(c.kind, run.atom, &word, &width) || (int)bit >= width || width == 256) {
-          snprintf(msg, sizeof msg, "layout: bit %u of atom %u not expressible", bit, run.atom);
-          err = msg; return false;
-        }
-        table[slot] = B3W_ENTRY(word + bit / 32, bit % 32, B3W_MODE_BIT);
-      }
-    }
-  }
-  for (uint32_t s = 0; s < c.nwit; s++) if (!seen[s]) { err = "layout: uncovered slot"; return false; }
-  return true;
 }
 
 bool build_exact_table(const CircuitDesc &c, std::vector<uint32_t> &table) {
@@ -235,8 +166,6 @@
 
 }
 
-bool b3w_int_build_slot_table(const CircuitDesc &c, std::vector<uint32_t> &table, std::string &err) { return build_slot_table(c, table, err); }
-
 namespace {
 int32_t ensure_scratch(b3w_ctx *ctx) {
   if (ctx->d_scratch) return B3W_OK;
@@ -296,11 +225,11 @@
   if (hipGetDeviceCount(&ndev) != hipSuccess || ndev <= 0 || device < 0 || device >= ndev) return B3W_E_NO_DEVICE;
   b3w_ctx *ctx = new b3w_ctx;
   ctx->circuit = circuit;
-  ctx->desc = CIRCUITS[circuit];
+  ctx->desc = *b3w_int_circuit_desc(circuit);
   ctx->device = device;
   set_inputs(ctx);
   std::vector<uint32_t> table;
-  if (!build_slot_table(ctx->desc, table, ctx->last_error)) { delete ctx; return B3W_E_BAD_ARGUMENT; }
+  if (!b3w_int_build_slot_table(ctx->desc, table, ctx->last_error)) { delete ctx; return B3W_E_BAD_ARGUMENT; }
   std::vector<uint32_t> wide_slots(B3W_NOVA_ISZERO, 0xFFFFFFFFu);
   ctx->fill_ok = ctx->desc.kind == B3W_KIND_COMP || ctx->desc.kind == B3W_KIND_NOVA_O2;
   for (uint32_t i = 0; i < table.size(); i++) {
diff --git a/hot-proofs-blake3-circom_amd/csrc/b3w_internal.h b/hot-proofs-blake3-circom_amd/csrc/b3w_internal.h
--- a/hot-proofs-blake3-circom_amd/csrc/b3w_internal.h
+++ b/hot-proofs-blake3-circom_amd/csrc/b3w_internal.h
@@ -24,22 +24,11 @@
 #include "b3w_capture.h"
 #include "b3w_kernels.h"
 #include "b3w_r1cs_host.h"
+#include "b3w_slot_table.h"
 
-
-struct b3w_layout_run { char kind; uint32_t slot, atom, bit0, len; };
 
 struct InputSignal { const char *name; uint32_t count; uint32_t rec_off; uint64_t hash; };
 
-struct CircuitDesc {
-  int kind;
-  uint32_t nwit, nin, npub;
-  const uint64_t *prime;
-  const b3w_layout_run *runs;
-  uint32_t nruns;
-  uint32_t lds_words;
-};
-inline constexpr uint64_t P_BN254[4] = {0x43e1f593f0000001ull, 0x2833e84879b97091ull, 0xb85045b68181585dull, 0x30644e72e131a029ull};
-inline constexpr uint64_t P_VESTA[4] = {0x8c46eb2100000001ull, 0x224698fc0994a8ddull, 0x0ull, 0x4000000000000000ull};
 constexpr uint32_t B3W_INV_TABLE_N = 2048;
 
 struct b3w_ctx {
@@ -120,7 +109,6 @@
   DeviceGuard _dev_guard((ctx)->device);       \
   if (_dev_guard.err != hipSuccess) return hip_fail(ctx, _dev_guard.err, "hipSetDevice")
 
-bool b3w_int_build_slot_table(const CircuitDesc &c, std::vector<uint32_t> &table, std::string &err);
 int b3w_int_default_variant(const b3w_ctx *ctx, uint32_t n, const uint8_t *d_bodies, uint64_t pitch);
 b3w_ctx *b3w_int_key_ctx(const b3w_commit_key *key);
 int32_t b3w_int_commit_records(b3w_ctx *ctx, const b3w_commit_key *key, const uint32_t *d_records, uint32_t n, uint8_t *d_points, uint32_t *d_public,
diff --git a/hot-proofs-blake3-circom_amd/csrc/b3w_kernels.h b/hot-proofs-blake3-circom_amd/csrc/b3w_kernels.h
--- a/hot-proofs-blake3-circom_amd/csrc/b3w_kernels.h
+++ b/hot-proofs-blake3-circom_amd/csrc/b3w_kernels.h
@@ -74,6 +74,8 @@
 };
 extern "C" int b3w_launch_commit_setup(const uint32_t *d_gens, const uint32_t *d_first_v, const uint32_t *d_nbits, uint32_t nslots,
                                        uint32_t *d_points, const B3wCurve *curve, hipStream_t stream);
+extern "C" int b3w_launch_commit_merge(const uint32_t *d_points, const uint32_t *d_class_start, const uint32_t *d_members, const uint32_t *d_class_v,
+                                       uint32_t nclass, uint32_t *d_merged, uint32_t *d_inf, const B3wCurve *curve, hipStream_t stream);
 extern "C" int b3w_launch_commit_windows(const uint32_t *d_points, uint32_t nwin, uint32_t window, uint32_t *d_table, const B3wCurve *curve, hipStream_t stream);
 extern "C" int b3w_launch_commit(const uint8_t *d_bodies, uint32_t n, uint64_t pitch, uint32_t first_slot, uint32_t nslots,
                                  const uint32_t *d_slotdesc ,
diff --git a/hot-proofs-blake3-circom_amd/csrc/b3w_slot_table.cpp b/hot-proofs-blake3-circom_amd/csrc/b3w_slot_table.cpp
--- /dev/null
+++ b/hot-proofs-blake3-circom_amd/csrc/b3w_slot_table.cpp
@@ -0,0 +1,81 @@
+#include "b3w_slot_table.h"
+
+#include <stdio.h>
+
+#include "b3w_layout_tables.inc"
+
+namespace {
+const CircuitDesc CIRCUITS[4] = {
+    {B3W_KIND_COMP, 24093, 28, 16, P_BN254, B3W_LAYOUT_0, B3W_LAYOUT_0_NRUNS, B3W_LDS_WORDS_COMP},
+    {B3W_KIND_NOVA_O2, 23291, 32, 15, P_BN254, B3W_LAYOUT_1, B3W_LAYOUT_1_NRUNS, B3W_LDS_WORDS_NOVA_O2},
+    {B3W_KIND_NOVA_O2, 23291, 32, 15, P_VESTA, B3W_LAYOUT_2, B3W_LAYOUT_2_NRUNS, B3W_LDS_WORDS_NOVA_O2},
+    {B3W_KIND_NOVA_O1, 24614, 32, 15, P_BN254, B3W_LAYOUT_3, B3W_LAYOUT_3_NRUNS, B3W_LDS_WORDS_NOVA_O1},
+};
+
+
+bool atom_lds(int kind, uint32_t atom, uint32_t *word, int *width ) {
+  if (atom < B3W_A_HG) { *word = atom; *width = 32; return true; }
+  if (atom < B3W_A_NV) {
+    const uint32_t k = (atom - B3W_A_HG) / 8, j = (atom - B3W_A_HG) % 8;
+    static const uint32_t off[8] = {0, 0, 2, 2, 4, 5, 6, 7};
+    *word = B3W_LDS_HG + 8 * k + off[j];
+    *width = (j == B3W_HG_S1 || j == B3W_HG_S3) ? 64 : 32;
+    return true;
+  }
+  if (kind == B3W_KIND_COMP) return false;
+  const uint32_t i = atom - B3W_A_NV;
+  if (i == NV_CHUNK_IDX) { *word = B3W_LDS_CHUNK_IDX; *width = 64; return true; }
+  if (i < NV_NARROW_COUNT) { *word = B3W_LDS_NV + i; *width = 32; return true; }
+  if (i >= NV_COUNT) return false;
+  uint32_t j = i - NV_NARROW_COUNT;
+  if (kind == B3W_KIND_NOVA_O2) {
+    if (j < 3) {  }
+    else if (i >= NV_EQ_INV && i < NV_EQ_INV + 64) j = 3 + (i - NV_EQ_INV);
+    else return false;
+  }
+  *word = B3W_LDS_WIDE + 8 * j;
+  *width = 256;
+  return true;
+}
+
+bool build_slot_table(const CircuitDesc &c, std::vector<uint32_t> &table, std::string &err) {
+  const uint32_t padded = ((c.nwit + 31) / 32 + 8) * 32;
+  table.assign(padded, B3W_ENTRY(0, 31, B3W_MODE_BIT));
+  std::vector<uint8_t> seen(c.nwit, 0);
+  char msg[128];
+  for (uint32_t r = 0; r < c.nruns; r++) {
+    const b3w_layout_run &run = c.runs[r];
+    for (uint32_t j = 0; j < run.len; j++) {
+      const uint32_t slot = run.slot + j;
+      if (slot >= c.nwit || seen[slot]) { err = "layout: bad or duplicate slot"; return false; }
+      seen[slot] = 1;
+      uint32_t word; int width;
+      if (run.kind == 'W') {
+        if (!atom_lds(c.kind, run.atom + j, &word, &width)) {
+          snprintf(msg, sizeof msg, "layout: atom %u not staged for this circuit kind", run.atom + j);
+          err = msg; return false;
+        }
+        table[slot] = B3W_ENTRY(word, 0, width == 32 ? B3W_MODE_W32 : width == 64 ? B3W_MODE_W64 : B3W_MODE_W256);
+      } else {
+        const uint32_t bit = run.bit0 + j;
+        if (run.atom == B3W_A_NV + NV_CHUNK_IDX && bit == 64) {
+          table[slot] = B3W_ENTRY(B3W_A_ONE, 31, B3W_MODE_BIT);
+          continue;
+        }
+        if (!atom_lds(c.kind, run.atom, &word, &width) || (int)bit >= width || width == 256) {
+          snprintf(msg, sizeof msg, "layout: bit %u of atom %u not expressible", bit, run.atom);
+          err = msg; return false;
+        }
+        table[slot] = B3W_ENTRY(word + bit / 32, bit % 32, B3W_MODE_BIT);
+      }
+    }
+  }
+  for (uint32_t s = 0; s < c.nwit; s++) if (!seen[s]) { err = "layout: uncovered slot"; return false; }
+  return true;
+}
+
+}
+
+const CircuitDesc *b3w_int_circuit_desc(int circuit) { return circuit >= 0 && circuit < 4 ? &CIRCUITS[circuit] : nullptr; }
+
+bool b3w_int_build_slot_table(const CircuitDesc &c, std::vector<uint32_t> &table, std::string &err) { return build_slot_table(c, table, err); }
diff --git a/hot-proofs-blake3-circom_amd/csrc/b3w_slot_table.h b/hot-proofs-blake3-circom_amd/csrc/b3w_slot_table.h
--- /dev/null
+++ b/hot-proofs-blake3-circom_amd/csrc/b3w_slot_table.h
@@ -0,0 +1,22 @@
+#pragma once
+#include <stdint.h>
+#include <string>
+#include <vector>
+
+#include "b3w_atoms.h"
+
+struct b3w_layout_run { char kind; uint32_t slot, atom, bit0, len; };
+
+struct CircuitDesc {
+  int kind;
+  uint32_t nwit, nin, npub;
+  const uint64_t *prime;
+  const b3w_layout_run *runs;
+  uint32_t nruns;
+  uint32_t lds_words;
+};
+inline constexpr uint64_t P_BN254[4] = {0x43e1f593f0000001ull, 0x2833e84879b97091ull, 0xb85045b68181585dull, 0x30644e72e131a029ull};
+inline constexpr uint64_t P_VESTA[4] = {0x8c46eb2100000001ull, 0x224698fc0994a8ddull, 0x0ull, 0x4000000000000000ull};
+
+const CircuitDesc *b3w_int_circuit_desc(int circuit);
+bool b3w_int_build_slot_table(const CircuitDesc &c, std::vector<uint32_t> &table, std::string &err);
diff --git a/include/b3wit.h b/include/b3wit.h
--- a/include/b3wit.h
+++ b/include/b3wit.h
@@ -115,6 +115,10 @@
                                      const uint8_t *folded , uint32_t window_bits,
                                      b3w_commit_key **out);
 int32_t b3w_slot_widths(b3w_ctx *ctx, uint16_t *out_bits );
+int32_t b3w_commit_key_create_merged(b3w_ctx *ctx, int32_t curve, uint32_t first_slot, const uint8_t *host_generators,
+                                     const uint8_t *folded , uint32_t window_bits,
+                                     b3w_commit_key **out);
+uint32_t b3w_commit_key_virtual_slots(const b3w_commit_key *key);
 uint32_t b3w_commit_key_window(const b3w_commit_key *key);
 int32_t b3w_commit_key_count(b3w_commit_key *key, int32_t on);
 int32_t b3w_commit_key_counts(const b3w_commit_key *key, uint64_t out[2]);
diff --git a/integrations/rust/b3wit_ffi.rs b/integrations/rust/b3wit_ffi.rs
--- a/integrations/rust/b3wit_ffi.rs
+++ b/integrations/rust/b3wit_ffi.rs
@@ -99,6 +99,9 @@
     pub fn b3w_comm_destroy(comm: *mut c_void);
     pub fn b3w_commit_key_create_ex(ctx: *mut c_void, curve: i32, first_slot: u32, host_generators: *const u8, window_bits: u32,
                                     out: *mut *mut c_void) -> i32;
+    pub fn b3w_commit_key_create_merged(ctx: *mut c_void, curve: i32, first_slot: u32, host_generators: *const u8, folded: *const u8,
+                                        window_bits: u32, out: *mut *mut c_void) -> i32;
+    pub fn b3w_commit_key_virtual_slots(key: *const c_void) -> u32;
     pub fn b3w_commit_key_destroy(key: *mut c_void);
     pub fn b3w_commit_records(ctx: *mut c_void, key: *const c_void, host_records: *const u32, n: u32, host_points: *mut u8,
                               host_public: *mut u32, host_status: *mut i32) -> i32;
```

Result: no change. 9.341 million, median of 3 (-0.1%).
